# THU-DA-6D-Pose-Group/GDR-Net

Hardware: AMD Instinct MI355X
Metric: RoI crops/sec (fwd+bwd) at 256×256 bs=64 (higher is better)
Workload: dtype bf16; 1 GPU; LM-13 a6_cPnP_lm13 graph: ResNet-34 + RotWithRegionHead + ConvPnPNet, 256x256 RoIs, bs=64/GPU, train step: fwd + 8 losses + bwd + fused Ranger optimizer step (all inside the timed region); global_batch=64, parallelism=dp1

## Files before the change

gdr-net_amd/cabi.py:

```python
import ctypes as C
import os

_HERE = os.path.dirname(os.path.abspath(__file__))
LIB_PATH = os.environ.get("GDRN_HIP_LIB") or os.path.join(_HERE, "lib", "libgdrn_hip.so")
LIB_PATH_F16 = os.environ.get("GDRN_HIP_LIB_F16") or os.path.join(_HERE, "lib", "libgdrn_hip_f16.so")

F32, BF16, F16 = 0, 1, 2
PREZEROED = 0x100
ACC_ROWS = 0x200
P = C.c_void_p
I = C.c_int
LL = C.c_longlong
F = C.c_float
D = C.c_double


class GdrnHipError(RuntimeError):
    pass


class ConvParams(C.Structure):
    _fields_ = [
        ("x", P), ("w", P), ("y", P), ("bias", P), ("addend", P), ("stats", P),
        ("bnb_x", P), ("bnb_mask", P), ("bnb_mean", P), ("bnb_invstd", P), ("bnb_scale", P), ("bnb_shift", P), ("bnb_rows", P),
        ("bnb_cs", I), ("w_frag", I),
        ("Hi", I), ("Wi", I), ("Cin", I), ("x_cs", I),
        ("Ho", I), ("Wo", I), ("Cout", I), ("y_cs", I), ("add_cs", I),
        ("KH", I), ("KW", I), ("stride", I), ("pad", I),
        ("mode", I), ("act", I), ("out_f32", I),
        ("M", I), ("w_rows", I), ("dtype", I),
        ("xf_mode", I), ("xf_relu", I),
        ("xf_x2", P), ("xf_a", P), ("xf_b", P), ("xf_c", P), ("xf_c2", P), ("xf_msc", P), ("xf_msh", P), ("xf_out", P),
        ("halo_waves", I), ("v3_min_wg", I),
    ]


class WgradParams(C.Structure):
    _fields_ = [
        ("x", P), ("dy", P), ("dw", P), ("ws", P),
        ("Hi", I), ("Wi", I), ("Cin", I), ("x_cs", I),
        ("Ho", I), ("Wo", I), ("Cout", I), ("dy_cs", I),
        ("KH", I), ("KW", I), ("stride", I), ("pad", I),
        ("M", I), ("dtype", I), ("splits", I), ("variant", I),
    ]


class S2Params(C.Structure):
    _fields_ = [
        ("x", P), ("w", P), ("y", P), ("bias", P), ("stats", P), ("wd", P), ("yd", P), ("bias_d", P), ("stats_d", P),
        ("Hi", I), ("Wi", I), ("Cin", I), ("x_cs", I),
        ("Ho", I), ("Wo", I), ("Cout", I), ("y_cs", I), ("yd_cs", I),
        ("N", I), ("w_rows", I), ("wd_rows", I), ("act", I), ("dtype", I),
        ("bnb_x", P), ("bnb_mask", P), ("bnb_mean", P), ("bnb_invstd", P), ("bnb_rows", P), ("bnb_cs", I),
    ]


class S2dParams(C.Structure):
    _fields_ = [
        ("dy", P), ("w", P), ("dx", P), ("dyd", P), ("wdd", P), ("bnb_x", P), ("bnb_mask", P), ("bnb_mean", P), ("bnb_invstd", P), ("bnb_rows", P),
        ("bnb_cs", I),
        ("Hi", I), ("Wi", I), ("Cin", I), ("dx_cs", I),
        ("Ho", I), ("Wo", I), ("Cout", I), ("dy_cs", I), ("dyd_cs", I),
        ("N", I), ("w_rows", I), ("wdd_rows", I), ("dtype", I),
        ("stats", P), ("bias", P), ("act", I),
    ]


class PoseParams(C.Structure):
    _fields_ = [
        ("fc", P), ("fs", I), ("cams", P), ("centers", P), ("whs", P), ("ratios", P), ("extents", P),
        ("gt_rot", P), ("gt_trans", P), ("gt_trans_ratio", P), ("points", P), ("npts", I),
        ("sym", P), ("sym_count", P), ("Kmax", I), ("N", I), ("train", I),
        ("rot", P), ("trans", P), ("losses", P), ("dfc", P), ("vis", P),
        ("loss_rows", P), ("gw", P), ("dfc_comb", P), ("fc2_ws", P), ("fc2_bias", P), ("f2_out", P), ("w_rt", P), ("b_rt", P), ("fc_w", P), ("fc2_splits", I),
    ]


class PackTask(C.Structure):
    _fields_ = [
        ("src", P), ("dst", P), ("scale", P),
        ("A1", I), ("A2", I), ("T", I), ("B", I), ("A1v", I), ("A2v", I), ("Bv", I), ("flip", I),
        ("s1", LL), ("s2", LL), ("st", LL), ("sb", LL), ("n", LL), ("frag", I), ("pad_", I),
    ]


def transpose_blocks(lib, t):
    if t.frag or t.flip or t.scale or t.sb == 1:
        return 0
    for u, (stride, size) in enumerate(((t.s1, t.A1), (t.s2, t.A2), (t.st, t.T)), start=1):
        if stride == 1 and size >= 32:
            t.frag, t.pad_ = 3, u
            nb = int(lib.gdrn_pack_transpose_blocks(C.byref(t)))
            if nb > 0:
                return nb
            t.frag, t.pad_ = 0, 0
    return 0


class ZeroTask(C.Structure):
    _fields_ = [("p", P), ("n16", LL)]


class WreduceTask(C.Structure):
    _fields_ = [("ws", P), ("dst", P), ("nsplit", I), ("Cout", I), ("Cin", I), ("cin_valid", I), ("s_co", LL), ("s_ci", LL), ("s_t", LL)]


class RangerTask(C.Structure):
    _fields_ = [("p", P), ("g", P), ("m", P), ("v", P), ("slow", P), ("rows", I), ("cols", I), ("gc", I), ("lr", F)]


class RoiTask(C.Structure):
    _fields_ = [
        ("image", P), ("coord2d", P), ("xyz_crop", P), ("seg", P), ("trunc", P),
        ("cx", D), ("cy", D), ("scale", D), ("bw", D), ("bh", D), ("ox", D), ("oy", D), ("tz", D),
        ("H", I), ("W", I), ("x1", I), ("y1", I), ("x2", I), ("y2", I), ("cls", I), ("pad_", I),
    ]


class AugTask(C.Structure):
    _fields_ = [
        ("frame", P), ("mask", P), ("bg", P), ("out", P), ("mask_trunc", P),
        ("inv_scale", D), ("trunc_u", D),
        ("H", I), ("W", I), ("bg_h", I), ("bg_w", I), ("ch", I), ("cw", I), ("oh", I), ("ow", I),
        ("trunc_mode", I), ("gh", I), ("gw", I), ("keep_off", I), ("lut_off", I), ("blur_r", I),
        ("blur_w", F * 9),
    ]


class RleTask(C.Structure):
    _fields_ = [
        ("mask", P), ("sy", LL), ("sx", LL), ("str_off", LL), ("run_off", LL), ("seg_off", LL),
        ("str_len", I), ("h", I), ("w", I), ("pad_", I),
    ]


def to_device_table(structs, device):
    import torch

    arr = (type(structs[0]) * len(structs))(*structs)
    return torch.frombuffer(bytearray(bytes(arr)), dtype=torch.uint8).to(device)


_SIGS = {
    "gdrn_version": [],
    "gdrn_last_hip_error": [C.c_char_p, I],
    "gdrn_workspace_bytes": [I, P],
    "gdrn_device_info": [I, C.c_char_p, C.POINTER(I), C.c_char_p],
    "gdrn_conv_gemm": [C.POINTER(ConvParams), P],
    "gdrn_correspondences": [P, P, P, P, LL, I, P, P, P, F, I, I, P, P, P, P, P, P],
    "gdrn_pack_stem_w32": [P, P, I, P],
    "gdrn_stem_stats_rows": [I],
    "gdrn_stem_conv": [P, P, P, P, I, I, P],
    "gdrn_stem_conv_pool": [P, P, P, P, P, I, I, P],
    "gdrn_head_conv_tail_fwd": [P, I, P, I, P, P, P, P, I, P, I, I, I, I, I, P],
    "gdrn_head_conv_tail_loss_rows": [I, I],
    "gdrn_head_out_dgrad_rows": [I, I],
    "gdrn_head_out_dgrad": [P, I, P, I, P, I, P, P, P, P, P, I, P, I, I, I, P],
    "gdrn_head_conv_tail_loss_fwd": [P, I, P, I, P, P, P, P, I, P, I, P, P, P, P, P, I, I, I, I, P],
    "gdrn_stem_wgrad_parts": [I],
    "gdrn_stem_wgrad": [P, P, P, P, P, P, I, P, P, I, P],
    "gdrn_linear_splitk": [P, P, P, P, I, I, I, I, I, I, I, P, I, P],
    "gdrn_conv_tile": [C.POINTER(ConvParams), C.POINTER(I), C.POINTER(I)],
    "gdrn_conv_stats_rows": [C.POINTER(ConvParams)],
    "gdrn_pack_wfrag": [P, P, I, I, I, P],
    "gdrn_pack_wfrag32": [P, P, I, I, I, P],
    "gdrn_conv3x3_wfrag": [C.POINTER(ConvParams)],
    "gdrn_conv3x3_halo": [C.POINTER(ConvParams), P],
    "gdrn_conv3x3_tile": [C.POINTER(ConvParams), C.POINTER(I), C.POINTER(I), C.POINTER(I)],
    "gdrn_conv3x3_stats_rows": [C.POINTER(ConvParams)],
    "gdrn_conv3x3_halo_waves": [C.POINTER(ConvParams)],
    "gdrn_conv_wgrad": [C.POINTER(WgradParams), P],
    "gdrn_conv3x3_wgrad": [C.POINTER(WgradParams), P],
    "gdrn_conv3x3_wgrad_ok": [C.POINTER(WgradParams)],
    "gdrn_conv3x3_wgrad_splits": [C.POINTER(WgradParams)],
    "gdrn_conv3x3_wgrad_multi": [P, P, I, I, P],
    "gdrn_conv3x3_wgrad_multi_lds": [P, P, I, I, I, P],
    "gdrn_wgrad_reduce_multi": [P, P, I, I, P],
    "gdrn_pack4": [P, P, I, I, I, I, I, I, I, LL, LL, LL, LL, I, I, P],
    "gdrn_unpack4": [P, P, I, I, I, I, I, I, I, LL, LL, LL, LL, I, P],
    "gdrn_pack_stem_w": [P, P, I, P],
    "gdrn_unpack_stem_w": [P, P, P],
    "gdrn_pack_image": [P, P, I, I, I, I, I, I, P],
    "gdrn_cast_from_f32": [P, P, LL, I, P],
    "gdrn_cast_to_f32": [P, P, LL, I, P],
    "gdrn_nhwc_to_nchw_f32": [P, I, I, I, P, I, I, I, P],
    "gdrn_bn_finalize": [P, I, I, D, P, P, P, P, P, F, F, P, P, P, P, P, P],
    "gdrn_bn_eval_params": [P, P, P, P, F, I, P, P, P],
    "gdrn_bn_apply": [P, P, P, P, P, LL, I, I, I, P],
    "gdrn_bn_bwd_reduce_rows": [LL, I, I],
    "gdrn_bn_bwd_reduce": [P, P, P, P, P, P, P, LL, I, P, I, P],
    "gdrn_bn_bwd_coef": [P, I, I, LL, P, P, P, P, P, P, P, P, P],
    "gdrn_bn_bwd_apply": [P, P, P, P, P, P, P, P, LL, I, P, P, I, P],
    "gdrn_bn_relu_maxpool_fwd": [P, P, P, P, P, I, I, I, I, I, P],
    "gdrn_maxpool_bwd_rows": [I, I, I, I, I],
    "gdrn_maxpool_bwd": [P, P, P, P, P, P, I, I, I, I, P, P, P, I, P],
    "gdrn_upsample2x_fwd": [P, P, I, I, I, I, I, P],
    "gdrn_upsample2x_bwd": [P, P, I, I, I, I, I, P],
    "gdrn_conv3x3s2_ok": [C.POINTER(S2Params)],
    "gdrn_conv3x3s2_stats_rows": [C.POINTER(S2Params)],
    "gdrn_conv3x3s2": [C.POINTER(S2Params), P],
    "gdrn_conv3x3s2_dgrad_ok": [C.POINTER(S2dParams)],
    "gdrn_conv3x3s2_dgrad_rows": [C.POINTER(S2dParams)],
    "gdrn_conv3x3s2_dgrad": [C.POINTER(S2dParams), P],
    "gdrn_block64_eval_ok": [I, I, I, I],
    "gdrn_block64_eval": [P, P, P, P, P, P, I, I, I, I, P],
    "gdrn_bn_relu_upsample2x_fwd": [P, P, P, P, I, I, I, I, I, P],
    "gdrn_upsample2x_bwd_bnsums": [P, P, P, P, P, P, P, I, I, I, I, P, I, P],
    "gdrn_gn_relu_fwd": [P, P, P, P, P, I, I, I, I, F, I, P],
    "gdrn_gn_relu_bwd": [P, P, P, P, P, P, P, P, I, I, I, I, I, P],
    "gdrn_leaky_bwd": [P, P, P, LL, I, P],
    "gdrn_bias_grad": [P, I, I, I, P, I, P],
    "gdrn_head_tail_fwd": [P, I, P, P, P, I, I, I, I, I, P],
    "gdrn_head_tail_loss_fwd": [P, I, P, P, P, I, P, P, P, P, P, I, I, I, I, P],
    "gdrn_map_loss_fwd": [P, I, P, P, P, P, I, I, I, P, P],
    "gdrn_map_loss_finalize": [P, I, I, P, P],
    "gdrn_head_tail_loss_rows": [I, I, I, I, I],
    "gdrn_map_loss_finalize_rows": [P, I, I, I, P, P],
    "gdrn_loss_finalize": [P, I, I, I, P, P, P, P, P],
    "gdrn_linear_splits": [I, I],
    "gdrn_head_tail_bwd": [P, I, P, P, I, P, P, P, P, P, P, P, P, I, I, I, I, I, P],
    "gdrn_pose_loss": [C.POINTER(PoseParams), P],
    "gdrn_combine3": [P, P, P, I, P],
    "gdrn_ranger_step": [P, P, P, P, P, I, I, I, F, F, F, F, F, F, I, I, F, P],
    "gdrn_pack_chunk": [],
    "gdrn_zero_chunk": [],
    "gdrn_zero_multi": [P, P, I, I, P],
    "gdrn_nonfinite_flag": [P, LL, P, P],
    "gdrn_pack_multi": [P, P, I, I, I, P],
    "gdrn_pack_transpose_blocks": [P],
    "gdrn_unpack_multi": [P, P, I, I, P],
    "gdrn_ranger_multi": [P, P, I, I, F, F, F, F, F, I, I, F, F, P],
    "gdrn_ranger_multi_dyn": [P, P, I, I, F, F, F, F, I, I, F, F, P, P],
    "gdrn_loss_scale_update": [P, I, P],
    "gdrn_unscale_or_zero": [P, LL, F, P, P],
    "gdrn_scaled_loss_weights": [P, P, I, P, P, P],
    "gdrn_roi_affine": [P, I, I, I, P, P, P, P, P],
    "gdrn_roi_crop_inputs": [P, P, I, I, I, C.POINTER(D), C.POINTER(D), P, P, P],
    "gdrn_roi_targets": [P, P, I, I, P, I, P, P, P, P, P, P, P],
    "gdrn_pose_metrics_workspace_bytes": [I, I],
    "gdrn_pose_errors": [P, P, P, P, P, P, P, I, P, P, I, P, P, P, I, I, P, P, P],
    "gdrn_pose_recall_accumulate": [P, P, P, I, P, I, P, P, P, P, P, P],
    "gdrn_pnp_workspace_bytes": [I, I, I],
    "gdrn_pnp_ransac": [P, P, P, P, P, I, I, D, I, C.c_ulonglong, I, P, P, P, P, P, P, P, P],
    "gdrn_pnp_refine": [P, P, P, P, P, I, I, I, P, P, P, P, P, P],
    "gdrn_pnp_ransac_f64": [P, P, P, P, P, I, I, D, I, C.c_ulonglong, I, P, P, P, P, P, P, P, P],
    "gdrn_pnp_refine_f64": [P, P, P, P, P, I, I, I, P, P, P, P, P, P],
    "gdrn_render_depth": [P, P, P, P, P, P, I, I, P, P, P, P, P, I, I, I, D, D, P, P],
    "gdrn_xyz_from_depth": [P, P, P, P, I, I, I, P, P, P, P, P],
    "gdrn_vsd_workspace_bytes": [I, I, I, I],
    "gdrn_vsd": [P, P, P, P, P, I, P, P, I, I, I, D, P, I, I, I, P, P, P, P],
    "gdrn_mssd_mspd_workspace_bytes": [I, I, I],
    "gdrn_mssd_mspd": [P, P, P, P, P, P, P, I, P, P, I, P, P, P, I, I, P, P, P],
    "gdrn_bop_recall_accumulate": [P, I, P, P, P, I, P, I, D, P, P, P, P, P, P, P, P],
    "gdrn_ad_errors_workspace_bytes": [I, I],
    "gdrn_ad_errors": [P, P, P, P, P, P, I, P, P, I, I, P, P, P],
    "gdrn_sym_errors_workspace_bytes": [I, I, I],
    "gdrn_sym_errors": [P, P, P, P, P, P, P, I, P, P, I, P, P, P, I, I, P, P, P],
    "gdrn_score_recall_accumulate": [P, P, P, P, I, P, P, I, P, P, P],
    "gdrn_aug_mask_cuts": [P, C.POINTER(AugTask), I, P, P],
    "gdrn_aug_frames": [P, C.POINTER(AugTask), I, P, LL, P, P],
    "gdrn_rle_decode": [P, C.POINTER(RleTask), I, P, LL, P, LL, P, P, P],
    "gdrn_rle_count": [P, C.POINTER(RleTask), I, P, LL, P, P, P],
    "gdrn_rle_positions": [P, C.POINTER(RleTask), I, P, LL, P, P, LL, P],
    "gdrn_rle_string": [P, C.POINTER(RleTask), I, P, P, LL, P, P, LL, P, P],
    "gdrn_model_prep_workspace_bytes": [I, I, I],
    "gdrn_model_bounds": [P, P, P, I, I, P, P],
    "gdrn_model_fps": [P, P, P, I, I, I, P, P, P, P],
    "gdrn_model_diameter": [P, P, P, I, I, P, P],
    "gdrn_scene_gt_canvas": [P, I, I, I, I, I, P, P, P, P],
    "gdrn_scene_gt_compose": [P, P, P, P, P, I, I, I, I, P, P],
    "gdrn_scene_gt_visibility": [P, P, P, P, I, P, I, I, I, D, I, P, P, P, P, P, P, P, P, P],
    "gdrn_render_visibility": [P, P, P, P, P, P, I, I, P, P, P, P, P, I, I, I, D, D, P, P],
    "gdrn_shade_frames": [P, P, P, P, P, P, P, P, P, I, P, P, P, P, P, P, P, P, P, I, I, I, I, P, P, P, P, P, P, P, P, P],
    "gdrn_shade_frames_tex": [P, P, P, P, P, P, P, P, P, P, P, P, P, I, I, P, P, P, P, P, P, P, P, P, I, I, I, I, P, P, I, I, P, P, P, P, P, P, P],
    "gdrn_cou_maps_workspace_bytes": [I],
    "gdrn_cou_maps": [P, P, I, I, I, I, P, P, P, P, P],
    "gdrn_cou_bb": [P, P, I, P, P],
    "gdrn_icp_workspace_bytes": [I, I, I],
    "gdrn_icp_accumulate": [P, P, P, P, I, P, I, I, I, D, D, P, P, P, P],
    "gdrn_icp_step": [P, P, I, I, P, P, P, P],
    "gdrn_icp_refine": [P, P, P, P, P, P, I, I, P, P, P, P, P, I, P, P, P, I, I, I, D, D, I, D, D, I, P, P, P, P, P, P, P],
    "gdrn_depth_align_workspace_bytes": [I, I, I],
    "gdrn_depth_offset": [P, P, P, P, I, I, I, I, D, I, P, P, P, P, P, P],
    "gdrn_depth_align": [P, P, P, P, P, P, I, I, P, P, P, P, P, I, P, P, P, I, I, I, D, D, I, D, I, P, P, P, P, P, P, P],
    "gdrn_sil_workspace_bytes": [I, I, I],
    "gdrn_sil_contour_transform": [P, P, P, P, I, I, I, I, P, P, P, P, P],
    "gdrn_sil_accumulate": [P, P, P, P, I, P, P, P, I, I, I, D, D, P, P, P, P],
    "gdrn_icp_step_sil": [P, P, P, P, D, I, I, P, P, P, P],
    "gdrn_icp_refine_sil": [P, P, P, P, P, P, I, I, P, P, P, P, P, I, P, P, P, I, P, I, I, D, D, I, D, D, I, D, D, P, P, P, P, P, P, P, P, P],
}

_SIGS["gdrn_half_format"] = []
_RET_LL = ("gdrn_workspace_bytes", "gdrn_pose_metrics_workspace_bytes", "gdrn_pnp_workspace_bytes", "gdrn_vsd_workspace_bytes",
           "gdrn_mssd_mspd_workspace_bytes", "gdrn_model_prep_workspace_bytes", "gdrn_ad_errors_workspace_bytes",
           "gdrn_sym_errors_workspace_bytes", "gdrn_cou_maps_workspace_bytes", "gdrn_icp_workspace_bytes",
           "gdrn_depth_align_workspace_bytes", "gdrn_sil_workspace_bytes")
EXPORTS = tuple(_SIGS.keys())
_libs = {}


def lib_path(dtype=BF16):
    return LIB_PATH_F16 if dtype == F16 else LIB_PATH


def load(dtype=BF16):
    kind = F16 if dtype == F16 else BF16
    if kind in _libs:
        return _libs[kind]
    import torch

    path = lib_path(kind)
    if not os.path.exists(path):
# ... 32 lines not shown
```

gdr-net_amd/csrc/conv_wgrad.hip:

```cpp
#include <hip/amd_detail/amd_hip_unsafe_atomics.h>

#include <cstdlib>

#include "common.h"
#include "launch_host.h"

namespace {

typedef __attribute__((address_space(3))) bf16x4_t lds_bf16x4_t;

template <typename T, int BCO, int BCI>
__global__ __launch_bounds__(256) void conv_wgrad_kernel(const gdrn_wgrad_params p) {
    constexpr int ESZ = (int)sizeof(T);
    constexpr int BKM = (ESZ == 2) ? 64 : 32;
    constexpr int PADB = (ESZ == 2) ? 32 : 64;
    constexpr int PA = BCO * ESZ + PADB, PB = BCI * ESZ + PADB;
    constexpr int SEGA = BCO * ESZ / 16, SEGB = BCI * ESZ / 16;
    constexpr int LDA = BKM * SEGA / 256, LDB = BKM * SEGB / 256;
    constexpr int RSA = 256 / SEGA, RSB = 256 / SEGB;
    constexpr int WCO = BCO / 2, WCI = BCI / 2;
    constexpr int FA = WCO / 16, FB = WCI / 16;
    extern __shared__ __attribute__((aligned(16))) unsigned char smem[];
    unsigned char* sA = smem;
    unsigned char* sB = smem + 2 * BKM * PA;

    const int tid = threadIdx.x, lane = tid & 63, wave = tid >> 6;
    const int wa = wave >> 1, wb = wave & 1;
    const int g = lane >> 4, r16 = lane & 15;

    const int KK = p.KH * p.KW;
    const int ncit = p.Cin / BCI;
    const int ncot = (p.Cout + BCO - 1) / BCO;
    const int ntile = ncot * ncit * KK;
    const int nsplit = (int)gridDim.x / ntile;
    int bid = blockIdx.x;
    {
        const int nwg = gridDim.x, q = nwg >> 3, r = nwg & 7, xcd = bid & 7, j = bid >> 3;
        bid = (xcd < r ? xcd * (q + 1) : r * (q + 1) + (xcd - r) * q) + j;
    }
    const int split = bid / ntile;
    int tile = bid - split * ntile;
    const int cot = tile % ncot; tile /= ncot;
    const int cit = tile % ncit;
    const int tap = tile / ncit;
    const int co0 = cot * BCO, ci0 = cit * BCI;
    const int ky = tap / p.KW, kx = tap - ky * p.KW;

    const int nstage_all = (p.M + BKM - 1) / BKM;
    const int per = (nstage_all + nsplit - 1) / nsplit;
    const int s_begin = split * per;
    const int s_end = min(nstage_all, s_begin + per);
    if (s_begin >= s_end) return;

    const int segA = tid % SEGA, rowA = tid / SEGA;
    const int segB = tid % SEGB, rowB = tid / SEGB;
    const char* dyg = reinterpret_cast<const char*>(p.dy);
    const char* xg = reinterpret_cast<const char*>(p.x);
    const int HW = p.Ho * p.Wo;
    const bool pow2 = (p.Wo & (p.Wo - 1)) == 0 && (HW & (HW - 1)) == 0;
    const int lgW = 31 - __builtin_clz(p.Wo), lgHW = 31 - __builtin_clz(HW);

    uint4 ra[LDA], rb[LDB];
    auto load_stage = [&](int s) {
        const int m0 = s * BKM;
#pragma unroll
        for (int i = 0; i < LDA; ++i) {
            const int m = m0 + rowA + RSA * i;
            uint4 v = make_uint4(0, 0, 0, 0);
            if (m < p.M) v = *reinterpret_cast<const uint4*>(dyg + ((size_t)m * p.dy_cs + co0) * ESZ + segA * 16);
            ra[i] = v;
        }
#pragma unroll
        for (int i = 0; i < LDB; ++i) {
            const int m = m0 + rowB + RSB * i;
            uint4 v = make_uint4(0, 0, 0, 0);
            if (m < p.M) {
                int n, oy, ox;
                if (pow2) {
                    n = m >> lgHW;
                    const int rem = m & (HW - 1);
                    oy = rem >> lgW;
                    ox = rem & (p.Wo - 1);
                } else {
                    n = m / HW;
                    const int rem = m - n * HW;
                    oy = rem / p.Wo;
                    ox = rem - oy * p.Wo;
                }
                const int iy = oy * p.stride - p.pad + ky, ix = ox * p.stride - p.pad + kx;
                if (iy >= 0 && iy < p.Hi && ix >= 0 && ix < p.Wi)
                    v = *reinterpret_cast<const uint4*>(xg + ((size_t)((n * p.Hi + iy) * p.Wi + ix) * p.x_cs + ci0) * ESZ + segB * 16);
            }
            rb[i] = v;
        }
    };
    auto write_stage = [&](int buf) {
#pragma unroll
        for (int i = 0; i < LDA; ++i)
            *reinterpret_cast<uint4*>(sA + (size_t)buf * BKM * PA + (rowA + RSA * i) * PA + segA * 16) = ra[i];
#pragma unroll
        for (int i = 0; i < LDB; ++i)
            *reinterpret_cast<uint4*>(sB + (size_t)buf * BKM * PB + (rowB + RSB * i) * PB + segB * 16) = rb[i];
    };

    f32x4_t acc[FA][FB];
#pragma unroll
    for (int a = 0; a < FA; ++a)
#pragma unroll
        for (int b = 0; b < FB; ++b) acc[a][b] = f32x4_t{0.f, 0.f, 0.f, 0.f};

    load_stage(s_begin);
    write_stage(0);
    __syncthreads();

    for (int s = s_begin; s < s_end; ++s) {
        const int buf = (s - s_begin) & 1;
        if (s + 1 < s_end) load_stage(s + 1);
        const unsigned char* tA = sA + (size_t)buf * BKM * PA;
        const unsigned char* tB = sB + (size_t)buf * BKM * PB;
        if constexpr (ESZ == 2) {
#pragma unroll
            for (int ks = 0; ks < BKM / 32; ++ks) {
                bf16x8_t fa[FA], fb[FB];
                {
                    const int trow = ks * 32 + g * 4 + (r16 >> 2), tcol = (r16 & 3) * 4;
#pragma unroll
                    for (int a = 0; a < FA; ++a) {
                        const unsigned char* q0 = tA + trow * PA + (wa * WCO + a * 16 + tcol) * 2;
                        bf16x4_t lo = GDRN_TR16((lds_bf16x4_t*)(q0));
                        bf16x4_t hi = GDRN_TR16((lds_bf16x4_t*)(q0 + 16 * PA));
                        fa[a] = __builtin_shufflevector(lo, hi, 0, 1, 2, 3, 4, 5, 6, 7);
                    }
#pragma unroll
                    for (int b = 0; b < FB; ++b) {
                        const unsigned char* q0 = tB + trow * PB + (wb * WCI + b * 16 + tcol) * 2;
                        bf16x4_t lo = GDRN_TR16((lds_bf16x4_t*)(q0));
                        bf16x4_t hi = GDRN_TR16((lds_bf16x4_t*)(q0 + 16 * PB));
                        fb[b] = __builtin_shufflevector(lo, hi, 0, 1, 2, 3, 4, 5, 6, 7);
                    }
                }
#pragma unroll
                for (int a = 0; a < FA; ++a)
#pragma unroll
                    for (int b = 0; b < FB; ++b)
                        acc[a][b] = GDRN_MFMA16(fa[a], fb[b], acc[a][b]);
            }
        } else {
#pragma unroll 4
            for (int ks = 0; ks < BKM / 4; ++ks) {
                float fa[FA], fb[FB];
                const int mrow = ks * 4 + g;
#pragma unroll
                for (int a = 0; a < FA; ++a)
                    fa[a] = *reinterpret_cast<const float*>(tA + mrow * PA + (wa * WCO + a * 16 + r16) * 4);
#pragma unroll
                for (int b = 0; b < FB; ++b)
                    fb[b] = *reinterpret_cast<const float*>(tB + mrow * PB + (wb * WCI + b * 16 + r16) * 4);
#pragma unroll
                for (int a = 0; a < FA; ++a)
#pragma unroll
                    for (int b = 0; b < FB; ++b)
                        acc[a][b] = __builtin_amdgcn_mfma_f32_16x16x4f32(fa[a], fb[b], acc[a][b], 0, 0, 0);
            }
        }
        if (s + 1 < s_end) write_stage(buf ^ 1);
        __syncthreads();
    }

#pragma unroll
    for (int a = 0; a < FA; ++a) {
#pragma unroll
        for (int j = 0; j < 4; ++j) {
            const int co = co0 + wa * WCO + a * 16 + g * 4 + j;
            if (co >= p.Cout) continue;
#pragma unroll
            for (int b = 0; b < FB; ++b) {
                const int ci = ci0 + wb * WCI + b * 16 + r16;
                unsafeAtomicAdd(p.dw + ((size_t)co * KK + tap) * p.Cin + ci, acc[a][b][j]);
            }
        }
    }
}

template <typename T, int BCO, int BCI>
int launch(const gdrn_wgrad_params& p, hipStream_t st) {
    constexpr int ESZ = (int)sizeof(T);
    constexpr int BKM = (ESZ == 2) ? 64 : 32;
    constexpr int PADB = (ESZ == 2) ? 32 : 64;
    constexpr size_t smem = 2 * (size_t)BKM * ((BCO * ESZ + PADB) + (BCI * ESZ + PADB));
    if (!lds_limit_once<&conv_wgrad_kernel<T, BCO, BCI>>(smem)) return GDRN_ERR_LAUNCH;
    const int tiles = cdiv(p.Cout, BCO) * (p.Cin / BCI) * p.KH * p.KW;
    int splits = p.splits;
    if (splits <= 0) {
        const int nst = cdiv(p.M, BKM);
        constexpr int target = 2048;
        splits = max(1, min(nst / 8 > 0 ? nst / 8 : 1, cdiv(target, tiles)));
    }
    GDRN_LAUNCH((conv_wgrad_kernel<T, BCO, BCI>), dim3(tiles * splits), dim3(256), smem, st, p);
    GDRN_CHECK_LAUNCH();
    return GDRN_OK;
}

}

extern "C" int gdrn_conv_wgrad(const gdrn_wgrad_params* pp, void* stream) {
    if (!pp || !pp->x || !pp->dy || !pp->dw) return GDRN_ERR_ARG;
    const gdrn_wgrad_params& p = *pp;
    if (p.dtype != GDRN_DT_F32 && p.dtype != GDRN_DT_H16) return GDRN_ERR_ARG;
    const int esz = p.dtype == GDRN_DT_H16 ? 2 : 4;
    if (p.Cin <= 0 || p.Cin % 64 != 0 || p.M <= 0 || p.Cout <= 0) return GDRN_ERR_SHAPE;
    if (p.KH <= 0 || p.KW <= 0 || p.stride <= 0 || p.pad < 0 || p.Hi <= 0 || p.Wi <= 0 || p.Ho <= 0 || p.Wo <= 0) return GDRN_ERR_SHAPE;
    if (p.M % (p.Ho * p.Wo) != 0) return GDRN_ERR_SHAPE;
    if (p.x_cs <= 0 || ((p.x_cs * esz) % 16 != 0 && (p.x_cs * esz) % 8 != 0)) return GDRN_ERR_SHAPE;
    if ((p.dy_cs * esz) % 16 != 0) return GDRN_ERR_SHAPE;
    const int bco = p.Cout <= 64 ? 64 : 128;
    const int bci = (p.Cin % 128 == 0) ? 128 : 64;
    if (p.dy_cs < cdiv(p.Cout, bco) * bco) return GDRN_ERR_SHAPE;
    hipStream_t st = reinterpret_cast<hipStream_t>(stream);
    if (p.dtype == GDRN_DT_H16) {
        if (bco == 64) return bci == 64 ? launch<bf16_t, 64, 64>(p, st) : launch<bf16_t, 64, 128>(p, st);
        return bci == 64 ? launch<bf16_t, 128, 64>(p, st) : launch<bf16_t, 128, 128>(p, st);
    } else {
        if (bco == 64) return bci == 64 ? launch<float, 64, 64>(p, st) : launch<float, 64, 128>(p, st);
        return bci == 64 ? launch<float, 128, 64>(p, st) : launch<float, 128, 128>(p, st);
    }
}
```

gdr-net_amd/csrc/multi.hip:

```cpp
#include <algorithm>

#include "common.h"
#include "../../include/gdrn_hip.h"

namespace {

__device__ __forceinline__ int find_task(const int* __restrict__ start, int n, int b) {
    int lo = 0, hi = n;
    while (hi - lo > 1) {
        const int mid = (lo + hi) >> 1;
        if (start[mid] <= b) lo = mid; else hi = mid;
    }
    return lo;
}

constexpr int PACK_CHUNK = 2048;

struct TrGeo { int U, Uv, O1, O2, O1v, O2v, UT, BT; };
__host__ __device__ inline TrGeo tr_geo(const gdrn_pack_task& k) {
    TrGeo g;
    const int d[3] = {k.A1, k.A2, k.T}, dv[3] = {k.A1v, k.A2v, k.T};
    const int u = k.pad_ - 1, a = u == 0 ? 1 : 0, b = u == 2 ? 1 : 2;
    g.U = d[u]; g.Uv = dv[u]; g.O1 = d[a]; g.O2 = d[b]; g.O1v = dv[a]; g.O2v = dv[b];
    g.UT = (g.U + 63) / 64; g.BT = (k.B + 63) / 64;
    return g;
}
__host__ inline bool tr_ok(const gdrn_pack_task& k) {
    if (k.frag != 3 || k.pad_ < 1 || k.pad_ > 3 || k.flip || k.scale != nullptr) return false;
    const long long s[3] = {k.s1, k.s2, k.st};
    return s[k.pad_ - 1] == 1 && k.A1 > 0 && k.A2 > 0 && k.T > 0 && k.B > 0;
}
__device__ __forceinline__ void tr_idx(const gdrn_pack_task& k, int u, int o1, int o2, int& a1, int& a2, int& t) {
    if (k.pad_ == 1) { a1 = u; a2 = o1; t = o2; }
    else if (k.pad_ == 2) { a1 = o1; a2 = u; t = o2; }
    else { a1 = o1; a2 = o2; t = u; }
}
template <typename T, bool UNPACK>
__device__ __forceinline__ void tr_tile(const gdrn_pack_task& k, int blk) {
    __shared__ float tile[64][68];
    const TrGeo g = tr_geo(k);
    const int bt = blk % g.BT; blk /= g.BT;
    const int ut = blk % g.UT; blk /= g.UT;
    const int o2 = blk % g.O2, o1 = blk / g.O2;
    const int u0 = ut * 64, b0 = bt * 64;
    const long long sa = (k.pad_ == 1 ? 0 : k.s1) | (k.pad_ == 2 ? 0 : k.s2) | (k.pad_ == 3 ? 0 : k.st) | k.sb;
    const bool v4 = (sa & 3) == 0 && (g.Uv & 3) == 0 && (reinterpret_cast<uintptr_t>(UNPACK ? k.dst : (const void*)k.src) & 15) == 0;
    const bool b8 = (k.B & 7) == 0 && (reinterpret_cast<uintptr_t>(UNPACK ? (const void*)k.src : k.dst) & 15) == 0;
    auto strided = [&](int u, int b) -> long long {
        int a1, a2, t;
        tr_idx(k, u, o1, o2, a1, a2, t);
        return (long long)a1 * k.s1 + (long long)a2 * k.s2 + (long long)t * k.st + (long long)b * k.sb;
    };
    auto dense = [&](int u, int b) -> long long {
        int a1, a2, t;
        tr_idx(k, u, o1, o2, a1, a2, t);
        return (((long long)a1 * k.A2 + a2) * k.T + t) * k.B + b;
    };
    auto valid = [&](int u, int b) -> bool {
        int a1, a2, t;
        tr_idx(k, u, o1, o2, a1, a2, t);
        return u < g.Uv && b < k.Bv && a1 < k.A1v && a2 < k.A2v;
    };
    if constexpr (!UNPACK) {
        if (v4) {
            for (int i = threadIdx.x; i < 1024; i += 256) {
                const int u4 = (i & 15) * 4, bb = i >> 4, u = u0 + u4, b = b0 + bb;
                float4 v = make_float4(0.f, 0.f, 0.f, 0.f);
                if (valid(u, b)) v = *reinterpret_cast<const float4*>(k.src + strided(u, b));
                *reinterpret_cast<float4*>(&tile[bb][u4]) = v;
            }
        } else {
            for (int i = threadIdx.x; i < 4096; i += 256) {
                const int uu = i & 63, bb = i >> 6, u = u0 + uu, b = b0 + bb;
                tile[bb][uu] = valid(u, b) ? k.src[strided(u, b)] : 0.f;
            }
        }
        __syncthreads();
        T* dst = reinterpret_cast<T*>(k.dst);
        if (b8) {
            for (int i = threadIdx.x; i < 512; i += 256) {
                const int b8_ = (i & 7) * 8, uu = i >> 3, u = u0 + uu, b = b0 + b8_;
                if (u < g.U && b < k.B) {
                    float v[8];
#pragma unroll
                    for (int j2 = 0; j2 < 8; ++j2) v[j2] = tile[b8_ + j2][uu];
                    T* d = dst + dense(u, b);
                    if constexpr (sizeof(T) == 2) *reinterpret_cast<uint4*>(d) = Vec16<T>::pack(v);
                    else { Vec16<T>::store(d, v); Vec16<T>::store(d + 4, v + 4); }
                }
            }
        } else {
            for (int i = threadIdx.x; i < 4096; i += 256) {
                const int bb = i & 63, uu = i >> 6, u = u0 + uu, b = b0 + bb;
                if (u < g.U && b < k.B) st1<T>(dst + dense(u, b), tile[bb][uu]);
            }
        }
    } else {
        if (b8) {
            for (int i = threadIdx.x; i < 1024; i += 256) {
                const int b4 = (i & 15) * 4, uu = i >> 4, u = u0 + uu, b = b0 + b4;
                float4 v = make_float4(0.f, 0.f, 0.f, 0.f);
                if (u < g.U && b < k.B) v = *reinterpret_cast<const float4*>(k.src + dense(u, b));
                tile[b4][uu] = v.x; tile[b4 + 1][uu] = v.y; tile[b4 + 2][uu] = v.z; tile[b4 + 3][uu] = v.w;
            }
        } else {
            for (int i = threadIdx.x; i < 4096; i += 256) {
                const int bb = i & 63, uu = i >> 6, u = u0 + uu, b = b0 + bb;
                tile[bb][uu] = (u < g.U && b < k.B) ? k.src[dense(u, b)] : 0.f;
            }
        }
        __syncthreads();
        float* dst = reinterpret_cast<float*>(k.dst);
        if (v4) {
            for (int i = threadIdx.x; i < 1024; i += 256) {
                const int u4 = (i & 15) * 4, bb = i >> 4, u = u0 + u4, b = b0 + bb;
                if (valid(u, b)) *reinterpret_cast<float4*>(dst + strided(u, b)) = *reinterpret_cast<const float4*>(&tile[bb][u4]);
            }
        } else {
            for (int i = threadIdx.x; i < 4096; i += 256) {
                const int uu = i & 63, bb = i >> 6, u = u0 + uu, b = b0 + bb;
                if (valid(u, b)) dst[strided(u, b)] = tile[bb][uu];
            }
        }
    }
}

template <typename T>
__global__ __launch_bounds__(256) void pack_multi_kernel(const gdrn_pack_task* __restrict__ tasks, const int* __restrict__ blk_start,
                                                         int ntasks) {
    constexpr int EPS = 128 / (int)sizeof(T), GE = 16 / (int)sizeof(T);
    const int t = find_task(blk_start, ntasks, blockIdx.x);
    const gdrn_pack_task k = tasks[t];
    T* dst = reinterpret_cast<T*>(k.dst);
    if (k.frag == 3) { tr_tile<T, false>(k, blockIdx.x - blk_start[t]); return; }
    if constexpr (sizeof(T) == 2) {
        if (k.frag) {
            __shared__ bf16_t tile[16][9][72];
            const int brick = blockIdx.x - blk_start[t];
            const int kch = k.B >> 6;
            const int cb = brick / kch, kc = brick - cb * kch;
            const int b0 = kc * 64;
            const int FNp = k.A1 <= 64 ? 1 : 2;
            auto srow = [&](int a) {
                if (k.frag == 2) { const int f = cb >> 1, r = (cb & 1) * 16 + a; return (f >> 1) * 64 + ((r >> 2) & 1) * 32 + (f & 1) * 16 + (r >> 3) * 4 + (r & 3); }
                return (cb / FNp) * 16 * FNp + (a >> 2) * (4 * FNp) + (cb % FNp) * 4 + (a & 3);
            };
            __shared__ float rsc[16];
            if (threadIdx.x < 16) rsc[threadIdx.x] = (k.scale != nullptr && srow((int)threadIdx.x) < k.A1v) ? k.scale[srow((int)threadIdx.x)] : 1.f;
            __syncthreads();
            const bool full = srow(15) < k.A1v && b0 + 63 < k.Bv && ((size_t)k.src & 15) == 0;
            if (full && k.st == 1 && k.sb == 9 && (k.s1 & 3) == 0) {
                for (int q = threadIdx.x; q < 16 * 144; q += 256) {
                    const int a = q / 144, r4 = (q - a * 144) * 4;
                    const float4 v4 = *reinterpret_cast<const float4*>(k.src + (long long)srow(a) * k.s1 + (long long)b0 * 9 + r4);
                    const float vv[4] = {v4.x, v4.y, v4.z, v4.w};
#pragma unroll
                    for (int e = 0; e < 4; ++e) {
                        const int r = r4 + e, b = r / 9, tp = r - b * 9;
                        tile[a][k.flip ? 8 - tp : tp][b] = f2bf(vv[e] * rsc[a]);
                    }
                }
            } else if (full && k.st == 1 && k.s1 == 9 && (k.sb & 3) == 0) {
                for (int q = threadIdx.x; q < 64 * 4 * 9; q += 256) {
                    const int b = q / 36, r = q - b * 36, grp = r / 9, f4 = r - grp * 9;
                    const float4 v4 = *reinterpret_cast<const float4*>(k.src + (long long)srow(grp * 4) * 9 + (long long)(b0 + b) * k.sb + f4 * 4);
                    const float vv[4] = {v4.x, v4.y, v4.z, v4.w};
#pragma unroll
                    for (int e = 0; e < 4; ++e) {
                        const int w = f4 * 4 + e, al = w / 9, tp = w - al * 9, a = grp * 4 + al;
                        tile[a][k.flip ? 8 - tp : tp][b] = f2bf(vv[e] * rsc[a]);
                    }
                }
            } else if (k.st == 1 && k.sb == 9) {
                for (int idx = threadIdx.x; idx < 16 * 576; idx += 256) {
                    const int a = idx / 576, r = idx - a * 576, b = r / 9, tp = r - b * 9;
                    const bool ok = srow(a) < k.A1v && b0 + b < k.Bv;
                    const float v = ok ? k.src[(long long)srow(a) * k.s1 + (long long)(b0 + b) * 9 + tp] * rsc[a] : 0.f;
                    tile[a][k.flip ? 8 - tp : tp][b] = f2bf(v);
                }
            } else if (k.st == 1 && k.s1 == 9) {
                for (int idx = threadIdx.x; idx < 64 * 144; idx += 256) {
                    const int b = idx / 144, r = idx - b * 144, a = r / 9, tp = r - a * 9;
                    const bool ok = srow(a) < k.A1v && b0 + b < k.Bv;
                    const float v = ok ? k.src[(long long)srow(a) * 9 + (long long)(b0 + b) * k.sb + tp] * rsc[a] : 0.f;
                    tile[a][k.flip ? 8 - tp : tp][b] = f2bf(v);
                }
            } else {
                for (int idx = threadIdx.x; idx < 16 * 576; idx += 256) {
                    const int a = idx / 576, r = idx - a * 576, b = r / 9, tp = r - b * 9;
                    const bool ok = srow(a) < k.A1v && b0 + b < k.Bv;
                    const float v = ok ? k.src[(long long)srow(a) * k.s1 + (long long)(b0 + b) * k.sb + (long long)tp * k.st] * rsc[a] : 0.f;
                    tile[a][k.flip ? 8 - tp : tp][b] = f2bf(v);
                }
            }
            __syncthreads();
            if (k.frag == 2) {
                const int nfr = k.A1 >> 5, f = cb >> 1, half = cb & 1;
                for (int gi = threadIdx.x; gi < 9 * 4 * 32; gi += 256) {
                    const int a = gi & 15, hh = (gi >> 4) & 1, ks = (gi >> 5) & 3, tap = gi >> 7;
                    const uint4 v = *reinterpret_cast<const uint4*>(&tile[a][tap][(ks * 2 + hh) * 8]);
                    *reinterpret_cast<uint4*>(dst + ((size_t)((((kc * 9 + tap) * 4 + ks) * nfr + f) * 64 + hh * 32 + half * 16 + a) << 3)) = v;
                }
                return;
            }
            for (int gi = threadIdx.x; gi < 9 * 2 * 64; gi += 256) {
                const int lane = gi & 63, ks = (gi >> 6) & 1, tap = gi >> 7;
                const uint4 v = *reinterpret_cast<const uint4*>(&tile[lane & 15][tap][(ks * 4 + (lane >> 4)) * 8]);
                *reinterpret_cast<uint4*>(dst + ((size_t)((((cb * 9 + tap) * kch + kc) * 2 + ks) * 64 + lane) << 3)) = v;
            }
            return;
        }
    }
    const long long base = (long long)(blockIdx.x - blk_start[t]) * PACK_CHUNK;
    if ((k.B % GE) == 0 && (k.n % GE) == 0) {
        const unsigned B = (unsigned)k.B, Tt = (unsigned)k.T, A2 = (unsigned)k.A2;
        for (int g = threadIdx.x; g < PACK_CHUNK / GE; g += 256) {
            const long long i = base + (long long)g * GE;
            if (i >= k.n) break;
            unsigned a1, a2, tt, b0;
            unsigned r = (unsigned)(i / GE);
            if (k.frag) {
                const unsigned lane = r & 63u; r >>= 6;
                const unsigned ks = r & 1u; r >>= 1;
                const unsigned kch = B / EPS;
                unsigned kc;
                if (k.pad_ > 0) { kc = r & (kch - 1u); r >>= (unsigned)(k.pad_ - 1); }
                else { kc = r % kch; r /= kch; }
                tt = r % 9u;
                {
                    const unsigned cbq = r / 9u, rr = lane & 15u, fnp = (k.A1 <= 64 || sizeof(T) == 4) ? 1u : 2u;
                    a1 = (cbq / fnp) * 16u * fnp + (rr >> 2) * (4u * fnp) + (cbq % fnp) * 4u + (rr & 3u);
                }
                a2 = 0;
                b0 = kc * EPS + (ks * 4u + (lane >> 4)) * GE;
            } else {
                const unsigned bg = B / GE;
                b0 = (r % bg) * GE; r /= bg;
                tt = r % Tt; r /= Tt;
                a2 = r % A2;
                a1 = r / A2;
            }
            float v[GE];
            const bool ok = (int)a1 < k.A1v && (int)a2 < k.A2v;
            const unsigned ts = k.flip ? (Tt - 1u - tt) : tt;
            const float* sp = k.src + (long long)a1 * k.s1 + (long long)a2 * k.s2 + (long long)ts * k.st;
            const float rs = (k.scale != nullptr && ok) ? k.scale[a1] : 1.f;
#pragma unroll
            for (int el = 0; el < GE; ++el) {
                const int b = (int)b0 + el;
                v[el] = (ok && b < k.Bv) ? sp[(long long)b * k.sb] * rs : 0.f;
            }
            Vec16<T>::store(dst + i, v);
        }
        return;
    }
    for (int e = threadIdx.x; e < PACK_CHUNK; e += 256) {
        const long long i = base + e;
        if (i >= k.n) break;
        int a1, a2, tt, b;
        if (k.frag) {
            const int el = (int)(i % GE);
            long long r = i / GE;
            const int lane = (int)(r & 63); r >>= 6;
            const int ks = (int)(r & 1); r >>= 1;
            const int kch = k.B / EPS;
            const int kc = (int)(r % kch); r /= kch;
            tt = (int)(r % 9);
            {
                const int cbq = (int)(r / 9), rr = lane & 15, fnp = (k.A1 <= 64 || sizeof(T) == 4) ? 1 : 2;
                a1 = (cbq / fnp) * 16 * fnp + (rr >> 2) * (4 * fnp) + (cbq % fnp) * 4 + (rr & 3);
            }
            a2 = 0;
            b = kc * EPS + (ks * 4 + (lane >> 4)) * GE + el;
        } else {
            b = (int)(i % k.B);
            long long r = i / k.B;
            tt = (int)(r % k.T); r /= k.T;
            a2 = (int)(r % k.A2);
            a1 = (int)(r / k.A2);
        }
        float v = 0.f;
        if (a1 < k.A1v && a2 < k.A2v && b < k.Bv) {
            const int ts = k.flip ? (k.T - 1 - tt) : tt;
            v = k.src[a1 * k.s1 + a2 * k.s2 + ts * k.st + b * k.sb] * (k.scale != nullptr ? k.scale[a1] : 1.f);
        }
        st1<T>(dst + i, v);
    }
}

constexpr int ZERO_CHUNK = 4096;
__global__ __launch_bounds__(256) void zero_multi_kernel(const gdrn_zero_task* __restrict__ tasks, const int* __restrict__ blk_start, int ntasks) {
    const int t = find_task(blk_start, ntasks, blockIdx.x);
    const gdrn_zero_task k = tasks[t];
    const long long base = (long long)(blockIdx.x - blk_start[t]) * ZERO_CHUNK;
    uint4* dst = reinterpret_cast<uint4*>(k.p);
    for (int i = threadIdx.x; i < ZERO_CHUNK; i += 256) {
        const long long g = base + i;
        if (g >= k.n16) break;
        dst[g] = make_uint4(0u, 0u, 0u, 0u);
    }
}

__global__ __launch_bounds__(256) void unpack_multi_kernel(const gdrn_pack_task* __restrict__ tasks, const int* __restrict__ blk_start,
                                                           int ntasks) {
    const int t = find_task(blk_start, ntasks, blockIdx.x);
    const gdrn_pack_task k = tasks[t];
    if (k.frag == 3) { tr_tile<float, true>(k, blockIdx.x - blk_start[t]); return; }
    const long long base = (long long)(blockIdx.x - blk_start[t]) * PACK_CHUNK;
    float* dst = reinterpret_cast<float*>(k.dst);
    if ((k.Bv & 3) == 0 && (k.B & 3) == 0) {
        const unsigned bq = (unsigned)k.Bv >> 2, Tt = (unsigned)k.T, A2v = (unsigned)k.A2v;
        for (int g = threadIdx.x; g < PACK_CHUNK / 4; g += 256) {
            const long long i = base + (long long)g * 4;
            if (i >= k.n) break;
            unsigned r = (unsigned)(i >> 2);
            const unsigned b = (r % bq) * 4u; r /= bq;
            const unsigned tt = r % Tt; r /= Tt;
            const unsigned a2 = r % A2v, a1 = r / A2v;
            const unsigned ts = k.flip ? (Tt - 1u - tt) : tt;
            const float4 v = *reinterpret_cast<const float4*>(k.src + (((long long)a1 * k.A2 + a2) * k.T + tt) * k.B + b);
            float* dp = dst + (long long)a1 * k.s1 + (long long)a2 * k.s2 + (long long)ts * k.st + (long long)b * k.sb;
            dp[0] = v.x;
            dp[k.sb] = v.y;
            dp[2 * k.sb] = v.z;
            dp[3 * k.sb] = v.w;
        }
        return;
    }
    for (int e = threadIdx.x; e < PACK_CHUNK; e += 256) {
        const long long i = base + e;
        if (i >= k.n) break;
        const int b = (int)(i % k.Bv);
        long long r = i / k.Bv;
        const int tt = (int)(r % k.T); r /= k.T;
        const int a2 = (int)(r % k.A2v);
        const int a1 = (int)(r / k.A2v);
        const int ts = k.flip ? (k.T - 1 - tt) : tt;
        dst[a1 * k.s1 + a2 * k.s2 + ts * k.st + b * k.sb] = k.src[(((long long)a1 * k.A2 + a2) * k.T + tt) * k.B + b];
    }
}

__global__ __launch_bounds__(256) void ranger_multi_kernel(const gdrn_ranger_task* __restrict__ tasks, const int* __restrict__ row_start,
                                                           int ntasks, float beta1, float beta2, float eps, float wd, float step_size,
                                                           int adaptive, int lookahead, float alpha, float grad_scale,
                                                           const gdrn_loss_scale_state* __restrict__ dyn, int n_sma_threshold, int lookahead_k) {
    __shared__ float red[4];
    if (dyn != nullptr) {
        if (dyn->flag != 0) return;
        const int step = dyn->base_step + dyn->applied + 1;
        const double b2t = pow((double)beta2, (double)step), b1t = pow((double)beta1, (double)step);
        const double nmax = 2.0 / (1.0 - (double)beta2) - 1.0;
        const double nsma = nmax - 2.0 * step * b2t / (1.0 - b2t);
        adaptive = nsma > (double)n_sma_threshold;
        step_size = (float)(adaptive ? sqrt((1.0 - b2t) * (nsma - 4.0) / (nmax - 4.0) * (nsma - 2.0) / nsma * nmax / (nmax - 2.0)) / (1.0 - b1t)
                                     : 1.0 / (1.0 - b1t));
        lookahead = (step % lookahead_k) == 0;
        grad_scale *= dyn->inv_scale;
    }
    const int t = find_task(row_start, ntasks, blockIdx.x);
    const gdrn_ranger_task k = tasks[t];
    const size_t base = (size_t)(blockIdx.x - row_start[t]) * k.cols;
    ranger_row(k.p + base, k.g + base, k.m + base, k.v + base, k.slow + base, k.cols, k.gc, k.lr, beta1, beta2, eps, wd, step_size, adaptive, lookahead, alpha,
               grad_scale, red);
}

}

#define ST reinterpret_cast<hipStream_t>(stream)

extern "C" int gdrn_pack_chunk(void) { return PACK_CHUNK; }

extern "C" int gdrn_pack_transpose_blocks(const gdrn_pack_task* k) {
    if (!k || !tr_ok(*k)) return 0;
    const TrGeo g = tr_geo(*k);
    const long long nb = (long long)g.O1 * g.O2 * g.UT * g.BT;
    return nb > 0 && nb < (1ll << 30) ? (int)nb : 0;
}

extern "C" int gdrn_pack_multi(const gdrn_pack_task* tasks_dev, const int* blk_start_dev, int ntasks, int nblocks, int dtype, void* stream) {
    if (!tasks_dev || !blk_start_dev || ntasks <= 0 || nblocks <= 0) return GDRN_ERR_ARG;
    if (dtype == GDRN_DT_F32) GDRN_LAUNCH(pack_multi_kernel<float>, dim3(nblocks), dim3(256), 0, ST, tasks_dev, blk_start_dev, ntasks);
    else if (dtype == GDRN_DT_H16) GDRN_LAUNCH(pack_multi_kernel<bf16_t>, dim3(nblocks), dim3(256), 0, ST, tasks_dev, blk_start_dev, ntasks);
    else return GDRN_ERR_ARG;
    GDRN_CHECK_LAUNCH();
    return GDRN_OK;
}

extern "C" int gdrn_unpack_multi(const gdrn_pack_task* tasks_dev, const int* blk_start_dev, int ntasks, int nblocks, void* stream) {
    if (!tasks_dev || !blk_start_dev || ntasks <= 0 || nblocks <= 0) return GDRN_ERR_ARG;
    GDRN_LAUNCH(unpack_multi_kernel, dim3(nblocks), dim3(256), 0, ST, tasks_dev, blk_start_dev, ntasks);
    GDRN_CHECK_LAUNCH();
    return GDRN_OK;
}

extern "C" int gdrn_zero_chunk(void) { return ZERO_CHUNK; }

namespace {
__global__ __launch_bounds__(256) void nonfinite_flag_kernel(const float* __restrict__ x, long long n, int* __restrict__ flag) {
    const long long n4 = n >> 2;
    unsigned bad = 0;
    for (long long i = (long long)blockIdx.x * 256 + threadIdx.x; i < n4; i += (long long)gridDim.x * 256) {
        const uint4 v = *reinterpret_cast<const uint4*>(x + 4 * i);
        bad |= ((v.x & 0x7f800000u) == 0x7f800000u) | ((v.y & 0x7f800000u) == 0x7f800000u) | ((v.z & 0x7f800000u) == 0x7f800000u) |
               ((v.w & 0x7f800000u) == 0x7f800000u);
    }
    if (blockIdx.x == 0 && threadIdx.x < (int)(n & 3)) bad |= (__float_as_uint(x[(n4 << 2) + threadIdx.x]) & 0x7f800000u) == 0x7f800000u;
    if (__any(bad != 0) && (threadIdx.x & 63) == 0) atomicOr(flag, 1);
}
}

extern "C" int gdrn_nonfinite_flag(const float* x, long long n, int* flag, void* stream) {
    if (!x || !flag || n <= 0 || (reinterpret_cast<uintptr_t>(x) & 15)) return GDRN_ERR_ARG;
    const int grid = (int)std::min<long long>(((n >> 2) + 255) / 256 + 1, 2048);
    GDRN_LAUNCH(nonfinite_flag_kernel, dim3(grid), dim3(256), 0, ST, x, n, flag);
    GDRN_CHECK_LAUNCH();
    return GDRN_OK;
}

extern "C" int gdrn_zero_multi(const gdrn_zero_task* tasks_dev, const int* blk_start_dev, int ntasks, int nblocks, void* stream) {
    if (!tasks_dev || !blk_start_dev || ntasks <= 0 || nblocks <= 0) return GDRN_ERR_ARG;
    GDRN_LAUNCH(zero_multi_kernel, dim3(nblocks), dim3(256), 0, ST, tasks_dev, blk_start_dev, ntasks);
    GDRN_CHECK_LAUNCH();
    return GDRN_OK;
}

extern "C" int gdrn_ranger_multi(const gdrn_ranger_task* tasks_dev, const int* row_start_dev, int ntasks, int total_rows, float beta1,
                                 float beta2, float eps, float weight_decay, float step_size, int adaptive, int lookahead, float alpha, float grad_scale,
                                 void* stream) {
    if (!tasks_dev || !row_start_dev || ntasks <= 0 || total_rows <= 0) return GDRN_ERR_ARG;
    GDRN_LAUNCH(ranger_multi_kernel, dim3(total_rows), dim3(256), 0, ST, tasks_dev, row_start_dev, ntasks, beta1, beta2, eps,
                       weight_decay, step_size, adaptive, lookahead, alpha, grad_scale, (const gdrn_loss_scale_state*)nullptr, 0, 1);
    GDRN_CHECK_LAUNCH();
    return GDRN_OK;
}

extern "C" int gdrn_ranger_multi_dyn(const gdrn_ranger_task* tasks_dev, const int* row_start_dev, int ntasks, int total_rows, float beta1,
                                     float beta2, float eps, float weight_decay, int n_sma_threshold, int lookahead_k, float alpha, float grad_scale,
                                     const gdrn_loss_scale_state* dyn, void* stream) {
    if (!tasks_dev || !row_start_dev || !dyn || ntasks <= 0 || total_rows <= 0 || lookahead_k < 1) return GDRN_ERR_ARG;
    GDRN_LAUNCH(ranger_multi_kernel, dim3(total_rows), dim3(256), 0, ST, tasks_dev, row_start_dev, ntasks, beta1, beta2, eps,
                       weight_decay, 0.f, 0, 0, alpha, grad_scale, dyn, n_sma_threshold, lookahead_k);
    GDRN_CHECK_LAUNCH();
    return GDRN_OK;
}

namespace {
__global__ void loss_scale_update_kernel(gdrn_loss_scale_state* __restrict__ s, int applied_step) {
    if (threadIdx.x != 0 || blockIdx.x != 0) return;
    if (s->flag != 0) {
        s->scale = fmaxf(s->scale * 0.5f, 1.f);
        s->good = 0;
        s->skipped += 1;
        s->flag = 0;
        s->last_overflowed = 1;
    } else {
        s->applied += applied_step;
        s->good += 1;
        s->last_overflowed = 0;
        if (s->growth > 0 && s->good >= s->growth && s->scale < 65536.f) {
            s->scale *= 2.f;
            s->good = 0;
// ... 45 lines not shown
```

gdr-net_amd/csrc/norm.hip:

```cpp
#include <hip/amd_detail/amd_hip_unsafe_atomics.h>

#include <algorithm>

#include "common.h"
#include "../../include/gdrn_hip.h"

namespace {

__device__ __forceinline__ void rows_total4(const float* __restrict__ rows, int nrows, int C, int c4, double (&tot)[8], double (*red)[8]) {
    double s[8] = {0.0, 0.0, 0.0, 0.0, 0.0, 0.0, 0.0, 0.0};
#pragma unroll 4
    for (int r = threadIdx.x; r < nrows; r += 256) {
        const float4 a = *reinterpret_cast<const float4*>(rows + ((size_t)r * 2 + 0) * C + c4);
        const float4 b = *reinterpret_cast<const float4*>(rows + ((size_t)r * 2 + 1) * C + c4);
        s[0] += (double)a.x; s[1] += (double)a.y; s[2] += (double)a.z; s[3] += (double)a.w;
        s[4] += (double)b.x; s[5] += (double)b.y; s[6] += (double)b.z; s[7] += (double)b.w;
    }
#pragma unroll
    for (int j = 0; j < 8; ++j)
#pragma unroll
        for (int o = 32; o > 0; o >>= 1) s[j] += __shfl_xor(s[j], o, 64);
    if ((threadIdx.x & 63) == 0) {
#pragma unroll
        for (int j = 0; j < 8; ++j) red[threadIdx.x >> 6][j] = s[j];
    }
    __syncthreads();
#pragma unroll
    for (int j = 0; j < 8; ++j) tot[j] = red[0][j] + red[1][j] + red[2][j] + red[3][j];
}

__global__ __launch_bounds__(256) void bn_finalize_rows_kernel(const float* __restrict__ partial, int rows, int C, double count,
                                                               const float* gamma, const float* beta, float* running_mean,
                                                               float* running_var, long long* nbt, float momentum, float eps,
                                                               float* mean, float* invstd, float* scale, float* shift) {
    __shared__ double red[4][8];
    double tot[8];
    const int c4 = blockIdx.x * 4;
    float k_g = 0.f, k_b = 0.f, k_rm = 0.f, k_rv = 0.f;
    if (threadIdx.x < 4) {
        k_g = gamma[c4 + threadIdx.x];
        k_b = beta[c4 + threadIdx.x];
        if (running_mean != nullptr) { k_rm = running_mean[c4 + threadIdx.x]; k_rv = running_var[c4 + threadIdx.x]; }
    }
    rows_total4(partial, rows, C, c4, tot, red);
    if (threadIdx.x < 4) {
        const int ch = c4 + threadIdx.x;
        const double s1 = tot[threadIdx.x], s2 = tot[4 + threadIdx.x];
        const double m = s1 / count;
        double var = s2 / count - m * m;
        if (var < 0.0) var = 0.0;
        const double is = 1.0 / sqrt(var + (double)eps);
        mean[ch] = (float)m;
        invstd[ch] = (float)is;
        const float sc = k_g * (float)is;
        scale[ch] = sc;
        shift[ch] = k_b - (float)m * sc;
        if (running_mean != nullptr) {
            const double unb = count > 1.0 ? var * count / (count - 1.0) : var;
            running_mean[ch] = (1.f - momentum) * k_rm + momentum * (float)m;
            running_var[ch] = (1.f - momentum) * k_rv + momentum * (float)unb;
        }
    }
    if (blockIdx.x == 0 && threadIdx.x == 0 && nbt != nullptr) *nbt += 1;
}

__global__ __launch_bounds__(256) void bn_bwd_coef_kernel(const float* __restrict__ rows, int nrows, int C, float inv_n,
                                                          const float* gamma, const float* mean, const float* invstd,
                                                          float* ka, float* kb, float* kc, float* dgamma, float* dbeta) {
    __shared__ double red[4][8];
    double tot[8];
    const int c4 = blockIdx.x * 4;
    float k_g = 0.f, k_mu = 0.f, k_is = 0.f;
    if (threadIdx.x < 4) { k_g = gamma[c4 + threadIdx.x]; k_mu = mean[c4 + threadIdx.x]; k_is = invstd[c4 + threadIdx.x]; }
    rows_total4(rows, nrows, C, c4, tot, red);
    if (threadIdx.x < 4) {
        const int ch = c4 + threadIdx.x;
        float m1 = (float)tot[threadIdx.x], m2 = (float)tot[4 + threadIdx.x];
        if (dgamma != nullptr) { dbeta[ch] = m1; dgamma[ch] = m2; }
        m1 *= inv_n;
        m2 *= inv_n;
        const float a = k_g * k_is, b = -a * k_is * m2;
        ka[ch] = a;
        kb[ch] = b;
        kc[ch] = -a * m1 - b * k_mu;
    }
}

__global__ void bn_eval_params_kernel(const float* gamma, const float* beta, const float* rm, const float* rv, float eps,
                                      int C, float* scale, float* shift) {
    const int c = blockIdx.x * blockDim.x + threadIdx.x;
    if (c < C) {
        const float sc = gamma[c] / sqrtf(rv[c] + eps);
        scale[c] = sc;
        shift[c] = beta[c] - rm[c] * sc;
    }
}

template <typename T>
__global__ __launch_bounds__(256) void bn_apply_kernel(const T* __restrict__ x, const float* __restrict__ scale,
                                                       const float* __restrict__ shift, const T* __restrict__ res,
                                                       T* __restrict__ y, long long npix, int C, int relu, int rows_per_block) {
    constexpr int V = Vec16<T>::VEC;
    const int tpr = C / V, rpp = 256 / tpr;
    const int cv = threadIdx.x % tpr, rl = threadIdx.x / tpr;
    __shared__ float kst[2][512];
    for (int c = threadIdx.x; c < C; c += 256) { kst[0][c] = scale[c]; kst[1][c] = shift[c]; }
    __syncthreads();
    float sc[V], sh[V];
#pragma unroll
    for (int j = 0; j < V; ++j) { sc[j] = kst[0][cv * V + j]; sh[j] = kst[1][cv * V + j]; }
    const long long r0 = (long long)blockIdx.x * rows_per_block;
    const long long r1 = min(npix, r0 + rows_per_block);
    if (rl >= rpp) return;
    for (long long r = r0 + rl; r < r1; r += rpp) {
        const size_t o = (size_t)r * C + cv * V;
        float v[V], q[V];
        Vec16<T>::load(x + o, v);
        if (res != nullptr) Vec16<T>::load(res + o, q);
#pragma unroll
        for (int j = 0; j < V; ++j) {
            float t = __builtin_fmaf(v[j], sc[j], sh[j]);
            if (res != nullptr) t += q[j];
            if (relu) t = fmaxf(t, 0.f);
            v[j] = t;
        }
        Vec16<T>::store(y + o, v);
    }
}

template <typename T>
__global__ __launch_bounds__(256) void bn_bwd_reduce_kernel(const T* __restrict__ dy, const T* __restrict__ ym,
                                                            const T* __restrict__ x, const float* __restrict__ mean,
                                                            const float* __restrict__ invstd, const float* __restrict__ msc,
                                                            const float* __restrict__ msh, long long npix, int C,
                                                            float* __restrict__ rows, int rows_per_block) {
    constexpr int V = Vec16<T>::VEC;
    const int tpr = C / V, rpp = 256 / tpr;
    const int cv = threadIdx.x % tpr, rl = threadIdx.x / tpr;
    __shared__ float kst[4][512];
    __shared__ float part[4][2 * 512];
    for (int c = threadIdx.x; c < C; c += 256) {
        kst[0][c] = mean[c];
        kst[1][c] = invstd[c];
        kst[2][c] = msc ? msc[c] : 0.f;
        kst[3][c] = msc ? msh[c] : 1.f;
    }
// ... 711 lines not shown
    for (int r = rl; r < HW; r += rpp) {
        float g[V], yv[V], xv[V], o[V];
        const size_t off = base + (size_t)r * C + cv * V;
        Vec16<T>::load(dy + off, g);
        Vec16<T>::load(y + off, yv);
        Vec16<T>::load(x + off, xv);
#pragma unroll
        for (int j = 0; j < V; ++j) {
            const float gg = (yv[j] > 0.f) ? g[j] : 0.f;
            const float xh = (xv[j] - mu[j]) * rs[j];
            o[j] = rs[j] * (gg * gm[j] - A[j] - xh * B[j]);
        }
        Vec16<T>::store(dx + off, o);
    }
}

template <typename T>
__global__ __launch_bounds__(256) void leaky_bwd_kernel(const T* dy, const T* y, T* dx, long long nvec) {
    constexpr int V = Vec16<T>::VEC;
    for (long long i = (long long)blockIdx.x * blockDim.x + threadIdx.x; i < nvec; i += (long long)gridDim.x * blockDim.x) {
        float g[V], yv[V];
        Vec16<T>::load(dy + i * V, g);
        Vec16<T>::load(y + i * V, yv);
#pragma unroll
        for (int j = 0; j < V; ++j) g[j] = (yv[j] > 0.f) ? g[j] : 0.1f * g[j];
        Vec16<T>::store(dx + i * V, g);
    }
}

template <typename T>
__global__ __launch_bounds__(256) void bias_grad_kernel(const T* __restrict__ dy, int cs, int rows, int C, float* db,
                                                        int rows_per_block) {
    constexpr int V = Vec16<T>::VEC;
    __shared__ float acc[1024];
    const int tpr = cs / V;
    const int rpp = 256 / tpr;
    const int cv = threadIdx.x % tpr, rl = threadIdx.x / tpr;
    for (int i = threadIdx.x; i < cs; i += 256) acc[i] = 0.f;
    __syncthreads();
    float s[V];
#pragma unroll
    for (int j = 0; j < V; ++j) s[j] = 0.f;
    const int r0 = blockIdx.x * rows_per_block, r1 = min(rows, r0 + rows_per_block);
    if (rl < rpp) {
        for (int r = r0 + rl; r < r1; r += rpp) {
            float v[V];
            Vec16<T>::load(dy + (size_t)r * cs + cv * V, v);
#pragma unroll
            for (int j = 0; j < V; ++j) s[j] += v[j];
        }
#pragma unroll
        for (int j = 0; j < V; ++j) atomicAdd(&acc[cv * V + j], s[j]);
    }
    __syncthreads();
    for (int c = threadIdx.x; c < C; c += 256) unsafeAtomicAdd(&db[c], acc[c]);
}

inline void ew_rows(long long npix, int tpr, int* rpb, int* blocks) {
    const int rpp = 256 / tpr;
    long long r = (npix + 2047) / 2048;
    r = (r + rpp - 1) / rpp * rpp;
    if (r < 4LL * rpp) r = 4LL * rpp;
    *rpb = (int)r;
    *blocks = (int)((npix + r - 1) / r);
}

inline int ew_grid(long long n) { return (int)std::min<long long>((n + 255) / 256, 256LL * 16); }

}

#define ST reinterpret_cast<hipStream_t>(stream)

extern "C" int gdrn_bn_finalize(const float* partial, int rows, int C, double count, const float* gamma, const float* beta,
                                float* running_mean, float* running_var, long long* nbt, float momentum, float eps,
                                float* mean, float* invstd, float* scale, float* shift, double* ws, void* stream) {
    (void)ws;
    if (!partial || !gamma || !beta || !mean || !invstd || !scale || !shift || rows <= 0 || C <= 0 || (C & 3)) return GDRN_ERR_ARG;
    GDRN_LAUNCH(bn_finalize_rows_kernel, dim3(C / 4), dim3(256), 0, ST, partial, rows, C, count, gamma, beta, running_mean,
                       running_var, nbt, momentum, eps, mean, invstd, scale, shift);
    GDRN_CHECK_LAUNCH();
    return GDRN_OK;
}

extern "C" int gdrn_bn_bwd_coef(const float* rows, int nrows, int C, long long npix, const float* gamma, const float* mean,
                                const float* invstd, float* a, float* b, float* c, float* dgamma, float* dbeta, void* stream) {
    if (!rows || !gamma || !mean || !invstd || !a || !b || !c || nrows <= 0 || C <= 0 || (C & 3) || npix <= 0) return GDRN_ERR_ARG;
    if ((dgamma != nullptr) != (dbeta != nullptr)) return GDRN_ERR_ARG;
    GDRN_LAUNCH(bn_bwd_coef_kernel, dim3(C / 4), dim3(256), 0, ST, rows, nrows, C, (float)(1.0 / (double)npix), gamma, mean,
                       invstd, a, b, c, dgamma, dbeta);
    GDRN_CHECK_LAUNCH();
    return GDRN_OK;
}

extern "C" int gdrn_bn_eval_params(const float* gamma, const float* beta, const float* rm, const float* rv, float eps, int C,
                                   float* scale, float* shift, void* stream) {
    if (!gamma || !beta || !rm || !rv || !scale || !shift || C <= 0) return GDRN_ERR_ARG;
    GDRN_LAUNCH(bn_eval_params_kernel, dim3(cdiv(C, 256)), dim3(256), 0, ST, gamma, beta, rm, rv, eps, C, scale, shift);
    GDRN_CHECK_LAUNCH();
    return GDRN_OK;
}

extern "C" int gdrn_bn_apply(const void* x, const float* scale, const float* shift, const void* residual, void* y,
                             long long npix, int C, int relu, int dtype, void* stream) {
    if (!x || !scale || !shift || !y || npix <= 0 || C <= 0 || C > 512 || (C % 8)) return GDRN_ERR_ARG;
    const int V = dtype == GDRN_DT_H16 ? 8 : 4;
    if ((C / V) > 256 || 256 % (C / V)) return GDRN_ERR_SHAPE;
    int rpb, blocks;
    ew_rows(npix, C / V, &rpb, &blocks);
    DISPATCH(dtype,
             GDRN_LAUNCH(bn_apply_kernel<float>, dim3(blocks), dim3(256), 0, ST, (const float*)x, scale,
                                shift, (const float*)residual, (float*)y, npix, C, relu, rpb),
             GDRN_LAUNCH(bn_apply_kernel<bf16_t>, dim3(blocks), dim3(256), 0, ST, (const bf16_t*)x,
                                scale, shift, (const bf16_t*)residual, (bf16_t*)y, npix, C, relu, rpb));
    GDRN_CHECK_LAUNCH();
    return GDRN_OK;
}

static void bwd_reduce_grid(long long npix, int C, int dtype, int* rpb_out, int* blocks_out) {
    const int V = dtype == GDRN_DT_H16 ? 8 : 4;
    const int rpp = 256 / (C / V);
    int rpb = rpp * 4;
    long long blocks = (npix + rpb - 1) / rpb;
    if (blocks > 1024) { rpb = (int)(((npix + 1023) / 1024 + rpp - 1) / rpp * rpp); blocks = (npix + rpb - 1) / rpb; }
    *rpb_out = rpb;
    *blocks_out = (int)blocks;
}

extern "C" int gdrn_bn_bwd_reduce_rows(long long npix, int C, int dtype) {
    if (npix <= 0 || C <= 0 || C > 512 || (C % 8)) return GDRN_ERR_ARG;
    const int V = dtype == GDRN_DT_H16 ? 8 : 4;
    if (256 % (C / V)) return GDRN_ERR_SHAPE;
    int rpb, blocks;
    bwd_reduce_grid(npix, C, dtype, &rpb, &blocks);
    return blocks;
}

extern "C" int gdrn_bn_bwd_reduce(const void* dy, const void* ymask, const void* x, const float* mean, const float* invstd,
                                  const float* mask_scale, const float* mask_shift, long long npix, int C, float* rows, int dtype,
                                  void* stream) {
    if (!dy || !x || !mean || !invstd || !rows || npix <= 0 || C <= 0 || C > 512 || (C % 8)) return GDRN_ERR_ARG;
    if ((mask_scale != nullptr) != (mask_shift != nullptr)) return GDRN_ERR_ARG;
    const int V = dtype == GDRN_DT_H16 ? 8 : 4;
    if (256 % (C / V)) return GDRN_ERR_SHAPE;
    int rpb, blocks;
    bwd_reduce_grid(npix, C, dtype, &rpb, &blocks);
    DISPATCH(dtype,
             GDRN_LAUNCH(bn_bwd_reduce_kernel<float>, dim3(blocks), dim3(256), 0, ST, (const float*)dy,
                                (const float*)ymask, (const float*)x, mean, invstd, mask_scale, mask_shift, npix, C, rows, rpb),
             GDRN_LAUNCH(bn_bwd_reduce_kernel<bf16_t>, dim3(blocks), dim3(256), 0, ST, (const bf16_t*)dy,
                                (const bf16_t*)ymask, (const bf16_t*)x, mean, invstd, mask_scale, mask_shift, npix, C, rows, rpb));
    GDRN_CHECK_LAUNCH();
    return GDRN_OK;
}

extern "C" int gdrn_bn_bwd_apply(const void* dy, const void* ymask, const void* x, const float* a, const float* b, const float* c,
                                 const float* mask_scale, const float* mask_shift, long long npix, int C, void* dx, void* g_out,
                                 int dtype, void* stream) {
    if (!dy || !x || !a || !b || !c || !dx || npix <= 0 || C <= 0 || C > 512 || (C % 8)) return GDRN_ERR_ARG;
    if ((mask_scale != nullptr) != (mask_shift != nullptr)) return GDRN_ERR_ARG;
    const int V = dtype == GDRN_DT_H16 ? 8 : 4;
    if ((C / V) > 256 || 256 % (C / V)) return GDRN_ERR_SHAPE;
    int rpb, blocks;
    ew_rows(npix, C / V, &rpb, &blocks);
    DISPATCH(dtype,
             GDRN_LAUNCH(bn_bwd_apply_kernel<float>, dim3(blocks), dim3(256), 0, ST, (const float*)dy,
                                (const float*)ymask, (const float*)x, a, b, c, mask_scale, mask_shift, npix, C,
// ... 188 lines not shown
```

gdr-net_amd/engine.py:

```python
import ctypes as C
import math
from collections import OrderedDict
from types import SimpleNamespace as NS

import torch

from . import cabi
from .cabi import BF16, F16, F32, check, ptr

RESNET34_LAYERS = (3, 4, 6, 3)
RESNET34_PLANES = (64, 128, 256, 512)
HEAD_CONVS = ((3, 4, False), (6, 7, False), (10, 11, True), (13, 14, False), (17, 18, True), (20, 21, False))
BUCKET_LAYOUTS = {
    5: ((25, 17, 14, 8, 0), ("rot_head_net.features.23.bias", "backbone.layer4.2.bn2.bias", "backbone.layer3.5.bn2.bias", "backbone.layer2.3.bn2.bias")),
    4: ((25, 17, 8, 0), ("rot_head_net.features.23.bias", "backbone.layer4.2.bn2.bias", "backbone.layer2.3.bn2.bias")),
}
LOSS_NAMES = ("loss_coor_x", "loss_coor_y", "loss_coor_z", "loss_mask", "loss_region", "loss_PM_R", "loss_centroid", "loss_z")


def _ru(a, b):
    return (a + b - 1) // b * b


class Engine:
# ... 210 lines not shown
        h = "rot_head_net.features."
        self._add_conv(h + "0", "convT", [h + "0.weight"], 256, 512, 3, 3)
        for ci, _, up in HEAD_CONVS:
            self._add_conv(h + str(ci), "conv", [h + f"{ci}.weight"], 256, 256, 3, 3)
        self.head_c = 1 + 3 + self.nreg + 1
        self._add_conv(h + "23", "conv", [h + "23.weight"], self.head_c, 256, 1, 1, out_ch=128)
        q = "pnp_net.features."
        self.pnp_c = 3 + 2 + self.nreg
        self._add_conv(q + "0", "conv", [q + "0.weight"], 128, self.pnp_c, 3, 3, in_ch=128, s2=True)
        self._add_conv(q + "3", "conv", [q + "3.weight"], 128, 128, 3, 3, s2=True)
        self._add_conv(q + "6", "conv", [q + "6.weight"], 128, 128, 3, 3, s2=True)
        self._add_conv("pnp_net.fc1", "fc1", ["pnp_net.fc1.weight"], 1024, 128, 8, 8)
        self._add_conv("pnp_net.fc2", "fc", ["pnp_net.fc2.weight"], 256, 1024, 1, 1)
        self._add_conv("pnp_net.fc_rt", "fc", ["pnp_net.fc_r.weight", "pnp_net.fc_t.weight"], 9, 256, 1, 1)
        tot = 0
        for L in self.layers.values():
            L.dwp_off = tot
            tot += _ru(int(math.prod(L.dwp_shape)), 4)
        self.dwp_flat = torch.zeros(tot, dtype=torch.float32, device=self.dev)
        for L in self.layers.values():
            L.dwp = self.dwp_flat[L.dwp_off: L.dwp_off + int(math.prod(L.dwp_shape))]
        self.bn_ws = torch.zeros(64 * 2 * 512, dtype=torch.float64, device=self.dev)
        self.rt_w = torch.zeros(9, 256, dtype=torch.float32, device=self.dev)
        self.rt_b = torch.zeros(9, dtype=torch.float32, device=self.dev)

    def _src_version(self, L):
        return tuple(self.P[n]._version for n in L.src) + tuple(self.P[n].data_ptr() for n in L.src)

    def _pack_args(self, L, which):
        O, I, KK = L.O, L.I, L.KK
        if L.kind == "convT":
            return ((L.rows_f, 1, KK, L.cin_f, O, 1, I, KK, 0, 1, O * KK, 0) if which == "f"
                    else (L.rows_d, 1, KK, L.cin_d, I, 1, O, O * KK, 0, 1, KK, 0))
        if L.kind == "fc1":
            return ((L.rows_f, 1, KK, L.cin_f, O, 1, I, I * KK, 0, 1, KK, 0) if which == "f"
                    else (KK, L.in_ch, 1, L.cin_d, KK, I, O, 1, KK, 0, I * KK, 0))
        flip = 1 if (KK == 9 and not L.s2) else 0
        return ((L.rows_f, 1, KK, L.cin_f, O, 1, I, I * KK, 0, 1, KK, 0) if which == "f"
                else (L.rows_d, 1, KK, L.cin_d, I, 1, O, KK, 0, 1, I * KK, flip))

    def fold(self, bnkey, L):
        f = self.bn_fold.get(bnkey)
        if f is None:
            C_ = self.P[bnkey + ".weight"].numel()
            f = NS(scale=self._empty(C_, dtype=torch.float32), shift=self._empty(C_, dtype=torch.float32), layer=L, C=C_)
            self.bn_fold[bnkey] = f
            L.wf_e = torch.zeros_like(L.wf)
            L.wfF_e = torch.zeros_like(L.wfF) if L.wfF is not None else None
            self._eval_tab = None
        assert f.layer is L, (bnkey, L.key)
        return f

    def eval_refresh(self):
        from .cabi import PackTask, to_device_table

        lib, st = self.lib, self._stream()
        if not self.bn_fold:
            return
        if getattr(self, "_eval_tab", None) is None:
            chunk = lib.gdrn_pack_chunk()
            tasks, starts = [], [0]
            for bnkey, f in self.bn_fold.items():
                L = f.layer
                src = self.P[L.src[0]]
                halo_only = self.use_halo and self.halo_min_b <= 1 and L.wfF is not None and not L.s2 and L.kind == "conv"
                for dst, frag in ((L.wf_e, 0), (L.wfF_e, L.wfmt.get("e", 0) or 1)):
                    if dst is None or (halo_only and not frag):
                        continue
                    A1, A2, T, B, A1v, A2v, Bv, s1, s2, stt, sb, flip = self._pack_args(L, "f")
                    kch = B * (2 if self.h16 else 4) // 128
                    sh = (kch.bit_length() if (frag and kch > 0 and kch & (kch - 1) == 0) else 0)
                    t = PackTask(src=src.data_ptr(), dst=dst.data_ptr(), scale=f.scale.data_ptr(), A1=A1, A2=A2, T=T, B=B, A1v=A1v,
                                 A2v=A2v, Bv=Bv, flip=flip, s1=s1, s2=s2, st=stt, sb=sb, n=A1 * A2 * T * B, frag=frag, pad_=sh)
                    tasks.append(t)
                    starts.append(starts[-1] + ((A1 // 16) * (B // 64) if (frag and self.h16) else (t.n + chunk - 1) // chunk))
            self._eval_tab = (to_device_table(tasks, self.dev), torch.tensor(starts, dtype=torch.int32, device=self.dev), len(tasks), starts[-1])
        for bnkey, f in self.bn_fold.items():
            g, b = self.P[bnkey + ".weight"], self.P[bnkey + ".bias"]
            rm, rv = self.Bf[bnkey + ".running_mean"], self.Bf[bnkey + ".running_var"]
            check(lib.gdrn_bn_eval_params(ptr(g), ptr(b), ptr(rm), ptr(rv), 1e-5, f.C, ptr(f.scale), ptr(f.shift), st), "bn_eval_params")
        tab, stt, nt, nb = self._eval_tab
        check(lib.gdrn_pack_multi(ptr(tab), ptr(stt), nt, nb, self.dt, st), "pack_multi(eval)")

    def _build_pack_table(self):
        from .cabi import PackTask, to_device_table

        chunk = self.lib.gdrn_pack_chunk()
        tasks, starts = [], [0]
        for key, L in self.layers.items():
            if L.kind == "stem":
                continue
            src = self.rt_w if key == "pnp_net.fc_rt" else self.P[L.src[0]]
            halo_only = self.use_halo and self.halo_min_b <= 1 and L.wfF is not None and not L.s2 and L.kind == "conv"
            for which, dst, frag in (("f", L.wf, 0), ("d", L.wd, 0), ("f", L.wfF, L.wfmt["f"] or 1), ("d", L.wdF, L.wfmt["d"] or 1)):
                if dst is None or (halo_only and not frag):
                    continue
                A1, A2, T, B, A1v, A2v, Bv, s1, s2, st, sb, flip = self._pack_args(L, which)
                kch = B * (2 if self.h16 else 4) // 128
                sh = (kch.bit_length() if (frag and kch > 0 and kch & (kch - 1) == 0) else 0)
                t = PackTask(src=src.data_ptr(), dst=dst.data_ptr(), A1=A1, A2=A2, T=T, B=B, A1v=A1v, A2v=A2v, Bv=Bv, flip=flip,
                             s1=s1, s2=s2, st=st, sb=sb, n=A1 * A2 * T * B, frag=frag, pad_=sh)
                tasks.append(t)
                nblk = (A1 // 16) * (B // 64) if (frag and self.h16) else (cabi.transpose_blocks(self.lib, t) or (t.n + chunk - 1) // chunk)
                starts.append(starts[-1] + nblk)
        self._pack_tasks = to_device_table(tasks, self.dev)
        self._pack_starts = torch.tensor(starts, dtype=torch.int32, device=self.dev)
        self._pack_n = (len(tasks), starts[-1])
        off_of = lambda t: self.grad_offsets[names_of[t.src]]
        names_of = {}
        for key, L in self.layers.items():
            if L.kind != "stem":
                names_of[(self.rt_w if key == "pnp_net.fc_rt" else self.P[L.src[0]]).data_ptr()] = L.src[0]
        self._pack_buckets = []
        for lo, hi in self.bucket_bounds:
            sel = [(t, n) for t, n in zip(tasks, [starts[i + 1] - starts[i] for i in range(len(tasks))]) if lo <= off_of(t) < hi]
            if not sel:
                self._pack_buckets.append(None)
                continue
            st_ = [0]
            for _, n in sel:
                st_.append(st_[-1] + n)
            self._pack_buckets.append((to_device_table([t for t, _ in sel], self.dev), torch.tensor(st_, dtype=torch.int32, device=self.dev), len(sel), st_[-1]))

    def repack(self, force=False):
        sig = tuple(p._version for p in self.P.values())
        if not force and self._versions.get("sig") == sig and not getattr(self, "_pack_dirty", False):
            return
        self._versions["sig"] = sig
        st = self._stream()
        lib = self.lib
        with torch.no_grad():
            torch._foreach_copy_([self.rt_w[:6], self.rt_w[6:], self.rt_b[:6], self.rt_b[6:]],
                                 [self.P["pnp_net.fc_r.weight"].detach(), self.P["pnp_net.fc_t.weight"].detach(), self.P["pnp_net.fc_r.bias"].detach(),
                                  self.P["pnp_net.fc_t.bias"].detach()])
        Ls = self.layers["backbone.conv1"]
        check(lib.gdrn_pack_stem_w(ptr(self.P[Ls.src[0]]), ptr(Ls.wf), self.dt, st), "pack_stem_w")
        if self.stem_direct:
            check(lib.gdrn_pack_stem_w32(ptr(self.P[Ls.src[0]]), ptr(self.stem_w32), self.dt, st), "pack_stem_w32")
        if not hasattr(self, "_pack_tasks") or getattr(self, "_pack_dirty", False):
            self._build_pack_table()
            self._pack_dirty = False
        check(lib.gdrn_pack_multi(ptr(self._pack_tasks), ptr(self._pack_starts), self._pack_n[0], self._pack_n[1], self.dt, st), "pack_multi")

    def repack_bucket(self, b):
        if not hasattr(self, "_pack_tasks") or getattr(self, "_pack_dirty", False):
            return False
        lib, st = self.lib, self._stream()
        nb = len(self.bucket_bounds)
        if b == 0:
            with torch.no_grad():
                torch._foreach_copy_([self.rt_w[:6], self.rt_w[6:], self.rt_b[:6], self.rt_b[6:]],
                                     [self.P["pnp_net.fc_r.weight"].detach(), self.P["pnp_net.fc_t.weight"].detach(), self.P["pnp_net.fc_r.bias"].detach(),
                                      self.P["pnp_net.fc_t.bias"].detach()])
        if b == nb - 1:
            Ls = self.layers["backbone.conv1"]
            if self.stem_direct:
                check(lib.gdrn_pack_stem_w32(ptr(self.P[Ls.src[0]]), ptr(self.stem_w32), self.dt, st), "pack_stem_w32")
            else:
                check(lib.gdrn_pack_stem_w(ptr(self.P[Ls.src[0]]), ptr(Ls.wf), self.dt, st), "pack_stem_w")
        pb = self._pack_buckets[b]
        if pb is not None:
            check(lib.gdrn_pack_multi(ptr(pb[0]), ptr(pb[1]), pb[2], pb[3], self.dt, st), "pack_multi(bucket)")
        return True

    def mark_packed(self):
        self._versions["sig"] = tuple(p._version for p in self.P.values())

    def plan(self, B, bn_train, with_loss):
        key = (B, bool(bn_train), bool(with_loss))
        p = self.plans.get(key)
        if p is None:
            from .plan import Plan

            p = self.plans[key] = Plan(self, B, bool(bn_train), bool(with_loss))
            self.plan_builds += 1
            while len(self.plans) > self.max_plans:
                self.plans.pop(next(iter(self.plans)))
        else:
            self.plans.move_to_end(key)
        return p


class LossScaleState:

    def __init__(self, dev, scale, growth):
        self.t = torch.zeros(16, dtype=torch.int32, device=dev)
        self.f = self.t.view(torch.float32)
        self.write(scale=scale, growth=growth)

    @property
    def ptr(self):
        return self.t.data_ptr()

    def write(self, scale=None, growth=None, base_step=None):
        if scale is not None:
            self.f[5:7] = torch.tensor([float(scale), 1.0 / float(scale)], dtype=torch.float32).to(self.t.device, non_blocking=True)
        if growth is not None:
            self.t[4:5] = int(growth)
        if base_step is not None:
            self.t[7:8] = int(base_step)
            self.t[1:2] = 0

    def read(self):
        v = self.t.cpu()
        fv = v.view(torch.float32)
        return dict(flag=int(v[0]), applied=int(v[1]), skipped=int(v[2]), good=int(v[3]), growth=int(v[4]), scale=float(fv[5]), inv_scale=float(fv[6]),
                    base_step=int(v[7]), last_overflowed=int(v[8]))


_hip_rt = None


def make_stream(dev, prio="normal"):
    global _hip_rt
    if prio == "high":
        return torch.cuda.Stream(device=dev, priority=-1)
    if prio != "low":
        return torch.cuda.Stream(device=dev)
    try:
        if _hip_rt is None:
            path = "libamdhip64.so"
            with open("/proc/self/maps") as f:
                for line in f:
                    if "libamdhip64" in line:
                        path = line.split()[-1]
                        break
            _hip_rt = C.CDLL(path)
        least, greatest = C.c_int(0), C.c_int(0)
        _hip_rt.hipDeviceGetStreamPriorityRange(C.byref(least), C.byref(greatest))
        h = C.c_void_p()
        with torch.cuda.device(dev):
            err = _hip_rt.hipStreamCreateWithPriority(C.byref(h), C.c_uint(1), C.c_int(max(least.value, 1)))
        if err != 0 or not h.value:
            raise OSError(f"hipStreamCreateWithPriority returned {err}")
    except (OSError, AttributeError) as ex:
        import logging
# ... 5 lines not shown
```

gdr-net_amd/plan.py:

```python
import ctypes as C
from types import SimpleNamespace as NS

import torch

from . import cabi
from .cabi import ACC_ROWS, PREZEROED, ConvParams, PoseParams, S2Params, S2dParams, WgradParams, check, ptr
from .engine import HEAD_CONVS, RESNET34_LAYERS, RESNET34_PLANES, _ru

F32t = torch.float32


def _launch(fn, what, args, meta=None):
    cargs = tuple(ptr(a) if isinstance(a, torch.Tensor) else a for a in args)

    def run(st, ctx):
        check(fn(*cargs, st), what)

    run.args = args
    if meta is not None:
        run.meta = meta
    return run


def _launch_struct(fn, what, params, meta=None):
# ... 175 lines not shown
        return (op if bnb is None else self._with_coef(op, bnb.key, nrows)), nrows

    def _conv_meta(self, L, cp, halo_tile, Hi, Wi, Ho, Wo, mode, dgrad):
        e, ref = self.e, C.byref(cp)
        bm, bn = C.c_int(0), C.c_int(0)
        e.lib.gdrn_conv_tile(ref, C.byref(bm), C.byref(bn))
        small = (Ho * Wo) if (mode == 0 and (not dgrad or L.kind == "convT")) else (Hi * Wi)
        dn = "bf16" if e.h16 else "f32"
        th, tw, hbn = halo_tile or (0, 0, 0)
        if halo_tile and cp.w_frag == 2:
            kname = f"conv3x3_v3_kernel<{th},{hbn},{'2,4,1' if hbn == 256 else '2,2,2'},{cp.xf_mode}>"
        elif halo_tile:
            kname = f"conv3x3_halo_kernel<{dn},{th},{tw},{hbn},{cp.xf_mode},{int(e.lib.gdrn_conv3x3_halo_waves(ref)) // 4}>"
        else:
            kname = f"conv_gemm_kernel<{dn},{bm.value},{bn.value}>"
        return self._meta(kname, self._macs(L, small), (self.B * Hi * Wi * cp.Cin + self.B * Ho * Wo * cp.Cout + cp.Cout * cp.Cin * cp.KH * cp.KW) * e.esz,
                          L.key + (":dgrad" if dgrad else ""))

    def _s2(self, L, which, x, y, Hi, Ho, Ld=None, yd=None, stats=None, stats_d=None, bias=None, bias_d=None, act=0, bnb=None):
        e = self.e
        w = getattr(L, {"f": "wfF", "e": "wfF_e", "d": "wdF"}[which], None)
        if not e.h16 or w is None:
            return None
        dgrad = which == "d"
        cin, cout, w_rows = (L.cin_d, L.I, L.rows_d) if dgrad else (L.cin_f, L.O, L.rows_f)
        sp = S2Params()
        sp.x, sp.w, sp.y = ptr(x), ptr(w), ptr(y)
        sp.bias, sp.stats, sp.act = ptr(bias), ptr(stats), act
        if Ld is not None:
            sp.wd, sp.yd, sp.bias_d, sp.stats_d = ptr(Ld.wf_e if which == "e" else Ld.wf), ptr(yd), ptr(bias_d), ptr(stats_d)
            sp.yd_cs, sp.wd_rows = yd.shape[-1], Ld.rows_f
            assert Ld.cin_f == L.cin_f, (L.key, Ld.key)
        if bnb is not None:
            self._fill_bnb(sp, bnb)
        sp.Hi = sp.Wi = Hi
        sp.Ho = sp.Wo = Ho
        sp.Cin, sp.x_cs, sp.Cout, sp.y_cs = cin, x.shape[-1], cout, y.shape[-1]
        sp.N, sp.w_rows, sp.dtype = self.B, w_rows, e.dt
        if not int(e.lib.gdrn_conv3x3s2_ok(C.byref(sp))):
            return None
        self.keep.append(sp)
        nrows = int(e.lib.gdrn_conv3x3s2_stats_rows(C.byref(sp)))
        role = " (data gradient)" if dgrad else ""
        maps = 1 + (Ld is not None) + (bnb is not None)
        meta = self._meta(f"conv3x3s2_kernel<{'true' if Ld is not None else 'false'}>" + role,
                          self._macs(L, Ho * Ho) + (self._macs(Ld, Ho * Ho) if Ld is not None else 0),
                          (self.B * Hi * Hi * cin + maps * self.B * Ho * Ho * cout + cout * cin * 9) * 2,
                          L.key + (":dgrad" if dgrad else "") + ("+downsample" if Ld is not None else ""))
        op = _launch_struct(e.lib.gdrn_conv3x3s2, f"conv3x3s2{role} {L.key}", sp, meta)
        return (op if bnb is None else self._with_coef(op, bnb.key, nrows)), nrows

    def _s2d(self, L, which, dy, dx, Ho, Hi, Ld=None, dyd=None, bnb=None, stats=None, bias=None, act=0):
        e = self.e
        w = getattr(L, {"f": "wfF", "e": "wfF_e", "d": "wdF"}[which], None)
        if not e.h16 or w is None:
            return None
        fwd = which != "d"
        cin, cout, w_rows = (L.O, L.cin_f, L.rows_f) if fwd else (L.cin_f, L.cin_d, L.rows_d)
        sp = S2dParams()
        sp.dy, sp.w, sp.dx = ptr(dy), ptr(w), ptr(dx)
        sp.bias, sp.stats, sp.act = ptr(bias), ptr(stats), act
        if Ld is not None:
            sp.dyd, sp.wdd, sp.dyd_cs, sp.wdd_rows = ptr(dyd), ptr(Ld.wd), dyd.shape[-1], Ld.rows_d
            assert Ld.cin_d == L.cin_d, (L.key, Ld.key)
        if bnb is not None:
            self._fill_bnb(sp, bnb)
        sp.Hi = sp.Wi = Hi
        sp.Ho = sp.Wo = Ho
        sp.Cin, sp.dx_cs, sp.Cout, sp.dy_cs = cin, dx.shape[-1], cout, dy.shape[-1]
        sp.N, sp.w_rows, sp.dtype = self.B, w_rows, e.dt
        if not int(e.lib.gdrn_conv3x3s2_dgrad_ok(C.byref(sp))):
            return None
        self.keep.append(sp)
        nrows = int(e.lib.gdrn_conv3x3s2_dgrad_rows(C.byref(sp)))
        role = " (forward)" if fwd else ""
        tf = lambda b: "true" if b else "false"
        meta = self._meta(f"conv3x3s2_dgrad_kernel<{tf(Ld is not None)},{tf(bnb is not None)}>" + role,
                          self._macs(L, Ho * Ho) + (self._macs(Ld, Ho * Ho) if Ld is not None else 0),
                          (self.B * Hi * Hi * cin + (2 if Ld is not None else 1) * self.B * Ho * Ho * cout + cout * cin * 9) * 2,
                          L.key + ("" if fwd else ":dgrad") + ("+downsample:dgrad" if Ld is not None else ""))
        op = _launch_struct(e.lib.gdrn_conv3x3s2_dgrad, f"conv3x3s2_dgrad{role} {L.key}", sp, meta)
        return (op if bnb is None else self._with_coef(op, bnb.key, nrows)), nrows

    def _wgrad(self, L, x, dy, Hi, Wi, Ho, Wo, stride, pad, cin, cout, x_cs, dy_cs, KH=None, KW=None, defer=False):
        e = self.e
        wp = WgradParams()
        wp.x, wp.dy, wp.dw = ptr(x), ptr(dy), ptr(L.dwp)
        wp.Hi, wp.Wi, wp.Cin, wp.x_cs = Hi, Wi, cin, x_cs
        wp.Ho, wp.Wo, wp.Cout, wp.dy_cs = Ho, Wo, cout, dy_cs
        wp.KH, wp.KW, wp.stride, wp.pad = KH or L.KH, KW or L.KW, stride, pad
        wp.M, wp.dtype, wp.splits, wp.variant = self.B * Ho * Wo, e.dt, 0, 0
        self.keep.append(wp)
        if e.use_halo and L.kind in ("conv", "convT") and L.KK == 9 and bool(e.lib.gdrn_conv3x3_wgrad_ok(C.byref(wp))):
            self._wgrad_deferred.append((len(self.bwd_groups), L, wp, (2.0 * self._macs(L, Ho * Wo),
                                                                      2.0 * self.B * (Hi * Wi * cin + Ho * Wo * cout) + 4.0 * cout * cin * 9)))
            return None

        self._zero_regions.append(self._pad16(L.dwp, e.dwp_flat))
        bco, bci = (64 if cout <= 64 else 128), (128 if cin % 128 == 0 else 64)
        meta = self._meta(f"conv_wgrad_kernel<{'bf16' if e.h16 else 'f32'},{bco},{bci}>", self._macs(L, Ho * Wo),
                          self.B * (Hi * Wi * cin + Ho * Wo * cout) * e.esz + 4 * cout * cin * wp.KH * wp.KW, L.key + ":wgrad")
        return self._side(_launch_struct(e.lib.gdrn_conv_wgrad, f"conv_wgrad {L.key}", wp, meta), defer)

    @staticmethod
    def _side(op, defer=False):
        op.side = True
        op.defer = bool(defer)
        return op

    def _merge_forks(self):
        e = self.e
        if not e.wgrad_stream:
            return
        first = list(e.bucket_first_group)
        for bkt, g0 in enumerate(first):
            hi = first[bkt - 1] if bkt else len(self.bwd_groups)
            moved = []
            for gi in range(hi - 1, g0 - 1, -1):
                g = self.bwd_groups[gi]
                moved += [op for op in g if getattr(op, "defer", False)]
                self.bwd_groups[gi] = [op for op in g if not getattr(op, "defer", False)]
            if not moved:
                continue
            g = self.bwd_groups[g0]
            at = next((i for i, op in enumerate(g) if getattr(op, "bucket_end", False)), len(g))
            if bkt == len(first) - 1 and self._front_n:
                at = 0
            g[at:at] = moved

    @staticmethod
    def _pad16(t, flat):
        off = (t.data_ptr() - flat.data_ptr()) // 4
        assert 0 <= off and off % 4 == 0 and off + t.numel() <= flat.numel(), off
        return flat[off: min(off + _ru(t.numel(), 4), flat.numel())]

    def _grad16(self, g):
        return self._pad16(g, self.e.grad_flat)

    def _build_zero_table(self):
        from .cabi import ZeroTask, to_device_table

        e = self.e
        chunk = e.lib.gdrn_zero_chunk()
        tasks, starts = [], [0]
        seen = set()
        for t in self._zero_regions:
            if t.data_ptr() in seen:
                continue
            seen.add(t.data_ptr())
            assert t.dtype == torch.float32 and t.is_contiguous() and t.data_ptr() % 16 == 0 and (t.numel() * 4) % 16 == 0, (t.shape, t.data_ptr() % 16)
            n16 = t.numel() * 4 // 16
            tasks.append(ZeroTask(p=t.data_ptr(), n16=n16))
            starts.append(starts[-1] + (n16 + chunk - 1) // chunk)
        self._zero_tab = (to_device_table(tasks, e.dev), torch.tensor(starts, dtype=torch.int32, device=e.dev), len(tasks), starts[-1])

    def _unpack(self, L):
        e = self.e
        lib = e.lib
        O, I, KK = L.O, L.I, L.KK
        for n_ in L.src:
            self.grad_group[n_] = len(self.bwd_groups)
        if L.kind == "stem":
            g = e.grads[L.src[0]]
            return self._side(_launch(lib.gdrn_unpack_stem_w, "unpack_stem_w", (L.dwp, g)))
        self._unpack_pending.append((len(self.bwd_groups), L))
        return None

    def _bn_fwd(self, bnkey, raw, rows, C_, npix, y, residual=None, relu=1, stats=None):
        e, lib = self.e, self.e.lib
        stats = self.stats if stats is None else stats
        s = NS(mean=e._empty(C_, dtype=torch.float32), invstd=e._empty(C_, dtype=torch.float32),
               scale=e._empty(C_, dtype=torch.float32), shift=e._empty(C_, dtype=torch.float32), C=C_, npix=npix)
        self.bn[bnkey] = s
        g, b = e.P[bnkey + ".weight"], e.P[bnkey + ".bias"]
        rm, rv, nbt = e.Bf[bnkey + ".running_mean"], e.Bf[bnkey + ".running_var"], e.Bf[bnkey + ".num_batches_tracked"]
        ops = []
        if self.bn_train:
            assert rows * 2 * C_ <= stats.numel(), (bnkey, rows, C_)
            ops.append(_launch(lib.gdrn_bn_finalize, "bn_finalize", (stats, rows, C_, float(npix), g, b, rm, rv, nbt, 0.1, 1e-5, s.mean, s.invstd,
                                                                     s.scale, s.shift, e.bn_ws)))
        else:
            self.eval_prep.append(_launch(lib.gdrn_bn_eval_params, "bn_eval_params", (g, b, rm, rv, 1e-5, C_, s.scale, s.shift)))
        if y is not None:
            ops.append(_launch(lib.gdrn_bn_apply, "bn_apply", (raw, s.scale, s.shift, residual, y, npix, C_, relu, e.dt)))
        return ops

    def _xf_ok(self, L):
        return self.e.fuse_xf and self.bn_train and self._halo_layer(L)

    def _bn_coef_op(self, bnkey, rows, nrows):
        e, lib = self.e, self.e.lib
        s = self.bn[bnkey]
        if getattr(s, "ka", None) is None:
            s.ka, s.kb, s.kc = (e._empty(s.C, dtype=torch.float32) for _ in range(3))
        g = e.P[bnkey + ".weight"]
        dg, db = e.grads[bnkey + ".weight"], e.grads[bnkey + ".bias"]
        self.grad_group[bnkey + ".weight"] = self.grad_group[bnkey + ".bias"] = len(self.bwd_groups)
        return _launch(lib.gdrn_bn_bwd_coef, "bn_bwd_coef", (rows, nrows, s.C, s.npix, g, s.mean, s.invstd, s.ka, s.kb, s.kc, dg, db))

    def _conv_bn_eval(self, L, bnkey, x, xs, y, Hi, Wi, Ho, Wo, stride, pad, relu, residual=None, add_cs=0, **kw):
        f = self.e.fold(bnkey, L)
        self._hook_fold()
        return self._conv(L, x, xs, y, Hi, Wi, Ho, Wo, stride, pad, bias=f.shift, addend=residual, add_cs=add_cs, act=1 if relu else 0,
                          evalw=True, **kw)[0]

    def _fusable(self, L):
        e = self.e
        return e.use_halo and e.h16 and L.kind == "conv" and L.wfF is not None

    def _bn_bwd(self, bnkey, dy, ymask, raw, dx, g_out=None, affine_mask=False, sums="here", xf=False):
        e, lib = self.e, self.e.lib
        s = self.bn[bnkey]
        msc, msh = (s.scale, s.shift) if affine_mask else (None, None)
        ym = None if affine_mask else ymask
        ops = []
        if sums == "dgrad":
            self._bn_coef_op(bnkey, self.stats, 1)
            msc = msh = ym = None
        else:
            assert sums in ("here", "upsample"), sums
            nrows = int(lib.gdrn_bn_bwd_reduce_rows(s.npix, s.C, e.dt))
            assert nrows > 0 and nrows * 2 * s.C <= self.stats.numel(), (bnkey, nrows)
            coef = self._bn_coef_op(bnkey, self.stats, nrows)
            if sums == "here":
                ops.append(_launch(lib.gdrn_bn_bwd_reduce, "bn_bwd_reduce", (dy, ym, raw, s.mean, s.invstd, msc, msh, s.npix, s.C, self.stats, e.dt)))
            ops.append(coef)
        if xf:
            assert g_out is None and ym is None
            return ops, dict(mode=4 if msc is not None else 3, x2=raw, a=s.ka, b=s.kb, c=s.kc, msc=msc, msh=msh, out=dx, relu=False)
        ops.append(_launch(lib.gdrn_bn_bwd_apply, "bn_bwd_apply", (dy, ym, raw, s.ka, s.kb, s.kc, msc, msh, s.npix, s.C, dx, g_out, e.dt)))
        return ops, None

    def _unpack_task(self, L, packed_ptr, grad, rows_valid, rows_off=0):
        from .cabi import PackTask

        O, I, KK = L.O, L.I, L.KK
        if L.kind == "convT":
            a = (I, 1, KK, L.out_ch, I, 1, O, O * KK, 0, 1, KK)
        else:
            a = (rows_valid, 1, KK, L.in_ch, rows_valid, 1, I, I * KK, 0, 1, KK)
        A1, A2, T, B, A1v, A2v, Bv, s1, s2, st, sb = a
        return PackTask(src=packed_ptr, dst=grad.data_ptr(), A1=A1, A2=A2, T=T, B=B, A1v=A1v, A2v=A2v, Bv=Bv, flip=0, s1=s1, s2=s2,
                        st=st, sb=sb, n=A1v * A2v * T * Bv, frag=0, pad_=0)

    def _bucket_end(self, bkt, op):
        e = self.e
        op.bucket_end = True
        g = self.bwd_groups[e.bucket_first_group[bkt]]
        if e.wgrad_stream and bkt == len(e.bucket_first_group) - 1 and e.bucket_first_group[bkt] == 0:
            g.insert(self._front_n, op)
            self._front_n += 1
        else:
            g.append(op)

    def _table_op(self, fn, what, tasks, starts, tables, *extra):
        tab = cabi.to_device_table(tasks, self.e.dev)
        stt = torch.tensor(starts, dtype=torch.int32, device=self.e.dev)
        tables.append((tab, stt))
        op = _launch(fn, what, (tab, stt, len(tasks), starts[-1]) + extra)
        op.side = True
        return op

    def _finish_unpack(self):
        from .cabi import WreduceTask

        e, lib = self.e, self.e.lib
        chunk = lib.gdrn_pack_chunk()
        assert len(self.bwd_groups) == 29, len(self.bwd_groups)
# ... 146 lines not shown
        else:
            grp = [_launch(lib.gdrn_maxpool_bwd, "maxpool_bwd", (d_p0, idx0, raw0, s0.scale, s0.shift, g_stem, B, 128, 128, 64, None, None, None, e.dt))]
            grp += self._bn_bwd("backbone.bn1", g_stem, None, raw0, g_stem)[0]
            grp.append(self._wgrad(Ls, self.img_p, g_stem, 262, 272, 128, 128, 2, 0, 64, 64, 4, 64, KH=7, KW=1))
            grp.append(self._unpack(Ls))
        self.bwd_groups.append(grp)
        return NS(x=p0, d_x=d_p0, Hc=64, inpl=64, prev_raw2=None, pend=None)

    def _block(self, c, li, b, nb, pl):
        e, B, E = self.e, self.B, self._E
        pfx = f"backbone.layer{li}.{b}"
        stride = 2 if (b == 0 and li > 1) else 1
        Ho = c.Hc // stride
        k = NS(pfx=pfx, li=li, b=b, nb=nb, pl=pl, stride=stride, Ho=Ho, L1=e.layers[pfx + ".conv1"], L2=e.layers[pfx + ".conv2"],
               Ld=e.layers.get(pfx + ".downsample.0"), rawd=None)
        k.raw1, k.a1, k.raw2, k.out = E(B, Ho, Ho, pl), E(B, Ho, Ho, pl), E(B, Ho, Ho, pl), E(B, Ho, Ho, pl)
        self.tensors.update({pfx + ".raw1": k.raw1, pfx + ".a1": k.a1, pfx + ".raw2": k.raw2, pfx + ".out": k.out})
        pend = None
        if not self.bn_train:
            self._block_eval(c, k)
        else:
            pend = self._block_fwd(c, k)
            if self.has_backward:
                self._block_bwd(c, k)
        c.x, c.Hc, c.inpl, c.prev_raw2, c.pend = k.out, Ho, pl, k.raw2, pend

    def _block_eval(self, c, k):
        e, lib, B = self.e, self.e.lib, self.B
        x, Hc, inpl = c.x, c.Hc, c.inpl
        pfx, pl, Ho, stride, L1, L2, Ld, a1, out = k.pfx, k.pl, k.Ho, k.stride, k.L1, k.L2, k.Ld, k.a1, k.out
        if e.h16 and Ld is None and inpl == 64 and pl == 64 and e.use_halo and B >= e.halo_min_b and L1.wfF is not None \
                and L1.wfmt.get("e", 1) == 1 and L2.wfmt.get("e", 1) == 1 and int(lib.gdrn_block64_eval_ok(B, Hc, Hc, e.dt)):
            f1, f2 = e.fold(pfx + ".bn1", L1), e.fold(pfx + ".bn2", L2)
            L1.wfmt["e"] = L2.wfmt["e"] = 1
            self._hook_fold()
            self.fwd.append(_launch(lib.gdrn_block64_eval, "block64_eval", (x, L1.wfF_e, f1.shift, L2.wfF_e, f2.shift, out, B, Hc, Hc, e.dt),
                                    dict(kernel="block64_eval_kernel", flops=2.0 * 2 * B * Hc * Hc * 64 * 64 * 9, layer=pfx + ".conv1+conv2")))
            del self.tensors[pfx + ".raw1"], self.tensors[pfx + ".a1"], self.tensors[pfx + ".raw2"]
            return
        s2op = None
        if Ld is not None and e.h16 and L1.wfF is not None:
            f1, fd = e.fold(pfx + ".bn1", L1), e.fold(pfx + ".downsample.1", Ld)
            self._hook_fold()
            res = self._E(B, Ho, Ho, pl)
            s2op = self._s2(L1, "e", x, a1, Hc, Ho, Ld=Ld, yd=res, bias=f1.shift, bias_d=fd.shift, act=1)
        if s2op is not None:
            self.fwd.append(s2op[0])
        else:
            self.fwd.append(self._conv_bn_eval(L1, pfx + ".bn1", x, inpl, a1, Hc, Hc, Ho, Ho, stride, 1, relu=True))
        res = x if Ld is None else (res if s2op is not None else None)
        if Ld is not None and s2op is None:
            res = self._E(B, Ho, Ho, pl)
            self.fwd.append(self._conv_bn_eval(Ld, pfx + ".downsample.1", x, inpl, res, Hc, Hc, Ho, Ho, stride, 0, relu=False))
        self.fwd.append(self._conv_bn_eval(L2, pfx + ".bn2", a1, pl, out, Ho, Ho, Ho, Ho, 1, 1, relu=True, residual=res, add_cs=pl))

    def _block_fwd(self, c, k):
        e, B, S, E = self.e, self.B, self.bn_train, self._E
        x, Hc, inpl, pend = c.x, c.Hc, c.inpl, c.pend
        pfx, pl, Ho, stride, L1, L2, Ld, raw1, a1, raw2, out = k.pfx, k.pl, k.Ho, k.stride, k.L1, k.L2, k.Ld, k.raw1, k.a1, k.raw2, k.out
        npo = B * Ho * Ho
        assert pend is None or self._xf_ok(L1)
        s2op = None
        if Ld is not None and pend is None:
            rawd_ = E(B, Ho, Ho, pl)
            s2op = self._s2(L1, "f", x, raw1, Hc, Ho, Ld=Ld, yd=rawd_, stats=self.stats if S else None, stats_d=self.stats_b if S else None)
        op, rows1 = s2op or self._conv(L1, pend.x1 if pend else x, inpl, raw1, Hc, Hc, Ho, Ho, stride, 1, stats=self.stats if S else None,
                                       xf=dict(pend.xf, out=x) if pend else None)
        self.fwd.append(op)
        xf1 = self._xf_ok(L2)
        self.fwd += self._bn_fwd(pfx + ".bn1", raw1, rows1, pl, npo, None if xf1 else a1)
        op, rows2 = self._conv(L2, raw1 if xf1 else a1, pl, raw2, Ho, Ho, Ho, Ho, 1, 1, stats=self.stats if S else None,
                               xf=_xf_bn_relu(self.bn[pfx + ".bn1"], out=a1) if xf1 else None)
        self.fwd.append(op)
        nxt1 = e.layers.get(f"backbone.layer{k.li}.{k.b + 1}.conv1")
        xf_out = nxt1 is not None and self._xf_ok(nxt1)
        if Ld is None:
            self.fwd += self._bn_fwd(pfx + ".bn2", raw2, rows2, pl, npo, None if xf_out else out, residual=x)
            s2 = self.bn[pfx + ".bn2"]
            return _pend(raw2, dict(mode=2, x2=x, a=s2.scale, c=s2.shift, relu=True)) if xf_out else None
        k.rawd, idn = (rawd_ if s2op is not None else E(B, Ho, Ho, pl)), (None if xf_out else E(B, Ho, Ho, pl))
        self.tensors[pfx + ".rawd"] = k.rawd
        if idn is not None:
            self.tensors[pfx + ".idn"] = idn
        self.fwd += self._bn_fwd(pfx + ".bn2", raw2, rows2, pl, npo, None)
        if s2op is not None:
            self.fwd += self._bn_fwd(pfx + ".downsample.1", k.rawd, rows1, pl, npo, idn, relu=0, stats=self.stats_b)
        else:
            op, rows_d = self._conv(Ld, x, inpl, k.rawd, Hc, Hc, Ho, Ho, stride, 0, stats=self.stats if S else None)
            self.fwd.append(op)
            self.fwd += self._bn_fwd(pfx + ".downsample.1", k.rawd, rows_d, pl, npo, idn, relu=0)
        s2, sd = self.bn[pfx + ".bn2"], self.bn[pfx + ".downsample.1"]
        if xf_out:
            return _pend(raw2, dict(mode=2, x2=k.rawd, a=s2.scale, b=sd.scale, c=s2.shift, c2=sd.shift, relu=True))
        self.fwd.append(_launch(e.lib.gdrn_bn_apply, "bn_apply", (raw2, s2.scale, s2.shift, idn, out, npo, pl, 1, e.dt)))
        return None

    def _block_bwd(self, c, k):
        e, B, E = self.e, self.B, self._E
        x, d_x, Hc, inpl, prev_raw2 = c.x, c.d_x, c.Hc, c.inpl, c.prev_raw2
        pfx, li, b, pl, Ho, stride, L1, L2, Ld = k.pfx, k.li, k.b, k.pl, k.Ho, k.stride, k.L1, k.L2, k.Ld
        raw1, a1, raw2, out, rawd = k.raw1, k.a1, k.raw2, k.out, k.rawd
        d_out = E(B, Ho, Ho, pl)
        d_raw2, d_a1, d_raw1 = E(B, Ho, Ho, pl), E(B, Ho, Ho, pl), E(B, Ho, Ho, pl)
        self.tensors.update({pfx + ".d_out": d_out, pfx + ".d_raw2": d_raw2, pfx + ".d_a1": d_a1, pfx + ".d_raw1": d_raw1})
        pre2 = self._fusable(e.layers[f"backbone.layer{li}.{b + 1}.conv1"]) if b + 1 < k.nb else e.gemm_bnb
        xfb2 = pre2 and self._xf_ok(L2)
        need_dx = d_x is not None
        xfb1 = self._fusable(L2) and self._xf_ok(L1) and Ld is None and need_dx
        if pre2:
            g2 = d_out
            grp, xd2 = self._bn_bwd(pfx + ".bn2", d_out, None, raw2, d_raw2, sums="dgrad", xf=xfb2)
        else:
            g2 = E(B, Ho, Ho, pl)
            self.tensors[pfx + ".g2"] = g2
            grp, xd2 = self._bn_bwd(pfx + ".bn2", d_out, out, raw2, d_raw2, g_out=g2)
        grp.append(self._wgrad(L2, a1, d_raw2, Ho, Ho, Ho, Ho, 1, 1, pl, pl, pl, pl))
        grp.append(self._unpack(L2))
        pre1 = self._fusable(L2)
        grp.append(self._conv(L2, d_out if xfb2 else d_raw2, pl, d_a1, Ho, Ho, Ho, Ho, 1, 1, w=L2.wd, rows=L2.rows_d, cin=L2.cin_d, cout=pl,
                              bnb=_bnb(pfx + ".bn1", raw1, affine=True) if pre1 else None, xf=xd2)[0])
        ops1, xd1 = self._bn_bwd(pfx + ".bn1", d_a1, a1, raw1, d_raw1, affine_mask=True, sums="dgrad" if pre1 else "here", xf=xfb1)
        grp += ops1
        grp.append(self._wgrad(L1, x, d_raw1, Hc, Hc, Ho, Ho, stride, 1, inpl, pl, inpl, pl))
        grp.append(self._unpack(L1))
        if Ld is not None:
            d_rawd, d_xd = E(B, Ho, Ho, pl), E(B, Hc, Hc, inpl)
            self.tensors.update({pfx + ".d_rawd": d_rawd, pfx + ".d_xd": d_xd})
            grp += self._bn_bwd(pfx + ".downsample.1", g2, None, rawd, d_rawd)[0]
            grp.append(self._wgrad(Ld, x, d_rawd, Hc, Hc, Ho, Ho, stride, 0, inpl, pl, inpl, pl, defer=li >= 3))
            grp.append(self._unpack(Ld))
            bnb = _bnb(f"backbone.layer{li - 1}.{RESNET34_LAYERS[li - 2] - 1}.bn2", prev_raw2, x) if e.gemm_bnb else None
            s2d = self._s2d(L1, "d", d_raw1, d_x, Ho, Hc, Ld=Ld, dyd=d_rawd, bnb=bnb) if bnb else None
            if s2d is not None:
                grp.append(s2d[0])
                del self.tensors[pfx + ".d_xd"]
            else:
                grp.append(self._conv(Ld, d_rawd, pl, d_xd, Ho, Ho, Hc, Hc, 2, 0, mode=1, w=Ld.wd, rows=Ld.rows_d, cin=Ld.cin_d, cout=inpl)[0])
                grp.append(self._conv(L1, d_raw1, pl, d_x, Ho, Ho, Hc, Hc, 2, 1, mode=1, w=L1.wd, rows=L1.rows_d, cin=L1.cin_d,
                                      cout=inpl, addend=d_xd, add_cs=inpl, bnb=bnb)[0])
        elif need_dx:
            fuse_prev = b >= 1 and self._fusable(L1)
            grp.append(self._conv(L1, d_a1 if xfb1 else d_raw1, pl, d_x, Ho, Ho, Hc, Hc, 1, 1, w=L1.wd, rows=L1.rows_d, cin=L1.cin_d, cout=inpl,
                                  addend=g2, add_cs=pl, bnb=_bnb(f"backbone.layer{li}.{b - 1}.bn2", prev_raw2, x) if fuse_prev else None, xf=xd1)[0])
        self.bwd_groups.append(grp)
        c.d_x = d_out

    def _head_convT(self, feat, d_feat, prev_raw2):
        e, B, S, T, E = self.e, self.B, self.bn_train, self.has_backward, self._E
        h = "rot_head_net.features."
        LT = e.layers[h + "0"]
        rawt, h0 = E(B, 16, 16, 256), E(B, 16, 16, 256)
        self.tensors.update({h + "0.raw": rawt, h + "0.act": h0})
        xf_first = S and (not HEAD_CONVS[0][2]) and self._xf_ok(e.layers[h + str(HEAD_CONVS[0][0])])
        if not S:
            f = e.fold(h + "1", LT)
            self._hook_fold()
            tf = self._s2d(LT, "e", feat, h0, 8, 16, bias=f.shift, act=1)
            self.fwd.append(tf[0] if tf is not None else
                            self._conv_bn_eval(LT, h + "1", feat, 512, h0, 8, 8, 16, 16, 2, 1, relu=True, mode=1, cin=512, cout=256))
        else:
            op, rows = self._s2d(LT, "f", feat, rawt, 8, 16, stats=self.stats) or \
                self._conv(LT, feat, 512, rawt, 8, 8, 16, 16, 2, 1, mode=1, cin=512, cout=256, stats=self.stats)
            self.fwd.append(op)
            self.fwd += self._bn_fwd(h + "1", rawt, rows, 256, B * 256, None if xf_first else h0)
        d_h0 = None
        if T:
            d_h0, d_rawt = E(B, 16, 16, 256), E(B, 16, 16, 256)
            self.tensors.update({h + "0.d_act": d_h0, h + "0.d_raw": d_rawt})
            pre_t = (not HEAD_CONVS[0][2]) and self._fusable(e.layers[h + str(HEAD_CONVS[0][0])])
# ... 44 lines not shown
        else:
            op, rows = self._conv(Lc, pend_h.x1 if pend_h else xin, 256, raw, Hh, Hh, Hh, Hh, 1, 1, stats=self.stats,
                                  xf=dict(pend_h.xf, out=xin) if pend_h else None)
            self.fwd.append(op)
            self.fwd += self._bn_fwd(h + str(bi), raw, rows, 256, B * Hh * Hh, None if (xf_next or up_next) else act)
        if not up_next:
            self.tensors[h + f"{ci}.act"] = act
        d_act = None
        if T:
            d_act, d_raw = E(B, Hh, Hh, 256), E(B, Hh, Hh, 256)
            self.tensors.update({h + f"{ci}.d_act": d_act, h + f"{ci}.d_raw": d_raw})
            pre = (not nxt[2] and self._fusable(e.layers[h + str(nxt[0])])) if nxt is not None else e.gemm_bnb
            xfb = self._xf_ok(Lc)
            ops, xd = self._bn_bwd(h + str(bi), d_act, act, raw, d_raw, affine_mask=True, xf=xfb,
                                   sums="dgrad" if pre else ("upsample" if up_next else "here"))
            grp += ops
            grp.append(self._wgrad(Lc, xin, d_raw, Hh, Hh, Hh, Hh, 1, 1, 256, 256, 256, 256))
            grp.append(self._unpack(Lc))
            fuse_in = (not up) and self._fusable(Lc)
            grp.append(self._conv(Lc, d_act if xfb else d_raw, 256, d_in, Hh, Hh, Hh, Hh, 1, 1, w=Lc.wd, rows=Lc.rows_d, cin=256, cout=256,
                                  bnb=_bnb(prev_bn, prev_raw, affine=True) if fuse_in else None, xf=xd)[0])
            if up_bwd is not None:
                grp.append(up_bwd)
            self.bwd_groups.append(grp)
        c.pend_h = _pend(raw, _xf_bn_relu(self.bn[h + str(bi)])) if xf_next else None
        c.hx, c.d_hx, c.Hh, c.prev_bn, c.prev_raw, c.up_next = act, d_act, Hh, h + str(bi), raw, up_next

    def _head_out(self, c):
        e, lib, B, T, WL, E = self.e, self.e.lib, self.B, self.has_backward, self.with_loss, self._E
        h, nreg = "rot_head_net.features.", e.nreg
        hx, d_hx, prev_bn, prev_raw = c.hx, c.d_hx, c.prev_bn, c.prev_raw
        LO = e.layers[h + "23"]
        M = B * 64 * 64
        self.hs = 72
        self.head_out = E(M, self.hs, dtype=F32t)
        bias_o = e.P[h + "23.bias"]
        fused_tail = e.h16 and nreg == 64
        if not fused_tail:
            self.fwd.append(self._conv(LO, hx, 256, self.head_out, 64, 64, 64, 64, 1, 0, bias=bias_o, out_f32=1, y_cs=self.hs, cout=e.head_c)[0])
        self.pnp_in = e._zeros(M, 128)
        self.keep.append(self.pnp_in)
        self.tensors.update({"head_out": self.head_out, "pnp_in": self.pnp_in})
        if WL:
            self.acc_rows = int(lib.gdrn_head_conv_tail_loss_rows(B, 4096) if fused_tail else lib.gdrn_head_tail_loss_rows(B, 4096, nreg, self.hs, 128))
            if self.acc_rows <= 0:
                check(self.acc_rows or -1, "head_tail_loss_rows")
            self.acc = E(8 + 8 * self.acc_rows, dtype=torch.float64)
            self.losses = e._zeros(8, dtype=F32t)
        if fused_tail and WL:
            def head_conv_tail(st, ctx):
                check(lib.gdrn_head_conv_tail_loss_fwd(ptr(hx), 256, ptr(LO.wf), LO.rows_f, ptr(bias_o), ctx["coord2d"], ctx["extents"], ptr(self.head_out), self.hs,
                                                       ptr(self.pnp_in), 128, ctx["gt_xyz"], ctx["mask_visib"], ctx["mask_trunc"], ctx["gt_region"], ptr(self.acc),
                                                       B, 4096, nreg, e.dt | PREZEROED, st), "head_conv_tail_loss_fwd")

            head_conv_tail.meta = dict(kernel="head_conv_tail64_kernel<bf16,true>", flops=2.0 * M * 256 * e.head_c, layer=h + "23+tail+losses")
            self.fwd.append(head_conv_tail)
        elif fused_tail:
            def head_conv_tail(st, ctx):
                self.head_valid = bool(ctx.get("want_maps", True))
                check(lib.gdrn_head_conv_tail_fwd(ptr(hx), 256, ptr(LO.wf), LO.rows_f, ptr(bias_o), ctx["coord2d"], ctx["extents"],
                                                  ptr(self.head_out) if ctx.get("want_maps", True) else None, self.hs,
                                                  ptr(self.pnp_in), 128, B, 4096, nreg, e.dt | PREZEROED, st), "head_conv_tail_fwd")

            head_conv_tail.meta = dict(kernel="head_conv_tail64_kernel<bf16,false>", flops=2.0 * M * 256 * e.head_c, layer=h + "23+tail")
            self.fwd.append(head_conv_tail)
        elif WL:
            self.fwd.append(lambda st, ctx: check(lib.gdrn_head_tail_loss_fwd(ptr(self.head_out), self.hs, ctx["coord2d"], ctx["extents"], ptr(self.pnp_in), 128,
                                                                              ctx["gt_xyz"], ctx["mask_visib"], ctx["mask_trunc"], ctx["gt_region"], ptr(self.acc),
                                                                              B, 4096, nreg, e.dt | PREZEROED | ACC_ROWS, st), "head_tail_loss_fwd"))
        else:
            self.fwd.append(lambda st, ctx: check(lib.gdrn_head_tail_fwd(ptr(self.head_out), self.hs, ctx["coord2d"], ctx["extents"],
                                                                         ptr(self.pnp_in), 128, B, 4096, nreg, e.dt | PREZEROED, st), "head_tail_fwd"))
        if not T:
            return
        self.d_head = e._zeros(M, 128)
        self.keep.append(self.d_head)
        self.d_pnp_in = E(M, 128)
        self.gw = e._zeros(8, dtype=F32t)
        self.tensors.update({"d_head": self.d_head, "d_pnp_in": self.d_pnp_in})
        grp = [lambda st, ctx: check(lib.gdrn_head_tail_bwd(ptr(self.head_out), self.hs, ptr(self.pnp_in), ptr(self.d_pnp_in), 128,
                                                            ctx["extents"], ctx["gt_xyz"], ctx["mask_visib"], ctx["mask_trunc"],
                                                            ctx["gt_region"], ptr(self.acc), ptr(self.gw), ptr(self.d_head), 128, B,
                                                            4096, nreg, e.dt | PREZEROED, st), "head_tail_bwd")]
        grp.append(self._wgrad(LO, hx, self.d_head, 64, 64, 64, 64, 1, 0, 256, e.head_c, 256, 128))
        grp.append(self._unpack(LO))
        gb = e.grads[h + "23.bias"]
        self.grad_group[h + "23.bias"] = len(self.bwd_groups)
        self._zero_regions.append(self._grad16(gb))
        grp.append(self._side(_launch(lib.gdrn_bias_grad, "bias_grad", (self.d_head, 128, M, e.head_c, gb, e.dt | PREZEROED))))
        if e.h16 and e.gemm_bnb:
            sbp = self.bn[prev_bn]
            head_dgrad = _launch(lib.gdrn_head_out_dgrad, "head_out_dgrad", (self.d_head, 128, LO.wd, LO.cin_d, prev_raw, 256, sbp.mean, sbp.invstd, sbp.scale,
                                                                             sbp.shift, d_hx, 256, self.stats, B, 4096, e.dt),
                                 self._meta("head_out_dgrad64_kernel<bf16>", self._macs(LO, 4096), M * (128 + 256 + 256) * 2, h + "23:dgrad"))
            grp.append(self._with_coef(head_dgrad, prev_bn, int(lib.gdrn_head_out_dgrad_rows(B, 4096))))
        else:
            grp.append(self._conv(LO, self.d_head, 128, d_hx, 64, 64, 64, 64, 1, 0, w=LO.wd, rows=LO.rows_d, cin=128, cout=256,
                                  bnb=_bnb(prev_bn, prev_raw, affine=True) if e.gemm_bnb else None)[0])
        self.bwd_groups.append(grp)

    def _pnp_conv(self, c, ci, gi):
        e, lib, B, E = self.e, self.e.lib, self.B, self._E
        q = "pnp_net.features."
        px, d_px, Hp, cin = c.px, c.d_px, c.Hp, c.cin
        Lc = e.layers[q + str(ci)]
        Ho = Hp // 2
        r, gact = E(B, Ho, Ho, 128), E(B, Ho, Ho, 128)
        mr = E(B, 32, 2, dtype=F32t)
        self.tensors.update({q + f"{ci}.raw": r, q + f"{ci}.act": gact})
        s2_ok = cin == Lc.cin_f
        self.fwd.append(((self._s2(Lc, "f", px, r, Hp, Ho) if s2_ok else None) or self._conv(Lc, px, cin, r, Hp, Hp, Ho, Ho, 2, 1, cin=cin, cout=128))[0])
        gam, bet = e.P[q + f"{gi}.weight"], e.P[q + f"{gi}.bias"]
        self.fwd.append(_launch(lib.gdrn_gn_relu_fwd, "gn_relu_fwd", (r, gam, bet, gact, mr, B, Ho * Ho, 128, 32, 1e-5, e.dt)))
        d_g = None
        if self.has_backward:
            d_g, d_r = E(B, Ho, Ho, 128), E(B, Ho, Ho, 128)
            self.tensors.update({q + f"{ci}.d_act": d_g, q + f"{ci}.d_raw": d_r})
            dgam, dbet = e.grads[q + f"{gi}.weight"], e.grads[q + f"{gi}.bias"]
            self.grad_group[q + f"{gi}.weight"] = self.grad_group[q + f"{gi}.bias"] = len(self.bwd_groups)
            grp = [_launch(lib.gdrn_gn_relu_bwd, "gn_relu_bwd", (d_g, gact, r, gam, mr, d_r, dgam, dbet, B, Ho * Ho, 128, 32, e.dt | PREZEROED))]
            self._zero_regions += [self._grad16(dgam), self._grad16(dbet)]
            grp.append(self._wgrad(Lc, px, d_r, Hp, Hp, Ho, Ho, 2, 1, cin, 128, cin, 128))
            grp.append(self._unpack(Lc))
            grp.append(((self._s2d(Lc, "d", d_r, d_px, Ho, Hp) if s2_ok else None) or
                        self._conv(Lc, d_r, 128, d_px, Ho, Ho, Hp, Hp, 2, 1, mode=1, w=Lc.wd, rows=Lc.rows_d, cin=128, cout=cin))[0])
            self.bwd_groups.append(grp)
        c.px, c.d_px, c.Hp, c.cin = gact, d_g, Ho, 128

    def _fc_fwd(self, g2act):
        e, lib, B, E = self.e, self.e.lib, self.B, self._E
        L1, L2, L3 = e.layers["pnp_net.fc1"], e.layers["pnp_net.fc2"], e.layers["pnp_net.fc_rt"]
        f1, f2 = E(B, 1024), E(B, 256)
        self.fc_out = e._zeros(B, 64, dtype=F32t)
        self.keep.append(self.fc_out)
        self.tensors.update({"pnp_net.fc1.act": f1, "pnp_net.fc2.act": f2, "fc_out": self.fc_out})
        b1, b2 = e.P["pnp_net.fc1.bias"], e.P["pnp_net.fc2.bias"]
        if e.h16 and B <= 64:
            ws1 = e._zeros(16 * B * 1024 + 64, dtype=F32t)
            self.keep.append(ws1)
            self.fwd.append(_launch(lib.gdrn_linear_splitk, "linear_splitk fc1", (g2act, L1.wf, b1, f1, B, 8192, 1024, 8192, 8192, 1024, 2, ws1, e.dt),
                                    dict(kernel="linear_splitk_kernel", flops=2.0 * B * 8192 * 1024, layer="pnp_net.fc1")))
            ws2 = e._zeros(16 * B * 256 + 64, dtype=F32t)
            self.keep.append(ws2)
            self.fc_tail = (ws2, int(lib.gdrn_linear_splits(1024, 256))) if e.fc_tail else None
            self.fwd.append(_launch(lib.gdrn_linear_splitk, "linear_splitk fc2",
                                    (f1, L2.wf, b2, f2, B, 1024, 256, 1024, 1024, 256, -1 if self.fc_tail else 2, ws2, e.dt),
                                    dict(kernel="linear_splitk_kernel", flops=2.0 * B * 1024 * 256, layer="pnp_net.fc2")))
        else:
            self.fwd.append(self._conv(L1, g2act, 128, f1, 8, 8, 1, 1, 1, 0, bias=b1, act=2, cin=128, cout=1024)[0])
            self.fwd.append(self._conv(L2, f1, 1024, f2, 1, 1, 1, 1, 1, 0, bias=b2, act=2, cin=1024, cout=256)[0])
        if self.fc_tail is None:
            self.fwd.append(self._conv(L3, f2, 256, self.fc_out, 1, 1, 1, 1, 1, 0, bias=e.rt_b, out_f32=1, cin=256, cout=9, y_cs=64)[0])
        self._fc2 = (f2, b2, L3)
        return f1, f2

    def _fc_bwd(self, g2act, d_g2, f1, f2):
        e, lib, B, E = self.e, self.e.lib, self.B, self._E
        L1, L2, L3 = e.layers["pnp_net.fc1"], e.layers["pnp_net.fc2"], e.layers["pnp_net.fc_rt"]
        self.dfc3 = e._zeros(3, B, 64, dtype=F32t)
        d_fc32 = e._zeros(B, 64, dtype=F32t)
        d_fc = E(B, 64)
        d_f2, d_f2p, d_f1, d_f1p = E(B, 256), E(B, 256), E(B, 1024), E(B, 1024)
        self.tensors.update({"d_fc": d_fc, "pnp_net.fc2.d_act": d_f2, "pnp_net.fc2.d_pre": d_f2p, "pnp_net.fc1.d_act": d_f1, "pnp_net.fc1.d_pre": d_f1p})
        o_rt = e.grad_offsets["pnp_net.fc_r.bias"]
        assert e.grad_offsets["pnp_net.fc_t.bias"] == o_rt + 6 and o_rt % 4 == 0
        self._rt_gb_full = e.grad_flat[o_rt:o_rt + 12]
        self.rt_gb = self._rt_gb_full[:9]
        self._zero_regions += [self._rt_gb_full, self._grad16(e.grads["pnp_net.fc1.bias"]), self._grad16(e.grads["pnp_net.fc2.bias"])]
        g_b1, g_b2 = e.grads["pnp_net.fc1.bias"], e.grads["pnp_net.fc2.bias"]
        for n_ in ("pnp_net.fc1.bias", "pnp_net.fc2.bias", "pnp_net.fc_r.bias", "pnp_net.fc_t.bias"):
            self.grad_group[n_] = len(self.bwd_groups)
        comb = _launch(lib.gdrn_combine3, "combine3", (self.dfc3, self.gw.data_ptr() + 20, d_fc32, B * 64))
# ... 144 lines not shown
```

include/gdrn_hip.h:

```cpp
#ifndef GDRN_HIP_H
#define GDRN_HIP_H
#include <stddef.h>
#include <stdint.h>

#ifdef __cplusplus
extern "C" {
#endif

#define GDRN_ABI_VERSION 5
enum { GDRN_DT_F32 = 0, GDRN_DT_BF16 = 1, GDRN_DT_F16 = 2 };
enum { GDRN_OK = 0, GDRN_ERR_ARG = -1, GDRN_ERR_SHAPE = -2, GDRN_ERR_LAUNCH = -3 };
enum { GDRN_F32 = GDRN_DT_F32, GDRN_BF16 = GDRN_DT_BF16, GDRN_E_ARG = GDRN_ERR_ARG, GDRN_E_SHAPE = GDRN_ERR_SHAPE, GDRN_E_LAUNCH = GDRN_ERR_LAUNCH };
enum { GDRN_WGRAD_T64 = 0, GDRN_WGRAD_W128 = 1  };

int gdrn_version(void);
int gdrn_last_hip_error(char* name, int cap);
int gdrn_half_format(void);
enum {
    GDRN_WS_CONV_STATS = 0,
    GDRN_WS_CONV3X3_STATS = 1,
    GDRN_WS_CONV3X3_WGRAD = 2,
    GDRN_WS_STEM_WGRAD = 3,
    GDRN_WS_STEM_STATS = 4,
    GDRN_WS_LINEAR_SPLITK = 5,
    GDRN_WS_BN_BWD_ROWS = 6
};
long long gdrn_workspace_bytes(int op, const void* params);
int gdrn_device_info(int dev, char* name, int* cus, char* arch);

typedef struct gdrn_conv_params {
    const void* x;
    const void* w;
    void* y;
    const float* bias;
    const void* addend;
    float* stats;
    const void* bnb_x;
    const void* bnb_mask;
    const float* bnb_mean;
    const float* bnb_invstd;
    const float* bnb_scale;
    const float* bnb_shift;
    float* bnb_rows;
    int bnb_cs;
    int w_frag;
    int Hi, Wi, Cin, x_cs;
    int Ho, Wo, Cout, y_cs, add_cs;
    int KH, KW, stride, pad;
    int mode, act, out_f32;
    int M, w_rows, dtype;
    int xf_mode, xf_relu;
    const void* xf_x2;
    const float* xf_a;
    const float* xf_b;
    const float* xf_c;
    const float* xf_c2;
    const float* xf_msc;
    const float* xf_msh;
    void* xf_out;
    int halo_waves;
    int v3_min_wg;
} gdrn_conv_params;
int gdrn_conv_gemm(const gdrn_conv_params* p, void* stream);
int gdrn_conv_tile(const gdrn_conv_params* p, int* bm, int* bn);
int gdrn_pack_stem_w32(const float* w, void* dst, int dtype, void* stream);
int gdrn_stem_stats_rows(int N);
int gdrn_stem_conv(const void* canvas, const void* w32, void* y, float* stats, int N, int dtype, void* stream);
int gdrn_head_conv_tail_fwd(const void* x, int x_cs, const void* w, int w_rows, const float* bias, const float* coord2d, const float* extents,
                            float* head, int hs, void* pnp_in, int pcs, int N, int HW, int nreg, int dtype, void* stream);
int gdrn_head_conv_tail_loss_rows(int N, int HW);
int gdrn_head_conv_tail_loss_fwd(const void* x, int x_cs, const void* w, int w_rows, const float* bias, const float* coord2d, const float* extents,
                                 float* head, int hs, void* pnp_in, int pcs, const float* gt_xyz, const float* mask_visib, const float* mask_trunc,
                                 const long long* gt_region, double* acc, int N, int HW, int nreg, int dtype, void* stream);
int gdrn_head_out_dgrad_rows(int N, int HW);
int gdrn_head_out_dgrad(const void* dy, int dy_cs, const void* wd, int wd_cs, const void* raw, int raw_cs, const float* mean, const float* invstd,
                        const float* scale, const float* shift, void* dx, int dx_cs, float* rows, int N, int HW, int dtype, void* stream);
int gdrn_stem_conv_pool(const void* canvas, const void* w32, const float* scale, const float* shift, void* y, int N, int dtype, void* stream);
int gdrn_stem_wgrad_parts(int N);
int gdrn_stem_wgrad(const void* canvas, const void* g, const void* raw, const float* a, const float* b, const float* c, int N,
                    float* ws, float* grad, int dtype, void* stream);
#define GDRN_LINEAR_MAX_SPLITS 16
#define GDRN_LINEAR_NO_FINISH (-1)
int gdrn_linear_splits(int K, int N);
int gdrn_linear_splitk(const void* x, const void* w, const float* bias, void* y, int M, int K, int N, int x_rs, int w_rs,
                       int y_rs, int act, float* ws, int dtype, void* stream);
int gdrn_conv_stats_rows(const gdrn_conv_params* p);
int gdrn_pack_wfrag(const void* src, void* dst, int rows, int Cin, int dtype, void* stream);
int gdrn_pack_wfrag32(const void* src, void* dst, int rows, int Cin, int dtype, void* stream);
int gdrn_conv3x3_wfrag(const gdrn_conv_params* p);
int gdrn_conv3x3_halo(const gdrn_conv_params* p, void* stream);
int gdrn_conv3x3_tile(const gdrn_conv_params* p, int* th, int* tw, int* bn);
int gdrn_conv3x3_stats_rows(const gdrn_conv_params* p);
int gdrn_conv3x3_halo_waves(const gdrn_conv_params* p);

typedef struct gdrn_wgrad_params {
    const void* x;
    const void* dy;
    float* dw;
    float* ws;
    int Hi, Wi, Cin, x_cs;
    int Ho, Wo, Cout, dy_cs;
    int KH, KW, stride, pad;
    int M, dtype, splits, variant;
} gdrn_wgrad_params;
int gdrn_conv_wgrad(const gdrn_wgrad_params* p, void* stream);
int gdrn_conv3x3_wgrad(const gdrn_wgrad_params* p, void* stream);
int gdrn_conv3x3_wgrad_ok(const gdrn_wgrad_params* p);
int gdrn_conv3x3_wgrad_splits(const gdrn_wgrad_params* p);
int gdrn_conv3x3_wgrad_multi(const gdrn_wgrad_params* tasks_dev, const int* blk_start_dev, int ntasks, int nblocks, void* stream);
int gdrn_conv3x3_wgrad_multi_lds(const gdrn_wgrad_params* tasks_dev, const int* blk_start_dev, int ntasks, int nblocks, int lds_bytes, void* stream);
typedef struct gdrn_wreduce_task {
    const float* ws;
    float* dst;
    int nsplit, Cout, Cin, cin_valid;
    long long s_co, s_ci, s_t;
} gdrn_wreduce_task;
int gdrn_wgrad_reduce_multi(const gdrn_wreduce_task* tasks_dev, const int* blk_start_dev, int ntasks, int nblocks, void* stream);

int gdrn_pack4(const float* src, void* dst, int A1, int A2, int T, int B, int A1v, int A2v, int Bv,
               long long s1, long long s2, long long st, long long sb, int flip, int dtype, void* stream);
int gdrn_unpack4(const float* packed, float* dst, int A1, int A2, int T, int B, int A1v, int A2v, int Bv,
                 long long s1, long long s2, long long st, long long sb, int flip, void* stream);
int gdrn_pack_stem_w(const float* w, void* dst, int dtype, void* stream);
int gdrn_unpack_stem_w(const float* packed, float* dw, void* stream);
int gdrn_pack_image(const float* img, void* dst, int N, int H, int W, int Hp, int Wp, int dtype, void* stream);
int gdrn_cast_from_f32(const float* src, void* dst, long long n, int dtype, void* stream);
int gdrn_cast_to_f32(const void* src, float* dst, long long n, int dtype, void* stream);
int gdrn_nhwc_to_nchw_f32(const void* src, int cs, int c0, int C, float* dst, int N, int HW, int dtype, void* stream);

int gdrn_bn_finalize(const float* partial, int rows, int C, double count, const float* gamma, const float* beta,
                     float* running_mean, float* running_var, long long* num_batches_tracked, float momentum,
                     float eps, float* mean, float* invstd, float* scale, float* shift, double* ws, void* stream);
int gdrn_bn_eval_params(const float* gamma, const float* beta, const float* running_mean, const float* running_var,
                        float eps, int C, float* scale, float* shift, void* stream);
int gdrn_bn_apply(const void* x, const float* scale, const float* shift, const void* residual, void* y,
                  long long npix, int C, int relu, int dtype, void* stream);
int gdrn_bn_bwd_reduce_rows(long long npix, int C, int dtype);
int gdrn_bn_bwd_reduce(const void* dy, const void* ymask, const void* x, const float* mean, const float* invstd,
                       const float* mask_scale, const float* mask_shift, long long npix, int C, float* rows, int dtype,
                       void* stream);
int gdrn_bn_bwd_apply(const void* dy, const void* ymask, const void* x, const float* a, const float* b, const float* c,
                      const float* mask_scale, const float* mask_shift, long long npix, int C, void* dx, void* g_out,
                      int dtype, void* stream);
int gdrn_bn_bwd_coef(const float* rows, int nrows, int C, long long npix, const float* gamma, const float* mean,
                     const float* invstd, float* a, float* b, float* c, float* dgamma, float* dbeta, void* stream);
int gdrn_bn_relu_maxpool_fwd(const void* x, const float* scale, const float* shift, void* y, unsigned char* idx,
                             int N, int H, int W, int C, int dtype, void* stream);
int gdrn_maxpool_bwd_rows(int N, int H, int W, int C, int dtype);
int gdrn_maxpool_bwd(const void* dy, const unsigned char* idx, const void* x, const float* scale, const float* shift,
                     void* g, int N, int H, int W, int C, const float* mean, const float* invstd, float* rows, int dtype,
                     void* stream);

int gdrn_upsample2x_fwd(const void* x, void* y, int N, int H, int W, int C, int dtype, void* stream);
int gdrn_upsample2x_bwd(const void* dy, void* dx, int N, int H, int W, int C, int dtype, void* stream);
int gdrn_bn_relu_upsample2x_fwd(const void* x_raw, const float* scale, const float* shift, void* y, int N, int H, int W, int C, int dtype, void* stream);
int gdrn_upsample2x_bwd_bnsums(const void* dy, void* dx, const void* x_raw, const float* mean, const float* invstd, const float* mask_scale,
                               const float* mask_shift, int N, int H, int W, int C, float* rows, int dtype, void* stream);

int gdrn_gn_relu_fwd(const void* x, const float* gamma, const float* beta, void* y, float* mean_rstd, int N,
                     int HW, int C, int G, float eps, int dtype, void* stream);
int gdrn_gn_relu_bwd(const void* dy, const void* y, const void* x, const float* gamma, const float* mean_rstd,
                     void* dx, float* dgamma, float* dbeta, int N, int HW, int C, int G, int dtype, void* stream);

int gdrn_leaky_bwd(const void* dy, const void* y, void* dx, long long n, int dtype, void* stream);
int gdrn_bias_grad(const void* dy, int cs, int rows, int C, float* db, int dtype, void* stream);

int gdrn_head_tail_fwd(const float* head, int hs, const float* coord2d, const float* extents, void* pnp_in, int pcs,
                       int N, int HW, int nreg, int dtype, void* stream);
int gdrn_head_tail_loss_fwd(const float* head, int hs, const float* coord2d, const float* extents, void* pnp_in, int pcs,
                            const float* gt_xyz, const float* mask_visib, const float* mask_trunc, const long long* gt_region,
                            double* acc, int N, int HW, int nreg, int dtype, void* stream);
#define GDRN_ACC_ROWS 0x200
int gdrn_head_tail_loss_rows(int N, int HW, int nreg, int hs, int pcs);
int gdrn_map_loss_finalize_rows(double* acc, int nrows, int N, int HW, float* losses, void* stream);
int gdrn_map_loss_fwd(const float* head, int hs, const float* gt_xyz, const float* mask_visib, const float* mask_trunc,
                      const long long* gt_region, int N, int HW, int nreg, double* acc, void* stream);
int gdrn_head_tail_bwd(const float* head, int hs, const void* pnp_in, const void* d_pnp_in, int pcs,
                       const float* extents, const float* gt_xyz, const float* mask_visib, const float* mask_trunc,
                       const long long* gt_region, const double* acc, const float* gw, void* d_head, int dcs, int N,
                       int HW, int nreg, int dtype, void* stream);

typedef struct gdrn_pose_params {
    const float* fc;
    int fs;
    const float* cams;
    const float* centers;
    const float* whs;
    const float* ratios;
    const float* extents;
    const float* gt_rot;
    const float* gt_trans;
    const float* gt_trans_ratio;
    const float* points;
    int npts;
    const float* sym;
    const int* sym_count;
    int Kmax;
    int N;
    int train;
    float* rot;
    float* trans;
    float* losses;
    float* dfc;
    float* vis;
    float* loss_rows;
    const float* gw;
    void* dfc_comb;
    const float* fc2_ws;
    const float* fc2_bias;
    void* f2_out;
    const void* w_rt;
    const float* b_rt;
    float* fc_w;
    int fc2_splits;
} gdrn_pose_params;
int gdrn_pose_loss(const gdrn_pose_params* p, void* stream);
int gdrn_loss_finalize(double* acc, int nrows, int N, int HW, const float* pose_rows, float* losses, const float* w, float* weighted,
                       void* stream);

int gdrn_combine3(const float* in, const float* w, float* out, int n, void* stream);
int gdrn_map_loss_finalize(const double* acc, int N, int HW, float* losses, void* stream);

int gdrn_ranger_step(float* p, const float* g, float* exp_avg, float* exp_avg_sq, float* slow, int rows, int cols,
                     int gc, float lr, float beta1, float beta2, float eps, float weight_decay, float step_size,
                     int adaptive, int lookahead, float alpha, void* stream);

typedef struct gdrn_pack_task {
    const float* src;
    void* dst;
    const float* scale;
    int A1, A2, T, B, A1v, A2v, Bv;
    int flip;
    long long s1, s2, st, sb;
    long long n;
    int frag;
    int pad_;
} gdrn_pack_task;
typedef struct gdrn_ranger_task {
    float* p;
    const float* g;
    float* m;
    float* v;
    float* slow;
    int rows, cols, gc;
    float lr;
} gdrn_ranger_task;
typedef struct gdrn_zero_task {
    void* p;
    long long n16;
} gdrn_zero_task;
int gdrn_zero_chunk(void);
int gdrn_zero_multi(const gdrn_zero_task* tasks_dev, const int* blk_start_dev, int ntasks, int nblocks, void* stream);
int gdrn_nonfinite_flag(const float* x, long long n, int* flag, void* stream);
typedef struct gdrn_loss_scale_state {
    int flag;
    int applied;
    int skipped;
    int good;
    int growth;
    float scale;
    float inv_scale;
    int base_step;
    int last_overflowed;
    int pad_[7];
} gdrn_loss_scale_state;
int gdrn_loss_scale_update(gdrn_loss_scale_state* state, int applied_step, void* stream);
int gdrn_unscale_or_zero(float* g, long long n, float factor, const gdrn_loss_scale_state* state, void* stream);
int gdrn_scaled_loss_weights(const float* w, const float* w2, int n, const gdrn_loss_scale_state* state, float* out, void* stream);
#define GDRN_PREZEROED 0x100
int gdrn_pack_chunk(void);
int gdrn_pack_transpose_blocks(const gdrn_pack_task* task);
int gdrn_pack_multi(const gdrn_pack_task* tasks_dev, const int* blk_start_dev, int ntasks, int nblocks, int dtype, void* stream);
int gdrn_unpack_multi(const gdrn_pack_task* tasks_dev, const int* blk_start_dev, int ntasks, int nblocks, void* stream);
int gdrn_ranger_multi(const gdrn_ranger_task* tasks_dev, const int* row_start_dev, int ntasks, int total_rows, float beta1,
                      float beta2, float eps, float weight_decay, float step_size, int adaptive, int lookahead, float alpha,
                      float grad_scale, void* stream);
int gdrn_ranger_multi_dyn(const gdrn_ranger_task* tasks_dev, const int* row_start_dev, int ntasks, int total_rows, float beta1,
                          float beta2, float eps, float weight_decay, int n_sma_threshold, int lookahead_k, float alpha,
                          float grad_scale, const gdrn_loss_scale_state* state, void* stream);

typedef struct gdrn_s2_params {
    const void* x;
    const void* w;
    void* y;
    const float* bias;
    float* stats;
    const void* wd;
    void* yd;
    const float* bias_d;
    float* stats_d;
    int Hi, Wi, Cin, x_cs;
    int Ho, Wo, Cout, y_cs, yd_cs;
    int N, w_rows, wd_rows, act, dtype;
    const void* bnb_x;
    const void* bnb_mask;
    const float* bnb_mean;
    const float* bnb_invstd;
    float* bnb_rows;
    int bnb_cs;
} gdrn_s2_params;
int gdrn_conv3x3s2_ok(const gdrn_s2_params* p);
int gdrn_conv3x3s2_stats_rows(const gdrn_s2_params* p);
int gdrn_conv3x3s2(const gdrn_s2_params* p, void* stream);

typedef struct gdrn_s2d_params {
    const void* dy;
    const void* w;
    void* dx;
    const void* dyd;
    const void* wdd;
    const void* bnb_x;
    const void* bnb_mask;
    const float* bnb_mean;
    const float* bnb_invstd;
    float* bnb_rows;
    int bnb_cs;
    int Hi, Wi, Cin, dx_cs;
    int Ho, Wo, Cout, dy_cs, dyd_cs;
    int N, w_rows, wdd_rows, dtype;
    float* stats;
    const float* bias;
    int act;
} gdrn_s2d_params;
int gdrn_conv3x3s2_dgrad_ok(const gdrn_s2d_params* p);
int gdrn_conv3x3s2_dgrad_rows(const gdrn_s2d_params* p);
int gdrn_conv3x3s2_dgrad(const gdrn_s2d_params* p, void* stream);

int gdrn_block64_eval_ok(int N, int H, int W, int dtype);
int gdrn_block64_eval(const void* x, const void* w1, const float* b1, const void* w2, const float* b2, void* y, int N, int H, int W, int dtype,
                      void* stream);

int gdrn_correspondences(const float* mask, const float* coor_x, const float* coor_y, const float* coor_z, long long roi_stride,
                         int pix_stride, const float* coord2d, const float* extents, const float* im_hw, float mask_thr, int N,
                         int HW, float* out_mask, float* out_xyz, float* img_pts, float* model_pts, int* counts, void* stream);

typedef struct gdrn_roi_task {
    const unsigned char* image;
    const float* coord2d;
    const float* xyz_crop;
    const unsigned char* seg;
    const unsigned char* trunc;
    double cx, cy, scale, bw, bh, ox, oy, tz;
    int H, W, x1, y1, x2, y2, cls, pad_;
} gdrn_roi_task;
int gdrn_roi_affine(const gdrn_roi_task* tasks_dev, int B, int in_res, int out_res, double* minv, float* roi_wh, float* resize_ratio,
                    float* trans_ratio, void* stream);
int gdrn_roi_crop_inputs(const gdrn_roi_task* tasks_dev, const double* minv, int B, int in_res, int out_res, const double* pixel_mean,
                         const double* pixel_std, float* roi_img, float* roi_coord_2d, void* stream);
int gdrn_roi_targets(const gdrn_roi_task* tasks_dev, const double* minv, int B, int out_res, const double* fps_points, int nfps,
                     const float* extents, float* roi_xyz, float* roi_mask_trunc, float* roi_mask_visib, float* roi_mask_obj,
                     int* roi_region, void* stream);

long long gdrn_pose_metrics_workspace_bytes(int N, int n_max);
int gdrn_pose_errors(const double* R_est, const double* t_est, const double* R_gt, const double* t_gt, const double* K, const int* labels,
// ... 177 lines not shown
```

Measured before the change: 9145 RoI/s.

## Fuse bias grad into wgrad, pair BN finalizes, and pair weight packing

Several launch-reduction changes land together. The head output bias gradient is now accumulated inside the conv wgrad kernel through LDS plus global atomics, replacing a separate bias_grad launch. Two BN finalizes in downsampling blocks are merged into one rows2 launch. Pack tasks gain paired forward/transposed packing, two-source gathers and an f32 copy mode, with the pack kernel's shared memory unified into one buffer. Atomic bias accumulation makes the result nondeterministic, and the larger shared allocation may lower occupancy of the pack kernel.

Result: no change. 9209 RoI/s, median of 6 (+0.7%).

```diff
diff --git a/gdr-net_amd/cabi.py b/gdr-net_amd/cabi.py
--- a/gdr-net_amd/cabi.py
+++ b/gdr-net_amd/cabi.py
@@ -42,6 +42,15 @@
         ("Ho", I), ("Wo", I), ("Cout", I), ("dy_cs", I),
         ("KH", I), ("KW", I), ("stride", I), ("pad", I),
         ("M", I), ("dtype", I), ("splits", I), ("variant", I),
+        ("db", P),
+    ]
+
+
+class BnFinalizeTask(C.Structure):
+    _fields_ = [
+        ("partial", P), ("gamma", P), ("beta", P), ("running_mean", P), ("running_var", P), ("nbt", P),
+        ("mean", P), ("invstd", P), ("scale", P), ("shift", P),
+        ("count", D), ("momentum", D), ("eps", D), ("rows", I), ("C", I),
     ]
 
 
@@ -81,6 +90,7 @@
         ("src", P), ("dst", P), ("scale", P),
         ("A1", I), ("A2", I), ("T", I), ("B", I), ("A1v", I), ("A2v", I), ("Bv", I), ("flip", I),
         ("s1", LL), ("s2", LL), ("st", LL), ("sb", LL), ("n", LL), ("frag", I), ("pad_", I),
+        ("dst2", P), ("src2", P), ("A1_2", I), ("B_2", I), ("flip2", I), ("frag2", I), ("split_a1", I), ("split_b", I),
     ]
 
 
@@ -185,6 +195,7 @@
     "gdrn_cast_to_f32": [P, P, LL, I, P],
     "gdrn_nhwc_to_nchw_f32": [P, I, I, I, P, I, I, I, P],
     "gdrn_bn_finalize": [P, I, I, D, P, P, P, P, P, F, F, P, P, P, P, P, P],
+    "gdrn_bn_finalize_rows2": [C.POINTER(BnFinalizeTask), C.POINTER(BnFinalizeTask), P],
     "gdrn_bn_eval_params": [P, P, P, P, F, I, P, P, P],
     "gdrn_bn_apply": [P, P, P, P, P, LL, I, I, I, P],
     "gdrn_bn_bwd_reduce_rows": [LL, I, I],
@@ -228,6 +239,7 @@
     "gdrn_nonfinite_flag": [P, LL, P, P],
     "gdrn_pack_multi": [P, P, I, I, I, P],
     "gdrn_pack_transpose_blocks": [P],
+    "gdrn_pack_pair_blocks": [P],
     "gdrn_unpack_multi": [P, P, I, I, P],
     "gdrn_ranger_multi": [P, P, I, I, F, F, F, F, F, I, I, F, F, P],
     "gdrn_ranger_multi_dyn": [P, P, I, I, F, F, F, F, I, I, F, F, P, P],
diff --git a/gdr-net_amd/csrc/conv_wgrad.hip b/gdr-net_amd/csrc/conv_wgrad.hip
--- a/gdr-net_amd/csrc/conv_wgrad.hip
+++ b/gdr-net_amd/csrc/conv_wgrad.hip
@@ -94,7 +94,21 @@
             rb[i] = v;
         }
     };
+    constexpr int VA = Vec16<T>::VEC;
+    const bool do_db = p.db != nullptr && cit == 0 && tap == 0;
+    float bsum[VA];
+#pragma unroll
+    for (int j = 0; j < VA; ++j) bsum[j] = 0.f;
     auto write_stage = [&](int buf) {
+        if (do_db) {
+#pragma unroll
+            for (int i = 0; i < LDA; ++i) {
+                float v[VA];
+                Vec16<T>::unpack(ra[i], v);
+#pragma unroll
+                for (int j = 0; j < VA; ++j) bsum[j] += v[j];
+            }
+        }
 #pragma unroll
         for (int i = 0; i < LDA; ++i)
             *reinterpret_cast<uint4*>(sA + (size_t)buf * BKM * PA + (rowA + RSA * i) * PA + segA * 16) = ra[i];
@@ -165,6 +179,17 @@
         }
         if (s + 1 < s_end) write_stage(buf ^ 1);
         __syncthreads();
+    }
+
+    if (do_db) {
+        float* sdb = reinterpret_cast<float*>(smem);
+        for (int c = tid; c < BCO; c += 256) sdb[c] = 0.f;
+        __syncthreads();
+#pragma unroll
+        for (int j = 0; j < VA; ++j) atomicAdd(&sdb[segA * VA + j], bsum[j]);
+        __syncthreads();
+        for (int c = tid; c < BCO; c += 256)
+            if (co0 + c < p.Cout) unsafeAtomicAdd(p.db + co0 + c, sdb[c]);
     }
 
 #pragma unroll
diff --git a/gdr-net_amd/csrc/multi.hip b/gdr-net_amd/csrc/multi.hip
--- a/gdr-net_amd/csrc/multi.hip
+++ b/gdr-net_amd/csrc/multi.hip
@@ -35,16 +35,25 @@
     else if (k.pad_ == 2) { a1 = o1; a2 = u; t = o2; }
     else { a1 = o1; a2 = o2; t = u; }
 }
+__device__ __forceinline__ const float* pack_src(const gdrn_pack_task& k, int& a1, int& b) {
+    if (k.src2 != nullptr) {
+        if (k.split_a1 > 0 && a1 >= k.split_a1) { a1 -= k.split_a1; return k.src2; }
+        if (k.split_b > 0 && b >= k.split_b) { b -= k.split_b; return k.src2; }
+    }
+    return k.src;
+}
+
+constexpr int TR_TILE_BYTES = 64 * 68 * 4;
 template <typename T, bool UNPACK>
-__device__ __forceinline__ void tr_tile(const gdrn_pack_task& k, int blk) {
-    __shared__ float tile[64][68];
+__device__ __forceinline__ void tr_tile(const gdrn_pack_task& k, int blk, float (*tile)[68]) {
     const TrGeo g = tr_geo(k);
     const int bt = blk % g.BT; blk /= g.BT;
     const int ut = blk % g.UT; blk /= g.UT;
     const int o2 = blk % g.O2, o1 = blk / g.O2;
     const int u0 = ut * 64, b0 = bt * 64;
     const long long sa = (k.pad_ == 1 ? 0 : k.s1) | (k.pad_ == 2 ? 0 : k.s2) | (k.pad_ == 3 ? 0 : k.st) | k.sb;
-    const bool v4 = (sa & 3) == 0 && (g.Uv & 3) == 0 && (reinterpret_cast<uintptr_t>(UNPACK ? k.dst : (const void*)k.src) & 15) == 0;
+    const bool v4 = (sa & 3) == 0 && (g.Uv & 3) == 0 && (reinterpret_cast<uintptr_t>(UNPACK ? k.dst : (const void*)k.src) & 15) == 0 &&
+                    (UNPACK || k.src2 == nullptr);
     const bool b8 = (k.B & 7) == 0 && (reinterpret_cast<uintptr_t>(UNPACK ? (const void*)k.src : k.dst) & 15) == 0;
     auto strided = [&](int u, int b) -> long long {
         int a1, a2, t;
@@ -72,7 +81,17 @@
         } else {
             for (int i = threadIdx.x; i < 4096; i += 256) {
                 const int uu = i & 63, bb = i >> 6, u = u0 + uu, b = b0 + bb;
-                tile[bb][uu] = valid(u, b) ? k.src[strided(u, b)] : 0.f;
+                float v = 0.f;
+                if (valid(u, b)) {
+                    if (k.src2 == nullptr) v = k.src[strided(u, b)];
+                    else {
+                        int a1, a2, t, bs = b;
+                        tr_idx(k, u, o1, o2, a1, a2, t);
+                        const float* sp = pack_src(k, a1, bs);
+                        v = sp[(long long)a1 * k.s1 + (long long)a2 * k.s2 + (long long)t * k.st + (long long)bs * k.sb];
+                    }
+                }
+                tile[bb][uu] = v;
             }
         }
         __syncthreads();
@@ -125,17 +144,97 @@
     }
 }
 
+constexpr int PAIR_PITCH = 40;
+constexpr int PAIR_TILE_BYTES = 32 * 9 * PAIR_PITCH * 2;
+__device__ __forceinline__ int pair_run(int frag, int j, int r) { return frag == 2 ? (j >> 1) * 64 + (j & 1) * 16 + 32 * r : 32 * j + 16 * r; }
+__device__ __forceinline__ size_t frag_granule(int frag, int A1, int B, int R, int tap, int bcol) {
+    const int kch = B >> 6, kc = bcol >> 6, w = bcol & 63;
+    if (frag == 2) {
+        const int nfr = A1 >> 5, wr = R & 63;
+        const int f = (R >> 6) * 2 + ((wr >> 4) & 1), r = ((wr >> 2) & 3) * 8 + (wr >> 5) * 4 + (wr & 3);
+        return (size_t)((((kc * 9 + tap) * 4 + (w >> 4)) * nfr + f) * 64 + ((w >> 3) & 1) * 32 + r);
+    }
+    int cb, a;
+    if (A1 <= 64) { cb = R >> 4; a = R & 15; }
+    else { const int wr = R & 31; cb = (R >> 5) * 2 + ((wr >> 2) & 1); a = (wr >> 3) * 4 + (wr & 3); }
+    return (size_t)((((cb * 9 + tap) * kch + kc) * 2 + (w >> 5)) * 64 + ((w >> 3) & 3) * 16 + a);
+}
+__device__ __forceinline__ void pack_pair(const gdrn_pack_task& k, int blk, bf16_t (*T)[9][PAIR_PITCH]) {
+    const int nji = k.B >> 5;
+    const int jo = blk / nji, ji = blk - jo * nji;
+    const int ro0 = pair_run(k.frag, jo, 0), ro1 = pair_run(k.frag, jo, 1);
+    const int ri0 = pair_run(k.frag2, ji, 0), ri1 = pair_run(k.frag2, ji, 1);
+    auto orow = [&](int p) { return p < 16 ? ro0 + p : ro1 + p - 16; };
+    auto irow = [&](int p) { return p < 16 ? ri0 + p : ri1 + p - 16; };
+    const bool fastB = k.st == 1 && k.sb == 9, fastA = k.st == 1 && k.s1 == 9 && !fastB;
+    if (fastB || fastA) {
+        const long long S = fastB ? k.s1 : k.sb;
+        const int slowv = fastB ? k.A1v : k.Bv, fastv = fastB ? k.Bv : k.A1v;
+        const bool al = (reinterpret_cast<uintptr_t>(k.src) & 15) == 0 && (S & 3) == 0;
+        for (int q = threadIdx.x; q < 32 * 72; q += 256) {
+            const int ps = q / 72, rq = q - ps * 72, run = rq / 36, f4 = rq - run * 36;
+            const int srow = fastB ? orow(ps) : irow(ps);
+            const int f0 = fastB ? (run ? ri1 : ri0) : (run ? ro1 : ro0);
+            const float* sp = k.src + (long long)srow * S + (long long)f0 * 9 + f4 * 4;
+            float vv[4];
+            if (al && srow < slowv && f0 + 15 < fastv) {
+                const float4 v4 = *reinterpret_cast<const float4*>(sp);
+                vv[0] = v4.x; vv[1] = v4.y; vv[2] = v4.z; vv[3] = v4.w;
+            } else {
+#pragma unroll
+                for (int e = 0; e < 4; ++e) vv[e] = (srow < slowv && f0 + (f4 * 4 + e) / 9 < fastv) ? sp[e] : 0.f;
+            }
+#pragma unroll
+            for (int e = 0; e < 4; ++e) {
+                const int w = f4 * 4 + e, fl = w / 9, tp = w - fl * 9, pf = run * 16 + fl;
+                if (fastB) T[ps][tp][pf] = f2bf(vv[e]);
+                else T[pf][tp][ps] = f2bf(vv[e]);
+            }
+        }
+    } else {
+        for (int e = threadIdx.x; e < 32 * 32 * 9; e += 256) {
+            const int po = e / 288, r = e - po * 288, pi = r / 9, tp = r - pi * 9;
+            const int a1 = orow(po), b = irow(pi);
+            const float v = (a1 < k.A1v && b < k.Bv) ? k.src[(long long)a1 * k.s1 + (long long)b * k.sb + (long long)tp * k.st] : 0.f;
+            T[po][tp][pi] = f2bf(v);
+        }
+    }
+    __syncthreads();
+    bf16_t* d1 = reinterpret_cast<bf16_t*>(k.dst);
+    bf16_t* d2 = reinterpret_cast<bf16_t*>(k.dst2);
+    for (int g = threadIdx.x; g < 9 * 128; g += 256) {
+        const int pl = g & 15, g8 = (g >> 4) & 3, p = ((g >> 6) & 1) * 16 + pl, td = g >> 7;
+        const uint4 v1 = *reinterpret_cast<const uint4*>(&T[p][k.flip ? 8 - td : td][g8 * 8]);
+        *reinterpret_cast<uint4*>(d1 + (frag_granule(k.frag, k.A1, k.B, orow(p), td, irow(g8 * 8)) << 3)) = v1;
+        const int t2 = k.flip2 ? 8 - td : td;
+        uint32_t w2[4];
+#pragma unroll
+        for (int h = 0; h < 4; ++h) w2[h] = (uint32_t)T[g8 * 8 + 2 * h][t2][p] | ((uint32_t)T[g8 * 8 + 2 * h + 1][t2][p] << 16);
+        *reinterpret_cast<uint4*>(d2 + (frag_granule(k.frag2, k.A1_2, k.B_2, irow(p), td, orow(g8 * 8)) << 3)) = make_uint4(w2[0], w2[1], w2[2], w2[3]);
+    }
+}
+
 template <typename T>
 __global__ __launch_bounds__(256) void pack_multi_kernel(const gdrn_pack_task* __restrict__ tasks, const int* __restrict__ blk_start,
                                                          int ntasks) {
     constexpr int EPS = 128 / (int)sizeof(T), GE = 16 / (int)sizeof(T);
+    constexpr int BRICK_BYTES = 16 * 9 * 72 * 2;
+    __shared__ __attribute__((aligned(16))) unsigned char pk_smem[PAIR_TILE_BYTES > BRICK_BYTES + 64 ? PAIR_TILE_BYTES : BRICK_BYTES + 64];
+    static_assert(sizeof(pk_smem) >= TR_TILE_BYTES, "the transpose tile must fit");
     const int t = find_task(blk_start, ntasks, blockIdx.x);
     const gdrn_pack_task k = tasks[t];
     T* dst = reinterpret_cast<T*>(k.dst);
-    if (k.frag == 3) { tr_tile<T, false>(k, blockIdx.x - blk_start[t]); return; }
+    if (k.frag == 3) { tr_tile<T, false>(k, blockIdx.x - blk_start[t], reinterpret_cast<float (*)[68]>(pk_smem)); return; }
+    if (k.frag == 4) {
+        float* d32 = reinterpret_cast<float*>(k.dst);
+        const long long c0 = (long long)(blockIdx.x - blk_start[t]) * PACK_CHUNK;
+        for (int e = threadIdx.x; e < PACK_CHUNK && c0 + e < k.n; e += 256) d32[c0 + e] = k.src[c0 + e];
+        return;
+    }
     if constexpr (sizeof(T) == 2) {
+        if (k.frag && k.dst2 != nullptr) { pack_pair(k, blockIdx.x - blk_start[t], reinterpret_cast<bf16_t (*)[9][PAIR_PITCH]>(pk_smem)); return; }
         if (k.frag) {
-            __shared__ bf16_t tile[16][9][72];
+            bf16_t (*tile)[9][72] = reinterpret_cast<bf16_t (*)[9][72]>(pk_smem);
             const int brick = blockIdx.x - blk_start[t];
             const int kch = k.B >> 6;
             const int cb = brick / kch, kc = brick - cb * kch;
@@ -145,7 +244,7 @@
                 if (k.frag == 2) { const int f = cb >> 1, r = (cb & 1) * 16 + a; return (f >> 1) * 64 + ((r >> 2) & 1) * 32 + (f & 1) * 16 + (r >> 3) * 4 + (r & 3); }
                 return (cb / FNp) * 16 * FNp + (a >> 2) * (4 * FNp) + (cb % FNp) * 4 + (a & 3);
             };
-            __shared__ float rsc[16];
+            float* rsc = reinterpret_cast<float*>(pk_smem + BRICK_BYTES);
             if (threadIdx.x < 16) rsc[threadIdx.x] = (k.scale != nullptr && srow((int)threadIdx.x) < k.A1v) ? k.scale[srow((int)threadIdx.x)] : 1.f;
             __syncthreads();
             const bool full = srow(15) < k.A1v && b0 + 63 < k.Bv && ((size_t)k.src & 15) == 0;
@@ -245,6 +344,17 @@
             const unsigned ts = k.flip ? (Tt - 1u - tt) : tt;
             const float* sp = k.src + (long long)a1 * k.s1 + (long long)a2 * k.s2 + (long long)ts * k.st;
             const float rs = (k.scale != nullptr && ok) ? k.scale[a1] : 1.f;
+            if (k.src2 != nullptr) {
+#pragma unroll
+                for (int el = 0; el < GE; ++el) {
+                    int as = (int)a1, bs = (int)b0 + el;
+                    const bool okb = ok && bs < k.Bv;
+                    const float* s2p = pack_src(k, as, bs);
+                    v[el] = okb ? s2p[(long long)as * k.s1 + (long long)a2 * k.s2 + (long long)ts * k.st + (long long)bs * k.sb] * rs : 0.f;
+                }
+                Vec16<T>::store(dst + i, v);
+                continue;
+            }
 #pragma unroll
             for (int el = 0; el < GE; ++el) {
                 const int b = (int)b0 + el;
@@ -282,7 +392,9 @@
         float v = 0.f;
         if (a1 < k.A1v && a2 < k.A2v && b < k.Bv) {
             const int ts = k.flip ? (k.T - 1 - tt) : tt;
-            v = k.src[a1 * k.s1 + a2 * k.s2 + ts * k.st + b * k.sb] * (k.scale != nullptr ? k.scale[a1] : 1.f);
+            int as = a1, bs = b;
+            const float* sp = pack_src(k, as, bs);
+            v = sp[as * k.s1 + a2 * k.s2 + ts * k.st + bs * k.sb] * (k.scale != nullptr ? k.scale[a1] : 1.f);
         }
         st1<T>(dst + i, v);
     }
@@ -305,7 +417,8 @@
                                                            int ntasks) {
     const int t = find_task(blk_start, ntasks, blockIdx.x);
     const gdrn_pack_task k = tasks[t];
-    if (k.frag == 3) { tr_tile<float, true>(k, blockIdx.x - blk_start[t]); return; }
+    __shared__ __attribute__((aligned(16))) float tr_lds[64][68];
+    if (k.frag == 3) { tr_tile<float, true>(k, blockIdx.x - blk_start[t], tr_lds); return; }
     const long long base = (long long)(blockIdx.x - blk_start[t]) * PACK_CHUNK;
     float* dst = reinterpret_cast<float*>(k.dst);
     if ((k.Bv & 3) == 0 && (k.B & 3) == 0) {
@@ -377,6 +490,14 @@
     return nb > 0 && nb < (1ll << 30) ? (int)nb : 0;
 }
 
+extern "C" int gdrn_pack_pair_blocks(const gdrn_pack_task* k) {
+    if (!k || !k->src || !k->dst || !k->dst2 || k->scale != nullptr || k->src2 != nullptr) return 0;
+    if ((k->frag != 1 && k->frag != 2) || (k->frag2 != 1 && k->frag2 != 2) || k->A2 != 1 || k->T != 9) return 0;
+    if (k->A1 <= 0 || k->B <= 0 || (k->A1 & 63) || (k->B & 63) || k->A1_2 != k->B || k->B_2 != k->A1) return 0;
+    if (k->A1v < 0 || k->A1v > k->A1 || k->Bv < 0 || k->Bv > k->B) return 0;
+    return (k->A1 >> 5) * (k->B >> 5);
+}
+
 extern "C" int gdrn_pack_multi(const gdrn_pack_task* tasks_dev, const int* blk_start_dev, int ntasks, int nblocks, int dtype, void* stream) {
     if (!tasks_dev || !blk_start_dev || ntasks <= 0 || nblocks <= 0) return GDRN_ERR_ARG;
     if (dtype == GDRN_DT_F32) GDRN_LAUNCH(pack_multi_kernel<float>, dim3(nblocks), dim3(256), 0, ST, tasks_dev, blk_start_dev, ntasks);
diff --git a/gdr-net_amd/csrc/norm.hip b/gdr-net_amd/csrc/norm.hip
--- a/gdr-net_amd/csrc/norm.hip
+++ b/gdr-net_amd/csrc/norm.hip
@@ -29,13 +29,11 @@
     for (int j = 0; j < 8; ++j) tot[j] = red[0][j] + red[1][j] + red[2][j] + red[3][j];
 }
 
-__global__ __launch_bounds__(256) void bn_finalize_rows_kernel(const float* __restrict__ partial, int rows, int C, double count,
-                                                               const float* gamma, const float* beta, float* running_mean,
-                                                               float* running_var, long long* nbt, float momentum, float eps,
-                                                               float* mean, float* invstd, float* scale, float* shift) {
-    __shared__ double red[4][8];
+__device__ __forceinline__ void bn_finalize_rows_body(int c4, bool first, const float* __restrict__ partial, int rows, int C, double count,
+                                                      const float* gamma, const float* beta, float* running_mean, float* running_var,
+                                                      long long* nbt, float momentum, float eps, float* mean, float* invstd, float* scale,
+                                                      float* shift, double (*red)[8]) {
     double tot[8];
-    const int c4 = blockIdx.x * 4;
     float k_g = 0.f, k_b = 0.f, k_rm = 0.f, k_rv = 0.f;
     if (threadIdx.x < 4) {
         k_g = gamma[c4 + threadIdx.x];
@@ -61,7 +59,26 @@
             running_var[ch] = (1.f - momentum) * k_rv + momentum * (float)unb;
         }
     }
-    if (blockIdx.x == 0 && threadIdx.x == 0 && nbt != nullptr) *nbt += 1;
+    if (first && threadIdx.x == 0 && nbt != nullptr) *nbt += 1;
+}
+
+__global__ __launch_bounds__(256) void bn_finalize_rows_kernel(const float* __restrict__ partial, int rows, int C, double count,
+                                                               const float* gamma, const float* beta, float* running_mean,
+                                                               float* running_var, long long* nbt, float momentum, float eps,
+                                                               float* mean, float* invstd, float* scale, float* shift) {
+    __shared__ double red[4][8];
+    bn_finalize_rows_body(blockIdx.x * 4, blockIdx.x == 0, partial, rows, C, count, gamma, beta, running_mean, running_var, nbt, momentum, eps,
+                          mean, invstd, scale, shift, red);
+}
+
+__global__ __launch_bounds__(256) void bn_finalize_rows2_kernel(const gdrn_bn_finalize_task a, const gdrn_bn_finalize_task b) {
+    __shared__ double red[4][8];
+    const int na = a.C / 4;
+    const bool second = (int)blockIdx.x >= na;
+    const gdrn_bn_finalize_task& t = second ? b : a;
+    const int blk = second ? (int)blockIdx.x - na : (int)blockIdx.x;
+    bn_finalize_rows_body(blk * 4, blk == 0, t.partial, t.rows, t.C, t.count, t.gamma, t.beta, t.running_mean, t.running_var, t.nbt, (float)t.momentum,
+                          (float)t.eps, t.mean, t.invstd, t.scale, t.shift, red);
 }
 
 __global__ __launch_bounds__(256) void bn_bwd_coef_kernel(const float* __restrict__ rows, int nrows, int C, float inv_n,
@@ -939,6 +956,18 @@
     return GDRN_OK;
 }
 
+extern "C" int gdrn_bn_finalize_rows2(const gdrn_bn_finalize_task* a, const gdrn_bn_finalize_task* b, void* stream) {
+    if (!a || !b) return GDRN_ERR_ARG;
+    for (const gdrn_bn_finalize_task* t : {a, b}) {
+        if (!t->partial || !t->gamma || !t->beta || !t->mean || !t->invstd || !t->scale || !t->shift || t->rows <= 0 || t->C <= 0 || (t->C & 3))
+            return GDRN_ERR_ARG;
+        if ((t->running_mean != nullptr) != (t->running_var != nullptr)) return GDRN_ERR_ARG;
+    }
+    GDRN_LAUNCH(bn_finalize_rows2_kernel, dim3(a->C / 4 + b->C / 4), dim3(256), 0, ST, *a, *b);
+    GDRN_CHECK_LAUNCH();
+    return GDRN_OK;
+}
+
 extern "C" int gdrn_bn_bwd_coef(const float* rows, int nrows, int C, long long npix, const float* gamma, const float* mean,
                                 const float* invstd, float* a, float* b, float* c, float* dgamma, float* dbeta, void* stream) {
     if (!rows || !gamma || !mean || !invstd || !a || !b || !c || nrows <= 0 || C <= 0 || (C & 3) || npix <= 0) return GDRN_ERR_ARG;
diff --git a/gdr-net_amd/engine.py b/gdr-net_amd/engine.py
--- a/gdr-net_amd/engine.py
+++ b/gdr-net_amd/engine.py
@@ -316,38 +316,68 @@
         tab, stt, nt, nb = self._eval_tab
         check(lib.gdrn_pack_multi(ptr(tab), ptr(stt), nt, nb, self.dt, st), "pack_multi(eval)")
 
-    def _build_pack_table(self):
-        from .cabi import PackTask, to_device_table
+    def _pack_task_list(self, pair=True):
+        from .cabi import PackTask
 
         chunk = self.lib.gdrn_pack_chunk()
-        tasks, starts = [], [0]
+        out = []
         for key, L in self.layers.items():
             if L.kind == "stem":
                 continue
-            src = self.rt_w if key == "pnp_net.fc_rt" else self.P[L.src[0]]
+            src = self.P[L.src[0]]
             halo_only = self.use_halo and self.halo_min_b <= 1 and L.wfF is not None and not L.s2 and L.kind == "conv"
-            for which, dst, frag in (("f", L.wf, 0), ("d", L.wd, 0), ("f", L.wfF, L.wfmt["f"] or 1), ("d", L.wdF, L.wfmt["d"] or 1)):
-                if dst is None or (halo_only and not frag):
-                    continue
+            todo = [(which, dst, frag) for which, dst, frag in (("f", L.wf, 0), ("d", L.wd, 0), ("f", L.wfF, L.wfmt["f"] or 1), ("d", L.wdF, L.wfmt["d"] or 1))
+                    if dst is not None and not (halo_only and not frag)]
+
+            def task(which, dst, frag):
                 A1, A2, T, B, A1v, A2v, Bv, s1, s2, st, sb, flip = self._pack_args(L, which)
                 kch = B * (2 if self.h16 else 4) // 128
                 sh = (kch.bit_length() if (frag and kch > 0 and kch & (kch - 1) == 0) else 0)
-                t = PackTask(src=src.data_ptr(), dst=dst.data_ptr(), A1=A1, A2=A2, T=T, B=B, A1v=A1v, A2v=A2v, Bv=Bv, flip=flip,
-                             s1=s1, s2=s2, st=st, sb=sb, n=A1 * A2 * T * B, frag=frag, pad_=sh)
-                tasks.append(t)
-                nblk = (A1 // 16) * (B // 64) if (frag and self.h16) else (cabi.transpose_blocks(self.lib, t) or (t.n + chunk - 1) // chunk)
-                starts.append(starts[-1] + nblk)
+                return PackTask(src=src.data_ptr(), dst=dst.data_ptr(), A1=A1, A2=A2, T=T, B=B, A1v=A1v, A2v=A2v, Bv=Bv, flip=flip,
+                                s1=s1, s2=s2, st=st, sb=sb, n=A1 * A2 * T * B, frag=frag, pad_=sh)
+
+            fr = [c for c in todo if c[2]]
+            if pair and self.h16 and len(fr) == 2 and fr[0][2] == fr[1][2]:
+                t, td = task(*fr[0]), task(*fr[1])
+                t.dst2, t.A1_2, t.B_2, t.flip2, t.frag2 = td.dst, td.A1, td.B, td.flip, td.frag
+                nblk = int(self.lib.gdrn_pack_pair_blocks(C.byref(t)))
+                if nblk > 0 and (td.A1v, td.Bv, td.s1, td.sb, td.st, td.T) == (t.Bv, t.A1v, t.sb, t.s1, t.st, t.T):
+                    out.append((t, nblk, L.src[0]))
+                    todo = [c for c in todo if not c[2]]
+            for which, dst, frag in todo:
+                t = task(which, dst, frag)
+                if key == "pnp_net.fc_rt":
+                    t.src2 = self.P[L.src[1]].data_ptr()
+                    if which == "f":
+                        t.split_a1 = self.P[L.src[0]].shape[0]
+                    else:
+                        t.split_b = self.P[L.src[0]].shape[0]
+                nblk = (t.A1 // 16) * (t.B // 64) if (frag and self.h16) else (cabi.transpose_blocks(self.lib, t) or (t.n + chunk - 1) // chunk)
+                out.append((t, nblk, L.src[0]))
+        if "pnp_net.fc_rt" in self.layers:
+            r0 = self.P["pnp_net.fc_r.weight"].shape[0]
+            for name, dst in (("pnp_net.fc_r.weight", self.rt_w[:r0]), ("pnp_net.fc_t.weight", self.rt_w[r0:]),
+                              ("pnp_net.fc_r.bias", self.rt_b[:r0]), ("pnp_net.fc_t.bias", self.rt_b[r0:])):
+                n = self.P[name].numel()
+                assert n == dst.numel() and self.P[name].is_contiguous() and self.P[name].dtype == torch.float32, name
+                out.append((PackTask(src=self.P[name].data_ptr(), dst=dst.data_ptr(), A1=1, A2=1, T=1, B=n, A1v=1, A2v=1, Bv=n, s1=n, s2=n, st=n, sb=1,
+                                     n=n, frag=4), (n + chunk - 1) // chunk, name))
+        return out
+
+    def _build_pack_table(self):
+        from .cabi import to_device_table
+
+        lst = self._pack_task_list()
+        tasks = [t for t, _, _ in lst]
+        starts = [0]
+        for _, n, _ in lst:
+            starts.append(starts[-1] + n)
         self._pack_tasks = to_device_table(tasks, self.dev)
         self._pack_starts = torch.tensor(starts, dtype=torch.int32, device=self.dev)
         self._pack_n = (len(tasks), starts[-1])
-        off_of = lambda t: self.grad_offsets[names_of[t.src]]
-        names_of = {}
-        for key, L in self.layers.items():
-            if L.kind != "stem":
-                names_of[(self.rt_w if key == "pnp_net.fc_rt" else self.P[L.src[0]]).data_ptr()] = L.src[0]
         self._pack_buckets = []
         for lo, hi in self.bucket_bounds:
-            sel = [(t, n) for t, n in zip(tasks, [starts[i + 1] - starts[i] for i in range(len(tasks))]) if lo <= off_of(t) < hi]
+            sel = [(t, n) for t, n, name in lst if lo <= self.grad_offsets[name] < hi]
             if not sel:
                 self._pack_buckets.append(None)
                 continue
@@ -363,10 +393,6 @@
         self._versions["sig"] = sig
         st = self._stream()
         lib = self.lib
-        with torch.no_grad():
-            torch._foreach_copy_([self.rt_w[:6], self.rt_w[6:], self.rt_b[:6], self.rt_b[6:]],
-                                 [self.P["pnp_net.fc_r.weight"].detach(), self.P["pnp_net.fc_t.weight"].detach(), self.P["pnp_net.fc_r.bias"].detach(),
-                                  self.P["pnp_net.fc_t.bias"].detach()])
         Ls = self.layers["backbone.conv1"]
         check(lib.gdrn_pack_stem_w(ptr(self.P[Ls.src[0]]), ptr(Ls.wf), self.dt, st), "pack_stem_w")
         if self.stem_direct:
@@ -381,11 +407,6 @@
             return False
         lib, st = self.lib, self._stream()
         nb = len(self.bucket_bounds)
-        if b == 0:
-            with torch.no_grad():
-                torch._foreach_copy_([self.rt_w[:6], self.rt_w[6:], self.rt_b[:6], self.rt_b[6:]],
-                                     [self.P["pnp_net.fc_r.weight"].detach(), self.P["pnp_net.fc_t.weight"].detach(), self.P["pnp_net.fc_r.bias"].detach(),
-                                      self.P["pnp_net.fc_t.bias"].detach()])
         if b == nb - 1:
             Ls = self.layers["backbone.conv1"]
             if self.stem_direct:
diff --git a/gdr-net_amd/plan.py b/gdr-net_amd/plan.py
--- a/gdr-net_amd/plan.py
+++ b/gdr-net_amd/plan.py
@@ -281,7 +281,7 @@
         op = _launch_struct(e.lib.gdrn_conv3x3s2_dgrad, f"conv3x3s2_dgrad{role} {L.key}", sp, meta)
         return (op if bnb is None else self._with_coef(op, bnb.key, nrows)), nrows
 
-    def _wgrad(self, L, x, dy, Hi, Wi, Ho, Wo, stride, pad, cin, cout, x_cs, dy_cs, KH=None, KW=None, defer=False):
+    def _wgrad(self, L, x, dy, Hi, Wi, Ho, Wo, stride, pad, cin, cout, x_cs, dy_cs, KH=None, KW=None, defer=False, db=None):
         e = self.e
         wp = WgradParams()
         wp.x, wp.dy, wp.dw = ptr(x), ptr(dy), ptr(L.dwp)
@@ -293,8 +293,10 @@
         if e.use_halo and L.kind in ("conv", "convT") and L.KK == 9 and bool(e.lib.gdrn_conv3x3_wgrad_ok(C.byref(wp))):
             self._wgrad_deferred.append((len(self.bwd_groups), L, wp, (2.0 * self._macs(L, Ho * Wo),
                                                                       2.0 * self.B * (Hi * Wi * cin + Ho * Wo * cout) + 4.0 * cout * cin * 9)))
+            assert db is None, L.key
             return None
 
+        wp.db = ptr(db)
         self._zero_regions.append(self._pad16(L.dwp, e.dwp_flat))
         bco, bci = (64 if cout <= 64 else 128), (128 if cin % 128 == 0 else 64)
         meta = self._meta(f"conv_wgrad_kernel<{'bf16' if e.h16 else 'f32'},{bco},{bci}>", self._macs(L, Ho * Wo),
@@ -365,7 +367,7 @@
         self._unpack_pending.append((len(self.bwd_groups), L))
         return None
 
-    def _bn_fwd(self, bnkey, raw, rows, C_, npix, y, residual=None, relu=1, stats=None):
+    def _bn_fwd(self, bnkey, raw, rows, C_, npix, y, residual=None, relu=1, stats=None, finalize=True):
         e, lib = self.e, self.e.lib
         stats = self.stats if stats is None else stats
         s = NS(mean=e._empty(C_, dtype=torch.float32), invstd=e._empty(C_, dtype=torch.float32),
@@ -376,13 +378,37 @@
         ops = []
         if self.bn_train:
             assert rows * 2 * C_ <= stats.numel(), (bnkey, rows, C_)
-            ops.append(_launch(lib.gdrn_bn_finalize, "bn_finalize", (stats, rows, C_, float(npix), g, b, rm, rv, nbt, 0.1, 1e-5, s.mean, s.invstd,
-                                                                     s.scale, s.shift, e.bn_ws)))
+            s.fin = (stats, rows)
+            if finalize:
+                ops.append(_launch(lib.gdrn_bn_finalize, "bn_finalize", (stats, rows, C_, float(npix), g, b, rm, rv, nbt, 0.1, 1e-5, s.mean, s.invstd,
+                                                                         s.scale, s.shift, e.bn_ws)))
         else:
             self.eval_prep.append(_launch(lib.gdrn_bn_eval_params, "bn_eval_params", (g, b, rm, rv, 1e-5, C_, s.scale, s.shift)))
         if y is not None:
             ops.append(_launch(lib.gdrn_bn_apply, "bn_apply", (raw, s.scale, s.shift, residual, y, npix, C_, relu, e.dt)))
         return ops
+
+    def _bn_finalize2(self, key_a, key_b):
+        from .cabi import BnFinalizeTask
+
+        e = self.e
+        tasks = []
+        for k in (key_a, key_b):
+            s = self.bn[k]
+            stats, rows = s.fin
+            t = BnFinalizeTask(partial=ptr(stats), gamma=ptr(e.P[k + ".weight"]), beta=ptr(e.P[k + ".bias"]), running_mean=ptr(e.Bf[k + ".running_mean"]),
+                               running_var=ptr(e.Bf[k + ".running_var"]), nbt=ptr(e.Bf[k + ".num_batches_tracked"]), mean=ptr(s.mean), invstd=ptr(s.invstd),
+                               scale=ptr(s.scale), shift=ptr(s.shift), count=float(s.npix), rows=rows, C=s.C, momentum=0.1, eps=1e-5)
+            self.keep.append(t)
+            tasks.append(t)
+        ra, rb = C.byref(tasks[0]), C.byref(tasks[1])
+        fn = e.lib.gdrn_bn_finalize_rows2
+
+        def run(st, ctx):
+            check(fn(ra, rb, st), "bn_finalize_rows2")
+
+        run.args = tuple(tasks)
+        return run
 
     def _xf_ok(self, L):
         return self.e.fuse_xf and self.bn_train and self._halo_layer(L)
@@ -695,9 +721,13 @@
         self.tensors[pfx + ".rawd"] = k.rawd
         if idn is not None:
             self.tensors[pfx + ".idn"] = idn
-        self.fwd += self._bn_fwd(pfx + ".bn2", raw2, rows2, pl, npo, None)
+        pair = s2op is not None and S
+        self.fwd += self._bn_fwd(pfx + ".bn2", raw2, rows2, pl, npo, None, finalize=not pair)
         if s2op is not None:
-            self.fwd += self._bn_fwd(pfx + ".downsample.1", k.rawd, rows1, pl, npo, idn, relu=0, stats=self.stats_b)
+            ops_d = self._bn_fwd(pfx + ".downsample.1", k.rawd, rows1, pl, npo, idn, relu=0, stats=self.stats_b, finalize=not pair)
+            if pair:
+                self.fwd.append(self._bn_finalize2(pfx + ".bn2", pfx + ".downsample.1"))
+            self.fwd += ops_d
         else:
             op, rows_d = self._conv(Ld, x, inpl, k.rawd, Hc, Hc, Ho, Ho, stride, 0, stats=self.stats if S else None)
             self.fwd.append(op)
@@ -908,12 +938,13 @@
                                                             ctx["extents"], ctx["gt_xyz"], ctx["mask_visib"], ctx["mask_trunc"],
                                                             ctx["gt_region"], ptr(self.acc), ptr(self.gw), ptr(self.d_head), 128, B,
                                                             4096, nreg, e.dt | PREZEROED, st), "head_tail_bwd")]
-        grp.append(self._wgrad(LO, hx, self.d_head, 64, 64, 64, 64, 1, 0, 256, e.head_c, 256, 128))
-        grp.append(self._unpack(LO))
         gb = e.grads[h + "23.bias"]
         self.grad_group[h + "23.bias"] = len(self.bwd_groups)
         self._zero_regions.append(self._grad16(gb))
-        grp.append(self._side(_launch(lib.gdrn_bias_grad, "bias_grad", (self.d_head, 128, M, e.head_c, gb, e.dt | PREZEROED))))
+        grp.append(self._wgrad(LO, hx, self.d_head, 64, 64, 64, 64, 1, 0, 256, e.head_c, 256, 128, db=gb if e.h16 else None))
+        grp.append(self._unpack(LO))
+        if not e.h16:
+            grp.append(self._side(_launch(lib.gdrn_bias_grad, "bias_grad", (self.d_head, 128, M, e.head_c, gb, e.dt | PREZEROED))))
         if e.h16 and e.gemm_bnb:
             sbp = self.bn[prev_bn]
             head_dgrad = _launch(lib.gdrn_head_out_dgrad, "head_out_dgrad", (self.d_head, 128, LO.wd, LO.cin_d, prev_raw, 256, sbp.mean, sbp.invstd, sbp.scale,
diff --git a/include/gdrn_hip.h b/include/gdrn_hip.h
--- a/include/gdrn_hip.h
+++ b/include/gdrn_hip.h
@@ -102,6 +102,7 @@
     int Ho, Wo, Cout, dy_cs;
     int KH, KW, stride, pad;
     int M, dtype, splits, variant;
+    float* db;
 } gdrn_wgrad_params;
 int gdrn_conv_wgrad(const gdrn_wgrad_params* p, void* stream);
 int gdrn_conv3x3_wgrad(const gdrn_wgrad_params* p, void* stream);
@@ -131,6 +132,21 @@
 int gdrn_bn_finalize(const float* partial, int rows, int C, double count, const float* gamma, const float* beta,
                      float* running_mean, float* running_var, long long* num_batches_tracked, float momentum,
                      float eps, float* mean, float* invstd, float* scale, float* shift, double* ws, void* stream);
+typedef struct gdrn_bn_finalize_task {
+    const float* partial;
+    const float* gamma;
+    const float* beta;
+    float* running_mean;
+    float* running_var;
+    long long* nbt;
+    float* mean;
+    float* invstd;
+    float* scale;
+    float* shift;
+    double count, momentum, eps;
+    int rows, C;
+} gdrn_bn_finalize_task;
+int gdrn_bn_finalize_rows2(const gdrn_bn_finalize_task* a, const gdrn_bn_finalize_task* b, void* stream);
 int gdrn_bn_eval_params(const float* gamma, const float* beta, const float* running_mean, const float* running_var,
                         float eps, int C, float* scale, float* shift, void* stream);
 int gdrn_bn_apply(const void* x, const float* scale, const float* shift, const void* residual, void* y,
@@ -235,6 +251,10 @@
     long long n;
     int frag;
     int pad_;
+    void* dst2;
+    const float* src2;
+    int A1_2, B_2, flip2, frag2;
+    int split_a1, split_b;
 } gdrn_pack_task;
 typedef struct gdrn_ranger_task {
     float* p;
@@ -270,6 +290,7 @@
 #define GDRN_PREZEROED 0x100
 int gdrn_pack_chunk(void);
 int gdrn_pack_transpose_blocks(const gdrn_pack_task* task);
+int gdrn_pack_pair_blocks(const gdrn_pack_task* task);
 int gdrn_pack_multi(const gdrn_pack_task* tasks_dev, const int* blk_start_dev, int ntasks, int nblocks, int dtype, void* stream);
 int gdrn_unpack_multi(const gdrn_pack_task* tasks_dev, const int* blk_start_dev, int ntasks, int nblocks, void* stream);
 int gdrn_ranger_multi(const gdrn_ranger_task* tasks_dev, const int* row_start_dev, int ntasks, int total_rows, float beta1,
```
